# JiGuang283/Ray_Tracing-Rendering

Measured on AMD Instinct MI355X. Metric: Msamples/sec, Cornell Box 800x800 spp=400 MIS, higher is better.
Workload: dtype f64

## Files before the change

### ray_tracing-rendering_amd/csrc/rt_compile.h

```cpp
#pragma once

#include "rt_device.h"

#include <algorithm>
#include <cmath>
#include <cstdlib>
#include <cstring>
#include <map>
#include <set>
#include <vector>

struct CompiledScene {
    std::vector<FSub> subs;
    std::vector<rtr_node> dev_nodes;
    int n_compiled_subtrees = 0;
    std::vector<FInst> inst;
    std::vector<FXf> xf;
    std::vector<FRef> ref;
    std::vector<int32_t> exits;
    std::vector<FBvh> bvh;
    std::vector<double> scan;
    std::vector<FStep> steps;
    std::vector<FGuard> guards;
    std::map<int, std::pair<int, int>> guard_of_ref;
    int step_tail = 0;
    int stack_words = 1;
    bool ok = false;
};

namespace rtc {

constexpr int kLinearMax = 12;
constexpr int kLeafMax = 4;
constexpr int kGroupMax = 8;
constexpr int kMaxInstances = 1 << 18;
inline int top_tree_min() {
    const char* e = std::getenv("RTR_TOP_MIN");
    return e && *e ? std::atoi(e) : 40;
}
constexpr int kMaxTreeDepth = 56;

struct Box {
    double lo[3] = {INFINITY, INFINITY, INFINITY}, hi[3] = {-INFINITY, -INFINITY, -INFINITY};
    void grow(const double* p) {
        for (int c = 0; c < 3; ++c) lo[c] = std::min(lo[c], p[c]), hi[c] = std::max(hi[c], p[c]);
    }
    void grow(const Box& b) {
        grow(b.lo);
        grow(b.hi);
    }
    void pad() {
        for (int c = 0; c < 3; ++c) {
            const double e = 1e-4 + 1e-9 * std::max(std::fabs(lo[c]), std::fabs(hi[c]));
            lo[c] -= e, hi[c] += e;
        }
    }
};

struct PendingRef {
    int node;
    std::vector<int> wrappers;
    Box local;
    int order;
    int group;
    std::vector<int> guards;
};

struct Builder {
    const rtr_scene_desc* s;
    CompiledScene& out;
    int inst_base = 0;
    explicit Builder(CompiledScene& o) : out(o) {}
    double t_lo, t_hi;
    std::vector<int> chain;
    std::vector<int> wrappers;
    std::map<std::vector<uint64_t>, int> inst_of_chain;
    std::vector<std::vector<PendingRef>> pending;
    std::map<std::pair<int, std::vector<uint64_t>>, std::pair<int, int>> seen;
    int visit_counter = 0;
    int current_group = -1, group_counter = 0;
    bool too_complex = false;
    bool guard_mode = false, guard_fail = false;
    int hollows_seen = 0;
    std::vector<int> bvh_stack;
    std::map<std::pair<int, std::vector<uint64_t>>, int> hollows_at_first_visit;
    std::map<int, std::set<int>> hollows_under;
    static constexpr int kGuardLinearMax = 256;

    static uint64_t bits(double v) {
        uint64_t u;
        std::memcpy(&u, &v, 8);
        return u;
    }
    std::vector<uint64_t> chain_key() const {
        std::vector<uint64_t> k;
        for (int w : chain) {
            const rtr_node& n = s->nodes[w];
            k.push_back((uint64_t)n.type);
            k.push_back(bits(n.f[0])), k.push_back(bits(n.f[1])), k.push_back(bits(n.f[2]));
        }
        return k;
    }
    std::vector<uint64_t> full_key() const {
        std::vector<uint64_t> k = chain_key();
        k.push_back(~0ull);
        for (int w : wrappers) k.push_back((uint64_t)s->nodes[w].type);
        return k;
    }

    Box prim_box(const rtr_node& n) const {
        Box b;
        switch (n.type) {
        case RTR_NODE_SPHERE: {
            const double r = std::fabs(n.f[3]);
            double lo[3] = {n.f[0] - r, n.f[1] - r, n.f[2] - r}, hi[3] = {n.f[0] + r, n.f[1] + r, n.f[2] + r};
            b.grow(lo), b.grow(hi);
            break;
        }
        case RTR_NODE_MOVING_SPHERE: {
            const double r = std::fabs(n.f[8]);
            for (double t : {t_lo, t_hi}) {
                const double a = (t - n.f[6]) / (n.f[7] - n.f[6]);
                for (int c = 0; c < 3; ++c) {
                    const double ctr = n.f[c] + a * (n.f[3 + c] - n.f[c]);
                    b.lo[c] = std::min(b.lo[c], ctr - r), b.hi[c] = std::max(b.hi[c], ctr + r);
                }
            }
            break;
        }
        default: {
            const int ka = n.type == RTR_NODE_XY_RECT ? 2 : (n.type == RTR_NODE_XZ_RECT ? 1 : 0);
            const int aa = n.type == RTR_NODE_YZ_RECT ? 1 : 0;
            const int ba = n.type == RTR_NODE_XY_RECT ? 1 : 2;
            b.lo[ka] = n.f[4], b.hi[ka] = n.f[4];
            b.lo[aa] = std::min(n.f[0], n.f[1]), b.hi[aa] = std::max(n.f[0], n.f[1]);
            b.lo[ba] = std::min(n.f[2], n.f[3]), b.hi[ba] = std::max(n.f[2], n.f[3]);
        }
        }
        b.pad();
        return b;
    }

    void walk(int ix) {
        if (too_complex) return;
        const rtr_node& n = s->nodes[ix];
        switch (n.type) {
        case RTR_NODE_BVH:
            bvh_stack.push_back(ix);
            walk(n.a);
            if (n.b != n.a) walk(n.b);
            bvh_stack.pop_back();
            break;
        case RTR_NODE_LIST: {
            bool small = n.b >= 2 && n.b <= kGroupMax && current_group < 0;
            for (int k = 0; k < n.b && small; ++k) small = s->nodes[s->list_children[n.a + k]].type >= RTR_NODE_SPHERE;
            if (small) current_group = group_counter++;
            for (int k = 0; k < n.b; ++k) walk(s->list_children[n.a + k]);
            if (small) current_group = -1;
            break;
        }
        case RTR_NODE_TRANSLATE:
        case RTR_NODE_ROTATE_Y:
            chain.push_back(ix), wrappers.push_back(ix);
            walk(n.a);
            chain.pop_back(), wrappers.pop_back();
            break;
        case RTR_NODE_FLIP_FACE:
            wrappers.push_back(ix);
            walk(n.a);
            wrappers.pop_back();
            break;
        case RTR_NODE_MEDIUM: too_complex = true; break;
        default: {
            const int order = visit_counter++;
// ... 638 lines not shown
```

### ray_tracing-rendering_amd/csrc/rt_debug.h

```cpp
#pragma once

#include "rt_device.h"
#include "rtr_hip.h"

struct rtr_debug_view {
    DScene ds;
    hipStream_t stream;
    int device, n_cus, n_materials;
    int trav;
    size_t stack_bytes;
    int flat_trav;
};
struct rtr_debug_kernel {
    int pipeline;
    int integrator;
    int trav;
    int ms;
    int sorted;
    int shade_phases;
    int lean, quadlit, sort, media, machine;
    int accum;
};
struct rtr_debug_li_out {
    double L[3];
    uint32_t rng_exit;
    int32_t n_closest, n_shadow, pad;
};
struct rtr_debug_plan {
    int32_t fast_ok, has_media, flat_scene, flat_guarded, lean_materials, quad_lights_only, uv_order_dependent, machine_ok;
    int32_t guarded_program, top_tree, needs_uv, n_material_types, shared_div, pair_cast;
    int32_t n_steps, n_visits, n_refs, fast_stack_words, walk_stack_words, n_tie_refs, n_guard_refs;
    int32_t pick_trav, mega_trav, mega_ms, mega_sorted, mega_pair;
    int32_t n_finish;
};
extern "C" {
int rtr_debug_scene_plan(const rtr_scene_desc* scene, int integrator, int flags, rtr_debug_plan* out, size_t size_of_out,
                         int32_t* ref_flags, int64_t cap, void* finish, int64_t finish_cap);
int rtr_debug_frame_shapes(const rtr_scene_desc* scene, int32_t* shapes, int64_t cap, int32_t* n_inst);
int rtr_debug_view_get(rtr_context* ctx, int flags, rtr_debug_view* view, size_t size_of_view);
int rtr_debug_last_kernel(rtr_context* ctx, rtr_debug_kernel* out, size_t size_of_out);
int rtr_debug_li(rtr_context* ctx, const rtr_render_params* params, const int32_t* ijs, rtr_debug_li_out* out, int64_t n);
void rtr_debug_set_error(rtr_context* ctx, const char* msg);
}
```

### ray_tracing-rendering_amd/csrc/rt_device.h

```cpp
#pragma once

#include <hip/hip_runtime.h>
#include <stdint.h>

#include "rtr_hip.h"
#include "rtr_seed.h"

#ifndef RTR_BLOCK
#define RTR_BLOCK 256
#endif

#define RT_DEV __device__ __forceinline__
#define RT_HD __host__ __device__ __forceinline__

typedef double Real;

#define RT_STATS_WORDS 80
#define RT_PROF_BASE 8
#define RT_PROF_REGIONS 32
enum { RG_OTHER = 0, RG_SETUP = 1, RG_RECTS = 2, RG_SPHERES = 3, RG_GENERIC = 4, RG_TREE = 5, RG_LEAVES = 6, RG_FINISH = 7,
       RG_SH_SETUP = 8, RG_SH_RECTS = 9, RG_SH_SPHERES = 10, RG_SH_GENERIC = 11, RG_SH_TREE = 12, RG_SH_LEAVES = 13,
       RG_MEDIA = 14, RG_MATPREP = 15, RG_SHADE_A = 16, RG_SHADE_B = 17, RG_MISS = 18, RG_REGEN = 19, RG_SHADE_RR = 20,
       RG_PARK = 21, RG_BARRIER = 22, RG_EXCHANGE = 23, RG_PAIR_SETUP = 24, RG_PAIR_RUNS = 25, RG_PAIR_SPHERES = 26,
       RG_POLL = 27, RG_BEGIN = 28, RG_SETTLE = 29, RG_COUNT = 30, RG_REJECT = 31,
// ... 72 lines not shown
    s ^= s >> 17;
    s ^= s << 5;
    return s * 2.3283064365386963e-10;
}
RT_DEV Real rng_range(uint32_t& s, Real lo, Real hi) { return lo + (hi - lo) * rng_next(s); }
RT_DEV int rng_int(uint32_t& s, int lo, int hi) { return (int)rng_range(s, lo, hi + 1); }

RT_DEV Real rng_sym(uint32_t& s) {
    s ^= s << 13;
    s ^= s >> 17;
    s ^= s << 5;
    return -1.0 + s * 4.656612873077392578125e-10;
}

RT_DEV V3 random_in_unit_sphere(uint32_t& s) {
    const int region = RT_REGION_CURRENT();
    RT_REGION(RG_REJECT);
    for (;;) {
        Real z = rng_sym(s);
        Real y = rng_sym(s);
        Real x = rng_sym(s);
        V3 p = mk(x, y, z);
        if (len2(p) >= 1) continue;
        RT_REGION(region);
        return p;
    }
}
RT_DEV V3 random_unit_vector(uint32_t& s) { return unit(random_in_unit_sphere(s)); }
RT_DEV V3 random_in_unit_disk(uint32_t& s) {
    for (;;) {
        Real y = rng_sym(s);
        Real x = rng_sym(s);
        V3 p = mk(x, y, 0);
        if (len2(p) >= 1) continue;
        return p;
    }
}
RT_DEV V3 random_cosine_direction(uint32_t& s) {
    Real r1 = rng_next(s);
    Real r2 = rng_next(s);
    Real z = __builtin_sqrt(1 - r2);
    Real phi = 2 * RT_PI * r1;
    Real sphi, cphi;
    sincos(phi, &sphi, &cphi);
    Real x = cphi * __builtin_sqrt(r2);
    Real y = sphi * __builtin_sqrt(r2);
    return mk(x, y, z);
}

RT_DEV Real rcp_refined(Real d) {
    Real r = __builtin_amdgcn_rcp(d);
    Real e = __builtin_fma(-d, r, 1.0);
    r = __builtin_fma(r, e, r);
    e = __builtin_fma(-d, r, 1.0);
    return __builtin_fma(r, e, r);
}
RT_DEV bool rcp_safe(Real d) { return (__builtin_fabs(d) >= 0x1p-100) & (__builtin_fabs(d) <= 0x1p100); }
template <bool SHARED>
RT_DEV Real div_shared(Real n, Real d, Real r, bool guard) {
    if (!SHARED) return n / d;
    const Real q = n * r;
    const Real e = __builtin_fma(-d, q, n);
    Real t = __builtin_fma(e, r, q);
    if (guard && !(__builtin_fabs(n) >= 0x1p-300)) t = n / d;
    return t;
}
struct RayDiv {
    Real rx, ry, rz;
    Real a, ra;
    bool fast;
    bool guard;
};
RT_DEV RayDiv raydiv_none() {
    RayDiv q;
    q.rx = q.ry = q.rz = q.a = q.ra = 0;
    q.fast = q.guard = false;
    return q;
}
RT_DEV bool raydiv_origin_ok(V3 o) {
    return __all((__builtin_fabs(o.x) <= 0x1p80) & (__builtin_fabs(o.y) <= 0x1p80) & (__builtin_fabs(o.z) <= 0x1p80));
}
RT_DEV RayDiv raydiv_make(V3 d, Real tmin, bool origin_ok) {
    RayDiv q;
    q.rx = rcp_refined(d.x), q.ry = rcp_refined(d.y), q.rz = rcp_refined(d.z);
    q.a = q.ra = 0;
    q.guard = !(tmin >= 0x1p-100);
    q.fast = origin_ok && __all(rcp_safe(d.x) & rcp_safe(d.y) & rcp_safe(d.z));
    return q;
}
RT_DEV void raydiv_spheres(RayDiv& q, V3 d) {
    q.a = len2(d);
    q.ra = rcp_refined(q.a);
    q.fast = q.fast && __all(rcp_safe(q.a));
}
RT_DEV V3 raydiv_inv(const RayDiv& q, V3 d) {
    if (q.fast) return mk(q.rx, q.ry, q.rz);
    return mk(1.0 / d.x, 1.0 / d.y, 1.0 / d.z);
}

#define RT_CONST_AS __attribute__((address_space(4)))
template <class T>
RT_DEV const RT_CONST_AS T* as_const(const T* p) {
    return (const RT_CONST_AS T*)(unsigned long long)p;
}
template <class T>
RT_DEV T ld_const(const T* base, int idx) {
    static_assert(sizeof(T) % 8 == 0, "records are multiples of 8 bytes");
    const RT_CONST_AS unsigned long long* src = as_const(reinterpret_cast<const unsigned long long*>(base + idx));
    unsigned long long w[sizeof(T) / 8];
#pragma unroll
    for (unsigned k = 0; k < sizeof(T) / 8; ++k) w[k] = src[k];
    T v;
    __builtin_memcpy(&v, w, sizeof(T));
    return v;
}

struct DScene {
    const rtr_node* nodes;
    const int32_t* list_children;
    const rtr_material* materials;
    const rtr_texture* textures;
    const rtr_perlin* perlin;
    const rtr_image* images;
    const uint8_t* image_bytes;
    const rtr_light* lights;
    rtr_camera camera;
    double background[3];
    int32_t root;
    int32_t n_nodes;
    int32_t n_lights;
    int32_t needs_uv;
    int32_t shared_div;
    int32_t pair_cast;
    const struct FInst* finst;
    const struct FXf* fxf;
    const struct FRef* fref;
    const rtr_node* fprim;
    const double* fscan;
    const struct FMat* fmat;
    const struct FLeaf* fleaf;
    const int32_t* fexit;
    const struct FBvh* fbvh;
    const struct FSub* fsub;
    int32_t n_finst;
    int32_t top_root0, world_inst0, world_linear0;
    float top_bound0;
    int32_t n_fstep;
    const struct FStep* fstep;
    int32_t fstep_tail;
    const struct FGuard* fguard;
    int32_t n_fvisit;
    const struct FVisit* fvisit;
    const struct FFin* ffin;
};

struct FInst {
    double bmin[3], bmax[3];
    int32_t xf_first, n_xf;
    int32_t ref_first, n_ref;
    int32_t bvh_root;
    float bound;
    int32_t flags;
    int32_t scan_first;
    int32_t shape;
    uint64_t runs;
    int32_t xf_type[2];
    double xf_f[2][3];
    double head[6];
};
#define RT_INST_RUNS_MAX 8
#define RT_RUN_BITS 8
#define RT_RUN_COUNT_BITS 5
#define RT_RUN_COUNT_MAX 31
#define RT_INST_XF_INLINE 2
#define RT_INST_ROTATED 1
#define RT_INST_SPHERES 2
#define RT_INST_RUNS 4
#define RT_INST_KEEP_Y 8
#define RT_SHAPE_NONE 0
#define RT_SHAPE_T 1
#define RT_SHAPE_R 2
#define RT_SHAPE_TR 3
#define RT_SHAPE_RT 4
#define RT_SHAPE_OTHER 5
struct FXf {
    int32_t type;
    int32_t pad;
    double f[3];
};
#define RT_EXIT_LONG (~0ull)
struct FRef {
    int32_t node;
    int32_t exit_first;
    int32_t n_exit;
    int32_t pad;
};
struct alignas(16) FFin {
    int32_t kind;
    int32_t mat;
    int32_t levels;
    int32_t flip;
    double op[2][3];
    double g[4];
};
#define RT_FIN_SPHERE 3
#define RT_FIN_ROT0 4
#define RT_FIN_ROT1 8
struct FBvh {
    float lmin[3], lmax[3], rmin[3], rmax[3];
    int32_t left, right;
    int32_t pad[2];
};
#define RT_BVH_DONE (-2147483647 - 1)
struct FMat {
    int32_t type, solid;
    int32_t tex[4];
    int32_t pad[2];
    double f[4];
    double albedo[3];
    double rough, metal;
};
struct FLeaf {
    double f[6];
    int32_t type;
    int32_t tag;
    int32_t pad[2];
};
struct FSub {
    int32_t inst_first, n_inst;
    int32_t top_root;
    int32_t world_inst;
    int32_t world_linear;
    float top_bound;
    int32_t pad[2];
};
#define RT_TOP_INST (1 << 30)
#define RT_NODE_COMPILED 11
struct FStep {
    int32_t kind;
    int32_t sub;
    int32_t mat;
    int32_t pad;
    double neg_inv_density;
    int32_t xf_first, n_xf;
    int32_t exit_first, n_exit;
};
struct FGuard {
    double b[6];
};

struct Hit {
    V3 p, n;
    Real t, u, v;
    int mat;
    bool front;
};

RT_DEV void set_face_normal(Hit& rec, V3 rd, V3 outward) {
    rec.front = dot(rd, outward) < 0;
    rec.n = rec.front ? outward : neg(outward);
}

struct Stack {
    int* col;
    RT_DEV void put(int k, int v) const { col[k * RTR_BLOCK] = v; }
    RT_DEV int get(int k) const { return col[k * RTR_BLOCK]; }
    RT_DEV void putd(int k, Real v) const {
        put(k, __double2loint(v));
        put(k + 1, __double2hiint(v));
    }
    RT_DEV Real getd(int k) const { return __hiloint2double(get(k + 1), get(k)); }
};

#define RT_FRAME_TRANSLATE 8
#define RT_FRAME_ROTATE 14
#define RT_FRAME_FLIP 2
#define RT_LIST_BULK 8
#define RT_LIST_MARK 0x40000000

RT_DEV bool aabb_hit(const double* b, V3 o, V3 inv, Real t_min, Real t_max) {
    {
        Real t0 = (b[0] - o.x) * inv.x, t1 = (b[3] - o.x) * inv.x;
        if (inv.x < 0) {
            Real s = t0;
            t0 = t1, t1 = s;
        }
        t_min = t0 > t_min ? t0 : t_min;
        t_max = t1 < t_max ? t1 : t_max;
        if (t_max <= t_min) return false;
    }
    {
        Real t0 = (b[1] - o.y) * inv.y, t1 = (b[4] - o.y) * inv.y;
        if (inv.y < 0) {
            Real s = t0;
            t0 = t1, t1 = s;
        }
        t_min = t0 > t_min ? t0 : t_min;
        t_max = t1 < t_max ? t1 : t_max;
        if (t_max <= t_min) return false;
    }
    {
        Real t0 = (b[2] - o.z) * inv.z, t1 = (b[5] - o.z) * inv.z;
        if (inv.z < 0) {
            Real s = t0;
            t0 = t1, t1 = s;
        }
// ... 710 lines not shown
            for (int k = RT_INST_XF_INLINE; k < I.n_xf; ++k) {
                const FXf x = ld_const(sc.fxf, I.xf_first + k);
                wrapper_enter(x.type, x.f, lo, ld);
            }
        }
        bool found;
        if (I.bvh_root >= 0) {
            found = scan_instance<ANY, true, false, false>(sc, I, lo, ld, raydiv_none(), time, tmin, tmax, hit_ref, order, st, sp);
        } else if (I.flags & RT_INST_RUNS) {
            RayDiv q = raydiv_make(ld, tmin, origin_ok);
            if (I.flags & RT_INST_SPHERES) raydiv_spheres(q, ld);
            const bool one_box = I.runs == (uint64_t)(RT_RUN_BOX << RT_RUN_COUNT_BITS | 1);
            if (q.fast) {
                if (one_box)
                    run_box<false, true, true>(I.head, I.ref_first, lo, ld, q, tmin, tmax, hit_ref);
                else
                    scan_runs<false, true, true>(sc, I, lo, ld, q, time, tmin, tmax, hit_ref);
            } else {
                if (one_box)
                    run_box<false, false, true>(I.head, I.ref_first, lo, ld, q, tmin, tmax, hit_ref);
                else
                    scan_runs<false, false, true>(sc, I, lo, ld, q, time, tmin, tmax, hit_ref);
            }
            found = ANY && hit_ref != before;
        } else {
            found = leaf_refs<true, false, ANY>(sc, I.ref_first, I.ref_first + I.n_ref, lo, ld, time, tmin, tmax, hit_ref, order);
        }
        if (hit_ref != before) hit_inst = owner, tmax_f = float_above(tmax);
        if (ANY && found) return true;
        node = sp > sp0 ? st.get(--sp) : RT_BVH_DONE;
    }
    return false;
}

template <bool ANY, bool TREES, bool WEXIT, bool TOP, bool GUARD>
__device__ __forceinline__ bool trace_fast(const DScene& sc, const FSub sub, V3 o, V3 d, Real time, Real tmin, Real& tmax,
                                           int& hit_ref, int& hit_inst, const Stack st, const int sp0) {
    const bool top = TOP && sub.top_root >= 0;
    const int inst_first = top ? sub.world_inst : sub.inst_first;
    const int n_inst = top ? (sub.world_linear ? 1 : 0) : sub.n_inst;
    const bool use_boxes = n_inst > RT_FAST_NO_BOX_MAX;
    V3 inv = mk(0, 0, 0);
    if (use_boxes) inv = mk(1.0 / d.x, 1.0 / d.y, 1.0 / d.z);
    hit_ref = -1;
    hit_inst = -1;
    int order = -1;
#ifndef RTR_NO_SHARED_DIV
    const bool origin_ok = (RTR_TREE_SHARED || !TREES) && sc.shared_div != 0 && raydiv_origin_ok(o);
#endif
    for (int ii = inst_first; ii < inst_first + n_inst; ++ii) {
        RT_REGION(WEXIT ? RG_SH_SETUP : RG_SETUP);
        const FInst I = ld_const(sc.finst, ii);
        V3 lo = o, ld = d;
        const int n_xf = I.n_xf;
        if (n_xf) {
            if (use_boxes) {
                Real tn;
                if (!box_enter(I.bmin, I.bmax, o, inv, tmin, tmax, tn)) continue;
            }
            wrapper_enter(I.xf_type[0], I.xf_f[0], lo, ld);
            if (n_xf > 1) wrapper_enter(I.xf_type[1], I.xf_f[1], lo, ld);
            for (int k = RT_INST_XF_INLINE; k < n_xf; ++k) {
                const FXf x = ld_const(sc.fxf, I.xf_first + k);
                wrapper_enter(x.type, x.f, lo, ld);
            }
        }
        RayDiv q = raydiv_none();
#ifndef RTR_NO_SHARED_DIV
        if (RTR_TREE_SHARED || !TREES) {
            q = raydiv_make(ld, tmin, origin_ok);
            if (I.flags & RT_INST_SPHERES) raydiv_spheres(q, ld);
        }
#endif
        bool found;
        if (q.fast)
            found = scan_instance<ANY, TREES, WEXIT, true, GUARD>(sc, I, lo, ld, q, time, tmin, tmax, hit_ref, order, st, sp0);
        else
            found = scan_instance<ANY, TREES, WEXIT, false, GUARD>(sc, I, lo, ld, q, time, tmin, tmax, hit_ref, order, st, sp0);
        RT_REGION(WEXIT ? RG_SH_SETUP : RG_SETUP);
        if (hit_ref >= I.ref_first) hit_inst = ii;
        if (ANY && found) return true;
    }
    if (top) {
        RT_REGION(WEXIT ? RG_SH_TREE : RG_TREE);
        if (trace_top<ANY>(sc, sub, o, d, time, tmin, tmax, hit_ref, hit_inst, order, st, sp0) && ANY) return true;
    }
    return hit_ref >= 0;
}

template <int TYPE>
RT_DEV void pair_rect(Real a0, Real a1, Real b0, Real b1, Real k, int ref, V3 oA, V3 dA, const RayDiv& qA, Real& tmaxA,
                      int& hitA, V3 oB, V3 dB, const RayDiv& qB, Real& tmaxB, int& hitB) {
    const Real tmin = 0.001;
#define RT_PAIR_SEL(V, XY, XZ, YZ) (TYPE == RTR_NODE_XY_RECT ? V.XY : (TYPE == RTR_NODE_XZ_RECT ? V.XZ : V.YZ))
    const Real okA = RT_PAIR_SEL(oA, z, y, x), dkA = RT_PAIR_SEL(dA, z, y, x), rkA = RT_PAIR_SEL(qA, rz, ry, rx);
    const Real okB = RT_PAIR_SEL(oB, z, y, x), dkB = RT_PAIR_SEL(dB, z, y, x), rkB = RT_PAIR_SEL(qB, rz, ry, rx);
    const Real oaA = TYPE == RTR_NODE_YZ_RECT ? oA.y : oA.x, daA = TYPE == RTR_NODE_YZ_RECT ? dA.y : dA.x;
    const Real obA = TYPE == RTR_NODE_XY_RECT ? oA.y : oA.z, dbA = TYPE == RTR_NODE_XY_RECT ? dA.y : dA.z;
    const Real oaB = TYPE == RTR_NODE_YZ_RECT ? oB.y : oB.x, daB = TYPE == RTR_NODE_YZ_RECT ? dB.y : dB.x;
    const Real obB = TYPE == RTR_NODE_XY_RECT ? oB.y : oB.z, dbB = TYPE == RTR_NODE_XY_RECT ? dB.y : dB.z;
#undef RT_PAIR_SEL
    Real nA, nB, tA, tB, uA, wA, u;
    unsigned long long save;
    asm volatile("v_add_f64 %[nA], %[k], -%[okA]\n\t"
                 "v_add_f64 %[nB], %[k], -%[okB]\n\t"
                 "v_mul_f64 %[tA], %[nA], %[rkA]\n\t"
                 "v_mul_f64 %[tB], %[nB], %[rkB]\n\t"
                 "v_fma_f64 %[nA], -%[dkA], %[tA], %[nA]\n\t"
                 "v_fma_f64 %[nB], -%[dkB], %[tB], %[nB]\n\t"
                 "v_fma_f64 %[tA], %[nA], %[rkA], %[tA]\n\t"
                 "v_fma_f64 %[tB], %[nB], %[rkB], %[tB]\n\t"
                 "v_mul_f64 %[uA], %[tA], %[daA]\n\t"
                 "v_mul_f64 %[wA], %[tA], %[dbA]\n\t"
                 "v_add_f64 %[uA], %[oaA], %[uA]\n\t"
                 "v_add_f64 %[wA], %[obA], %[wA]"
                 : [nA] "=&v"(nA), [nB] "=&v"(nB), [tA] "=&v"(tA), [tB] "=&v"(tB), [uA] "=&v"(uA), [wA] "=&v"(wA)
                 : [k] "s"(k), [okA] "v"(okA), [dkA] "v"(dkA), [rkA] "v"(rkA), [okB] "v"(okB), [dkB] "v"(dkB), [rkB] "v"(rkB),
                   [oaA] "v"(oaA), [daA] "v"(daA), [obA] "v"(obA), [dbA] "v"(dbA));
    asm volatile("s_mov_b64 %[save], exec\n\t"
                 "v_cmpx_ngt_f64 vcc, %[tmin], %[tA]\n\t"
                 "v_cmpx_ngt_f64 vcc, %[tA], %[tmaxA]\n\t"
                 "v_cmpx_ngt_f64 vcc, %[a0], %[uA]\n\t"
                 "v_cmpx_nlt_f64 vcc, %[a1], %[uA]\n\t"
                 "v_cmpx_ngt_f64 vcc, %[b0], %[wA]\n\t"
                 "v_cmpx_nlt_f64 vcc, %[b1], %[wA]\n\t"
                 "v_mov_b64 %[tmaxA], %[tA]\n\t"
                 "v_mov_b32 %[hitA], %[ref]\n\t"
                 "s_mov_b64 exec, %[save]\n\t"
                 "v_cmpx_ngt_f64 vcc, %[tmin], %[tB]\n\t"
                 "v_cmpx_ngt_f64 vcc, %[tB], %[tmaxB]\n\t"
                 "s_cbranch_execz .Lpx%=\n\t"
                 "v_mul_f64 %[u], %[tB], %[daB]\n\t"
                 "v_add_f64 %[u], %[oaB], %[u]\n\t"
                 "v_cmpx_ngt_f64 vcc, %[a0], %[u]\n\t"
                 "v_cmpx_nlt_f64 vcc, %[a1], %[u]\n\t"
                 "v_mul_f64 %[u], %[tB], %[dbB]\n\t"
                 "v_add_f64 %[u], %[obB], %[u]\n\t"
                 "v_cmpx_ngt_f64 vcc, %[b0], %[u]\n\t"
                 "v_cmpx_nlt_f64 vcc, %[b1], %[u]\n\t"
                 "v_mov_b64 %[tmaxB], %[tB]\n\t"
                 "v_mov_b32 %[hitB], %[ref]\n"
                 ".Lpx%=:\n\t"
                 "s_mov_b64 exec, %[save]"
                 : [u] "=&v"(u), [save] "=&s"(save), [tmaxA] "+v"(tmaxA), [hitA] "+v"(hitA), [tmaxB] "+v"(tmaxB), [hitB] "+v"(hitB)
                 : [tA] "v"(tA), [uA] "v"(uA), [wA] "v"(wA), [tB] "v"(tB), [oaB] "v"(oaB), [daB] "v"(daB), [obB] "v"(obB),
                   [dbB] "v"(dbB), [a0] "s"(a0), [a1] "s"(a1), [b0] "s"(b0), [b1] "s"(b1), [ref] "s"(ref), [tmin] "s"(tmin)
                 : "vcc");
}
struct PairRay {
    V3 o, d;
    RayDiv q;
};
template <int TYPE>
RT_DEV void pair_rects(const RT_CONST_AS double* p, int cnt, int ref, const PairRay& A, Real& tmaxA, int& hitA, const PairRay& B,
                       Real& tmaxB, int& hitB) {
    int k = 0;
    for (; k + 1 < cnt; k += 2, p += 10) {
        const Real f0 = p[0], f1 = p[1], f2 = p[2], f3 = p[3], f4 = p[4];
        const Real g0 = p[5], g1 = p[6], g2 = p[7], g3 = p[8], g4 = p[9];
        pair_rect<TYPE>(f0, f1, f2, f3, f4, ref + k, A.o, A.d, A.q, tmaxA, hitA, B.o, B.d, B.q, tmaxB, hitB);
        pair_rect<TYPE>(g0, g1, g2, g3, g4, ref + k + 1, A.o, A.d, A.q, tmaxA, hitA, B.o, B.d, B.q, tmaxB, hitB);
    }
    if (k < cnt) pair_rect<TYPE>(p[0], p[1], p[2], p[3], p[4], ref + k, A.o, A.d, A.q, tmaxA, hitA, B.o, B.d, B.q, tmaxB, hitB);
}
RT_DEV void pair_runs(const DScene& sc, const FInst& I, const PairRay& A, Real time, Real& tmaxA, int& hitA, const PairRay& B,
                      Real& tmaxB, int& hitB) {
    const RT_CONST_AS double* p = as_const(sc.fscan) + I.scan_first;
    int ref = I.ref_first;
#pragma nounroll
    for (uint64_t runs = I.runs; runs != 0; runs >>= RT_RUN_BITS) {
        const int type = RTR_NODE_SPHERE + (int)((runs >> RT_RUN_COUNT_BITS) & 7), cnt = (int)(runs & RT_RUN_COUNT_MAX);
        RT_REGION(type >= RTR_NODE_XY_RECT ? RG_PAIR_RUNS : RG_PAIR_SPHERES);
        if (type == RTR_NODE_XY_RECT) {
            pair_rects<RTR_NODE_XY_RECT>(p, cnt, ref, A, tmaxA, hitA, B, tmaxB, hitB);
            p += 5 * cnt;
        } else if (type == RTR_NODE_XZ_RECT) {
            pair_rects<RTR_NODE_XZ_RECT>(p, cnt, ref, A, tmaxA, hitA, B, tmaxB, hitB);
            p += 5 * cnt;
        } else if (type == RTR_NODE_YZ_RECT) {
            pair_rects<RTR_NODE_YZ_RECT>(p, cnt, ref, A, tmaxA, hitA, B, tmaxB, hitB);
            p += 5 * cnt;
        } else if (type == RTR_NODE_SPHERE + RT_RUN_BOX) {
            for (int b = 0, r = ref; b < cnt; ++b, p += 6, r += 6) {
                const Real x0 = p[0], x1 = p[1], y0 = p[2], y1 = p[3], z0 = p[4], z1 = p[5];
                pair_rect<RTR_NODE_XY_RECT>(x0, x1, y0, y1, z1, r, A.o, A.d, A.q, tmaxA, hitA, B.o, B.d, B.q, tmaxB, hitB);
                pair_rect<RTR_NODE_XY_RECT>(x0, x1, y0, y1, z0, r + 1, A.o, A.d, A.q, tmaxA, hitA, B.o, B.d, B.q, tmaxB, hitB);
                pair_rect<RTR_NODE_XZ_RECT>(x0, x1, z0, z1, y1, r + 2, A.o, A.d, A.q, tmaxA, hitA, B.o, B.d, B.q, tmaxB, hitB);
                pair_rect<RTR_NODE_XZ_RECT>(x0, x1, z0, z1, y0, r + 3, A.o, A.d, A.q, tmaxA, hitA, B.o, B.d, B.q, tmaxB, hitB);
                pair_rect<RTR_NODE_YZ_RECT>(y0, y1, z0, z1, x1, r + 4, A.o, A.d, A.q, tmaxA, hitA, B.o, B.d, B.q, tmaxB, hitB);
                pair_rect<RTR_NODE_YZ_RECT>(y0, y1, z0, z1, x0, r + 5, A.o, A.d, A.q, tmaxA, hitA, B.o, B.d, B.q, tmaxB, hitB);
            }
            ref += 5 * cnt;
        } else {
            for (int k = 0; k < cnt; ++k, p += 4) {
                const V3 c = mk(p[0], p[1], p[2]);
                const Real r = p[3];
                Real t;
                if (sphere_hit_t<true>(c, r, A.o, A.d, A.q, 0.001, tmaxA, t)) tmaxA = t, hitA = ref + k;
                if (sphere_hit_t<true>(c, r, B.o, B.d, B.q, 0.001, tmaxB, t)) tmaxB = t, hitB = ref + k;
            }
        }
        ref += cnt;
    }
}
struct PairFrame {
    V3 ao, bo;
    Real adx, adz, bdx, bdz;
};
RT_HD void pair_rot(Real s, Real c, Real x, Real z, Real& rx, Real& rz) {
    rx = c * x - s * z;
    rz = s * x + c * z;
}
RT_HD PairFrame pair_frame(int shape, const double* f0, const double* f1, V3 ao, V3 ad, V3 bo, V3 bd) {
    PairFrame F;
    switch (shape) {
    case RT_SHAPE_T:
        F.ao.x = ao.x - f0[0], F.bo.x = bo.x - f0[0];
        F.ao.y = ao.y - f0[1], F.bo.y = bo.y - f0[1];
        F.ao.z = ao.z - f0[2], F.bo.z = bo.z - f0[2];
        F.adx = ad.x, F.adz = ad.z, F.bdx = bd.x, F.bdz = bd.z;
        break;
    case RT_SHAPE_R:
        pair_rot(f0[0], f0[1], ao.x, ao.z, F.ao.x, F.ao.z), pair_rot(f0[0], f0[1], bo.x, bo.z, F.bo.x, F.bo.z);
        F.ao.y = ao.y, F.bo.y = bo.y;
        pair_rot(f0[0], f0[1], ad.x, ad.z, F.adx, F.adz), pair_rot(f0[0], f0[1], bd.x, bd.z, F.bdx, F.bdz);
        break;
    case RT_SHAPE_TR: {
        const Real ax = ao.x - f0[0], bx = bo.x - f0[0];
        const Real az = ao.z - f0[2], bz = bo.z - f0[2];
        F.ao.y = ao.y - f0[1], F.bo.y = bo.y - f0[1];
        pair_rot(f1[0], f1[1], ax, az, F.ao.x, F.ao.z), pair_rot(f1[0], f1[1], bx, bz, F.bo.x, F.bo.z);
        pair_rot(f1[0], f1[1], ad.x, ad.z, F.adx, F.adz), pair_rot(f1[0], f1[1], bd.x, bd.z, F.bdx, F.bdz);
        break;
    }
    case RT_SHAPE_RT: {
        Real ax, az, bx, bz;
        pair_rot(f0[0], f0[1], ao.x, ao.z, ax, az), pair_rot(f0[0], f0[1], bo.x, bo.z, bx, bz);
        pair_rot(f0[0], f0[1], ad.x, ad.z, F.adx, F.adz), pair_rot(f0[0], f0[1], bd.x, bd.z, F.bdx, F.bdz);
        F.ao.x = ax - f1[0], F.bo.x = bx - f1[0];
        F.ao.y = ao.y - f1[1], F.bo.y = bo.y - f1[1];
        F.ao.z = az - f1[2], F.bo.z = bz - f1[2];
        break;
    }
    default:
        F.ao = ao, F.bo = bo;
        F.adx = ad.x, F.adz = ad.z, F.bdx = bd.x, F.bdz = bd.z;
        break;
    }
    return F;
}
__device__ __forceinline__ void trace_pair(const DScene& sc, V3 ao, V3 ad, Real atime, Real& a_tmax, int& a_ref, int& a_inst,
                                           V3 bo, V3 bd, Real& b_tmax, int& b_ref, const Stack st) {
    a_ref = -1, a_inst = -1, b_ref = -1;
#ifndef RTR_NO_SHARED_DIV
    const bool ok_a = raydiv_origin_ok(ao), ok_b = raydiv_origin_ok(bo);
#else
    const bool ok_a = false, ok_b = false;
#endif
    const Real way = rcp_refined(ad.y), wby = rcp_refined(bd.y);
    const bool wa_y = rcp_safe(ad.y), wb_y = rcp_safe(bd.y);
    for (int ii = 0; ii < sc.n_finst; ++ii) {
        RT_REGION(RG_PAIR_SETUP);
        const FInst I = ld_const(sc.finst, ii);
        PairRay A, B;
        if (I.shape != RT_SHAPE_OTHER) {
            const PairFrame F = pair_frame(I.shape, I.xf_f[0], I.xf_f[1], ao, ad, bo, bd);
            A.o = F.ao, B.o = F.bo;
            A.d = mk(F.adx, ad.y, F.adz), B.d = mk(F.bdx, bd.y, F.bdz);
        } else {
            A.o = ao, A.d = ad, B.o = bo, B.d = bd;
            wrapper_enter(I.xf_type[0], I.xf_f[0], A.o, A.d);
            wrapper_enter(I.xf_type[0], I.xf_f[0], B.o, B.d);
            if (I.n_xf > 1) {
                wrapper_enter(I.xf_type[1], I.xf_f[1], A.o, A.d);
                wrapper_enter(I.xf_type[1], I.xf_f[1], B.o, B.d);
            }
            for (int k = RT_INST_XF_INLINE; k < I.n_xf; ++k) {
                const FXf x = ld_const(sc.fxf, I.xf_first + k);
                wrapper_enter(x.type, x.f, A.o, A.d);
                wrapper_enter(x.type, x.f, B.o, B.d);
            }
        }
        A.q.guard = B.q.guard = false;
        A.q.rx = rcp_refined(A.d.x), A.q.rz = rcp_refined(A.d.z);
        B.q.rx = rcp_refined(B.d.x), B.q.rz = rcp_refined(B.d.z);
        A.q.ry = way, B.q.ry = wby;
        bool sa = rcp_safe(A.d.x) & rcp_safe(A.d.z) & wa_y, sb = rcp_safe(B.d.x) & rcp_safe(B.d.z) & wb_y;
        A.q.a = A.q.ra = B.q.a = B.q.ra = 0;
        if (I.flags & RT_INST_SPHERES) {
            A.q.a = len2(A.d), B.q.a = len2(B.d);
            A.q.ra = rcp_refined(A.q.a), B.q.ra = rcp_refined(B.q.a);
            sa = sa & rcp_safe(A.q.a), sb = sb & rcp_safe(B.q.a);
        }
        if (ok_a && ok_b && __all(sa & sb)) {
            A.q.fast = B.q.fast = true;
            pair_runs(sc, I, A, atime, a_tmax, a_ref, B, b_tmax, b_ref);
        } else {
            A.q.fast = ok_a && __all(sa), B.q.fast = ok_b && __all(sb);
            int order = -1;
            if (A.q.fast)
                scan_instance<false, false, false, true>(sc, I, A.o, A.d, A.q, atime, 0.001, a_tmax, a_ref, order, st, 0);
            else
                scan_instance<false, false, false, false>(sc, I, A.o, A.d, A.q, atime, 0.001, a_tmax, a_ref, order, st, 0);
            if (B.q.fast)
                scan_instance<true, false, true, true>(sc, I, B.o, B.d, B.q, 0.0, 0.001, b_tmax, b_ref, order, st, 0);
            else
                scan_instance<true, false, true, false>(sc, I, B.o, B.d, B.q, 0.0, 0.001, b_tmax, b_ref, order, st, 0);
        }
        RT_REGION(RG_PAIR_SETUP);
        if (a_ref >= I.ref_first) a_inst = ii;
    }
}

template <bool UV>
__device__ __forceinline__ void fast_finish_long(const DScene& sc, V3 o, V3 d, Real time, Real t, int ref, int inst, Hit& rec) {
    const FInst I = ld_const(sc.finst, inst);
    const FRef R = ld_const(sc.fref, ref);
    V3 lo = o, ld = d;
    for (int k = 0; k < I.n_xf; ++k) {
        const FXf x = ld_const(sc.fxf, I.xf_first + k);
        wrapper_enter(x.type, x.f, lo, ld);
    }
    const rtr_node n = ld_const(sc.fprim, ref);
    const int type = n.type;
    if (type >= RTR_NODE_XY_RECT) {
        Real oa, da, ob, db;
        if (type == RTR_NODE_XY_RECT) {
            oa = lo.x, da = ld.x, ob = lo.y, db = ld.y;
        } else if (type == RTR_NODE_XZ_RECT) {
            oa = lo.x, da = ld.x, ob = lo.z, db = ld.z;
        } else {
            oa = lo.y, da = ld.y, ob = lo.z, db = ld.z;
        }
        rect_fill(n, type, lo, ld, t, oa + t * da, ob + t * db, UV, rec);
    } else {
        V3 center;
        Real radius;
        sphere_geom(n, type, time, center, radius);
        sphere_fill(n, type, center, radius, lo, ld, t, UV, rec);
    }
    int level = I.n_xf;
    for (int e = 0; e < R.n_exit; ++e) {
        const rtr_node w = ld_const(sc.nodes, as_const(sc.fexit)[R.exit_first + e]);
        V3 wd = d;
        if (w.type != RTR_NODE_FLIP_FACE) {
            V3 wo = o;
            for (int k = 0; k < level; ++k) {
                const FXf x = ld_const(sc.fxf, I.xf_first + k);
                wrapper_enter(x.type, x.f, wo, wd);
            }
            --level;
        }
        wrapper_epilogue(w, wd, rec);
    }
}
RT_DEV void xf_exit(bool rot, Real f0, Real f1, Real f2, V3 wd, Hit& rec) {
    if (!rot) {
        rec.p = add(rec.p, mk(f0, f1, f2));
        set_face_normal(rec, wd, rec.n);
    } else {
        const Real s = f0, c = f1;
        V3 p = rec.p, nn = rec.n;
        p.x = c * rec.p.x + s * rec.p.z;
        p.z = -s * rec.p.x + c * rec.p.z;
        nn.x = c * rec.n.x + s * rec.n.z;
        nn.z = -s * rec.n.x + c * rec.n.z;
        rec.p = p;
        set_face_normal(rec, wd, nn);
    }
}
RT_DEV void xf_epilogue(int type, const double* f, V3 wd, Hit& rec) {
    xf_exit(type != RTR_NODE_TRANSLATE, f[0], f[1], f[2], wd, rec);
}
template <bool UV>
RT_DEV void fast_finish_flat(const FFin* ffin, V3 o, V3 d, Real t, int ref, Hit& rec) {
    FFin F = ld_const(ffin, ref);
    asm volatile("" : "+v"(F.kind), "+v"(F.mat), "+v"(F.levels), "+v"(F.flip));
    asm volatile("" : "+v"(F.op[0][0]), "+v"(F.op[0][1]), "+v"(F.op[0][2]), "+v"(F.op[1][0]), "+v"(F.op[1][1]), "+v"(F.op[1][2]));
    asm volatile("" : "+v"(F.g[0]), "+v"(F.g[1]), "+v"(F.g[2]), "+v"(F.g[3]));
    const int n_lev = F.levels & 3;
    const bool rot0 = (F.levels & RT_FIN_ROT0) != 0, rot1 = (F.levels & RT_FIN_ROT1) != 0;
    V3 lo = o, ld = d, d1 = d;
    if (n_lev > 0) {
        xf_enter(rot0, F.op[0][0], F.op[0][1], F.op[0][2], lo, ld);
        d1 = ld;
        if (n_lev > 1) xf_enter(rot1, F.op[1][0], F.op[1][1], F.op[1][2], lo, ld);
    }
    rec.t = t;
    if (F.kind != RT_FIN_SPHERE) {
        if (UV) {
            const Real oa = F.kind == 0 ? lo.y : lo.x, da = F.kind == 0 ? ld.y : ld.x;
            const Real ob = F.kind == 2 ? lo.y : lo.z, db = F.kind == 2 ? ld.y : ld.z;
            const Real a = oa + t * da, b = ob + t * db;
            rec.u = (a - F.g[0]) / (F.g[1] - F.g[0]);
            rec.v = (b - F.g[2]) / (F.g[3] - F.g[2]);
        }
        const V3 outward = mk(F.kind == 0 ? 1.0 : 0.0, F.kind == 1 ? 1.0 : 0.0, F.kind == 2 ? 1.0 : 0.0);
        set_face_normal(rec, ld, outward);
        rec.p = add(lo, scl(t, ld));
    } else {
        rec.p = add(lo, scl(t, ld));
        const V3 outward = divs(sub(rec.p, mk(F.g[0], F.g[1], F.g[2])), F.g[3]);
        set_face_normal(rec, ld, outward);
        if (UV) sphere_uv(outward, rec.u, rec.v);
    }
    rec.mat = F.mat;
    if (n_lev > 1) xf_exit(rot1, F.op[1][0], F.op[1][1], F.op[1][2], ld, rec);
    if (n_lev > 0) xf_exit(rot0, F.op[0][0], F.op[0][1], F.op[0][2], d1, rec);
    rec.front = rec.front != (F.flip != 0);
}
template <bool UV, bool FLAT>
RT_DEV void fast_finish(const DScene& sc, V3 o, V3 d, Real time, Real t, int ref, int inst, Hit& rec) {
    RT_REGION(RG_FINISH);
    if (FLAT && sc.ffin != nullptr) {
        fast_finish_flat<UV>(sc.ffin, o, d, t, ref, rec);
        return;
    }
    const FInst I = ld_const(sc.finst, inst);
    const rtr_node n = ld_const(sc.fprim, ref);
    unsigned long long code = (unsigned long long)__double_as_longlong(n.f[9]);
    const int type = n.type;
    if (I.n_xf > RT_INST_XF_INLINE || type == RTR_NODE_MOVING_SPHERE || code == RT_EXIT_LONG) {
        fast_finish_long<UV>(sc, o, d, time, t, ref, inst, rec);
        return;
    }
    V3 lo = o, ld = d;
    V3 d1 = d;
    if (I.n_xf > 0) {
        wrapper_enter(I.xf_type[0], I.xf_f[0], lo, ld);
        d1 = ld;
        if (I.n_xf > 1) wrapper_enter(I.xf_type[1], I.xf_f[1], lo, ld);
    }
    if (type >= RTR_NODE_XY_RECT) {
        Real oa, da, ob, db;
        if (type == RTR_NODE_XY_RECT) {
            oa = lo.x, da = ld.x, ob = lo.y, db = ld.y;
        } else if (type == RTR_NODE_XZ_RECT) {
            oa = lo.x, da = ld.x, ob = lo.z, db = ld.z;
        } else {
            oa = lo.y, da = ld.y, ob = lo.z, db = ld.z;
        }
        rect_fill(n, type, lo, ld, t, oa + t * da, ob + t * db, UV, rec);
    } else {
        sphere_fill(n, type, ld3(n.f), n.f[3], lo, ld, t, UV, rec);
    }
    int level = I.n_xf;
    for (; code != 0; code >>= 2) {
        if ((code & 3) == 2) {
            rec.front = !rec.front;
        } else {
            --level;
            const bool outer = level == 0;
            const double f[3] = {outer ? I.xf_f[0][0] : I.xf_f[1][0], outer ? I.xf_f[0][1] : I.xf_f[1][1],
                                 outer ? I.xf_f[0][2] : I.xf_f[1][2]};
            xf_epilogue(outer ? I.xf_type[0] : I.xf_type[1], f, outer ? d1 : ld, rec);
        }
    }
}

#define RT_TRAV_EXACT 0
#define RT_TRAV_MEDIA 1
#define RT_TRAV_FAST 2
#define RT_TRAV_PROGRAM 3
#define RT_TRAV_FLAT 4
// ... 1030 lines not shown
```

### ray_tracing-rendering_amd/csrc/rt_kernels.h

```cpp
#pragma once

#include "rt_render.h"

#ifndef RTR_MEGA_WAVES
#define RTR_MEGA_WAVES 4
#endif
#ifndef RTR_PROGRAM_WAVES
#define RTR_PROGRAM_WAVES 3
#endif

constexpr int mega_waves(int integ, int trav, int ms) {
    if (ms == RT_MS_LEAN) return RTR_MEGA_WAVES;
    if (rt_is_program(trav)) return RTR_PROGRAM_WAVES;
    if (trav == RT_TRAV_MEDIA || trav == RT_TRAV_EXACT) return 2;
    if (ms == RT_MS_QUADLIT) return 3;
    if (integ == RTR_INTEGRATOR_RR || integ == RTR_INTEGRATOR_PATH) return 3;
    return 2;
}

#define RT_PARK_WORDS 19
struct Park {
    double* base;
    RT_DEV V3 get3(int k) const { return mk(base[k * RTR_BLOCK], base[(k + 1) * RTR_BLOCK], base[(k + 2) * RTR_BLOCK]); }
    RT_DEV void set3(int k, V3 v) const {
// ... 187 lines not shown
            if (!__syncthreads_or(!done)) break;
            RT_REGION(RG_EXCHANGE);
            const int c0 = s_cnt[0], c1 = s_cnt[1], c2 = s_cnt[2], c3 = s_cnt[3];
            int b0 = 0, b1 = (c0 + 63) & ~63, b2 = b1 + ((c1 + 63) & ~63), b3 = b2 + ((c2 + 63) & ~63);
            if (b3 + c3 > RTR_BLOCK) b1 = c0, b2 = c0 + c1, b3 = c0 + c1 + c2;
            const int pos = (cls == 0 ? b0 : (cls == 1 ? b1 : (cls == 2 ? b2 : b3))) + ticket;
            if (shade_me) {
                xw[(SX_P + 0) * RTR_BLOCK + pos] = rec.p.x, xw[(SX_P + 1) * RTR_BLOCK + pos] = rec.p.y, xw[(SX_P + 2) * RTR_BLOCK + pos] = rec.p.z;
                xw[(SX_N + 0) * RTR_BLOCK + pos] = rec.n.x, xw[(SX_N + 1) * RTR_BLOCK + pos] = rec.n.y, xw[(SX_N + 2) * RTR_BLOCK + pos] = rec.n.z;
                xw[(SX_RD + 0) * RTR_BLOCK + pos] = ps.rd.x, xw[(SX_RD + 1) * RTR_BLOCK + pos] = ps.rd.y, xw[(SX_RD + 2) * RTR_BLOCK + pos] = ps.rd.z;
                const unsigned long long pack = (unsigned long long)rng | ((unsigned long long)(rec.mat & 0xffff) << 32) |
                                                ((unsigned long long)threadIdx.x << 48) | ((unsigned long long)(rec.front ? 1 : 0) << 56) |
                                                ((unsigned long long)(ps.depth >= P.rr_start ? 1 : 0) << 57);
                xw[SX_PACK * RTR_BLOCK + pos] = __longlong_as_double((long long)pack);
            }
            RT_REGION(RG_BARRIER);
            __syncthreads();
            RT_REGION(RG_EXCHANGE);
            if (threadIdx.x < 4) s_cnt[threadIdx.x] = 0;
            {
                const int q = threadIdx.x;
                const bool mine = (q >= b0 && q < b0 + c0) || (q >= b1 && q < b1 + c1) || (q >= b2 && q < b2 + c2) || (q >= b3 && q < b3 + c3);
                if (mine) {
                    const unsigned long long pack = (unsigned long long)__double_as_longlong(xin[SX_PACK * RTR_BLOCK + q]);
                    Hit h;
                    h.u = 0, h.v = 0, h.t = 0;
                    h.p = mk(xin[(SX_P + 0) * RTR_BLOCK + q], xin[(SX_P + 1) * RTR_BLOCK + q], xin[(SX_P + 2) * RTR_BLOCK + q]);
                    h.n = mk(xin[(SX_N + 0) * RTR_BLOCK + q], xin[(SX_N + 1) * RTR_BLOCK + q], xin[(SX_N + 2) * RTR_BLOCK + q]);
                    h.mat = (int)((pack >> 32) & 0xffff);
                    h.front = ((pack >> 56) & 1) != 0;
                    const int owner = (int)((pack >> 48) & 0xff);
                    const Park po{pk.base - threadIdx.x + owner};
                    PathState sh;
                    sh.rd = mk(xin[(SX_RD + 0) * RTR_BLOCK + q], xin[(SX_RD + 1) * RTR_BLOCK + q], xin[(SX_RD + 2) * RTR_BLOCK + q]);
                    sh.ro = h.p, sh.tm = 0;
                    sh.thr = po.get3(SK_THR);
                    sh.L = mk(0.0, 0.0, 0.0);
                    sh.prev_bsdf_pdf = 0.0;
                    sh.depth = ((pack >> 57) & 1) ? P.rr_start : P.rr_start - 1;
                    sh.specular_bounce = false;
                    uint32_t r2 = (uint32_t)pack;
                    const V3 wo = neg(unit(sh.rd));
                    ShadowReq rq;
                    const MatCtx mc = mat_prepare<MS>(sc, h);
                    shade_a_mis<MS, INTEG, 2>(sc, sh, h, mc, wo, r2, rq);
                    if (rq.valid) {
                        po.set3(SK_SWI, rq.wi);
                        po.set(SK_STMAX, rq.tmax);
                        po.set3(SK_CONTRIB, rq.contrib);
                    }
                    const bool go = shade_b_mis<MS, INTEG>(sc, sh, h, mc, wo, r2, P.rr_start);
                    po.set3(SK_THR, sh.thr);
                    po.set(SK_PDF, sh.prev_bsdf_pdf);
                    xw[(SX_RD + 0) * RTR_BLOCK + q] = sh.rd.x, xw[(SX_RD + 1) * RTR_BLOCK + q] = sh.rd.y, xw[(SX_RD + 2) * RTR_BLOCK + q] = sh.rd.z;
                    const unsigned long long back = (unsigned long long)r2 | ((unsigned long long)(go ? 1 : 0) << 32) |
                                                    ((unsigned long long)(sh.specular_bounce ? 1 : 0) << 33) |
                                                    ((unsigned long long)(rq.valid ? 1 : 0) << 34);
                    xw[SX_PACK * RTR_BLOCK + q] = __longlong_as_double((long long)back);
                }
            }
            RT_REGION(RG_BARRIER);
            __syncthreads();
            RT_REGION(RG_PARK);
            if (shade_me) {
                const unsigned long long back = (unsigned long long)__double_as_longlong(xin[SX_PACK * RTR_BLOCK + pos]);
                rng = (uint32_t)back;
                ps.ro = mk(xin[(SX_P + 0) * RTR_BLOCK + pos], xin[(SX_P + 1) * RTR_BLOCK + pos], xin[(SX_P + 2) * RTR_BLOCK + pos]);
                ps.rd = mk(xin[(SX_RD + 0) * RTR_BLOCK + pos], xin[(SX_RD + 1) * RTR_BLOCK + pos], xin[(SX_RD + 2) * RTR_BLOCK + pos]);
                ps.specular_bounce = ((back >> 33) & 1) != 0;
                pending = ((back >> 34) & 1) != 0;
                const bool go = ((back >> 32) & 1) != 0;
                ended = !go || ++ps.depth >= P.max_depth;
            }
            RT_REGION(RG_OTHER);
            if (pending) {
                pk.set(SK_NSHADOW, pk.get(SK_NSHADOW) + 1.0);
                if (!cast_shadow<TRAV>(sc, ps.ro, pk.get3(SK_SWI), pk.get(SK_STMAX), rng, st))
                    pk.set3(SK_L, add(pk.get3(SK_L), pk.get3(SK_CONTRIB)));
            }
            RT_REGION(RG_REGEN);
            if (ended) {
                const V3 L = pk.get3(SK_L);
                accp[0] += L.x, accp[RTR_BLOCK] += L.y, accp[2 * RTR_BLOCK] += L.z;
                if (ACC == 2) {
                    const double y = luminance(L);
                    q += y * y;
                }
                ++n_samples;
                ++s;
                done = s >= s_end || ((s & 7) == 0 && render_cancelled(P));
                if (!done) begin_sample<SK_THR, SK_L, SK_PDF>(sc, P, pk, slot, s, rng, ps);
            }
        }
        cnt.closest = (uint32_t)pk.get(SK_NCLOSEST);
        cnt.shadow = (uint32_t)pk.get(SK_NSHADOW);
    } else if (TRAV == RT_TRAV_MEDIA) {
        V3 acc = acc_start<ACC>(P, slot);
        while (!done) {
            if (fresh) {
                if ((s & 7) == 0 && render_cancelled(P)) break;
                V3 ro, rd;
                Real tm;
                camera_sample(sc, P, i, j, s, rng, ro, rd, tm);
                path_begin(ps, ro, rd, tm);
                fresh = false;
            }
            if (!bounce<INTEG, TRAV>(sc, ps, rng, st, P.max_depth, P.rr_start, cnt)) {
                acc = add(acc, ps.L);
                if (ACC == 2) {
                    const double y = luminance(ps.L);
                    q += y * y;
                }
                ++n_samples;
                ++s;
                fresh = true;
                done = s >= s_end;
            }
        }
        pk.set3(PK_ACC, acc);
    } else if (PAIR) {
        pk.set2(PK_NCAST, 0u, 0u);
        pk.set2(PK_PIXEL, (uint32_t)i, (uint32_t)j);
        pk.set3(PK_L, mk(0.0, 0.0, 0.0));
        if (!done) begin_sample<PK_THR, -1, PK_PDF, PK_PIXEL>(sc, P, pk, slot, s, rng, ps);
        uint32_t it = 0;
        bool pending = false;
        bool settle = false;
        V3 so = mk(0.0, 0.0, 0.0);
        PhaseClocks clk;
        while (!done || settle) {
            RTR_CLK(other);
            RT_REGION(RG_OTHER);
            const bool cast_a = !done;
            Real a_tmax = RT_INF, b_tmax = 0.0;
            int a_ref, a_inst, b_ref;
            V3 swi = mk(1.0, 1.0, 1.0);
            RT_REGION(RG_COUNT);
            {
                uint32_t n_closest, n_shadow;
                pk.get2(PK_NCAST, n_closest, n_shadow);
                pk.set2(PK_NCAST, n_closest + (cast_a ? 1u : 0u), n_shadow + (pending ? 1u : 0u));
            }
            RT_REGION(RG_OTHER);
            if (!cast_a) {
                ps.ro = mk(0.0, 0.0, 0.0), ps.rd = mk(1.0, 1.0, 1.0), ps.tm = 0.0;
                a_tmax = 0.0;
            }
            if (pending) {
                swi = pk.get3(PK_SWI);
                b_tmax = pk.get(PK_STMAX);
            } else {
                so = mk(0.0, 0.0, 0.0);
            }
            trace_pair(sc, ps.ro, ps.rd, ps.tm, a_tmax, a_ref, a_inst, so, swi, b_tmax, b_ref, st);
            RTR_CLK(closest);
            RT_REGION(RG_POLL);
            const uint32_t cancel_word = cancel_poll_issue(P, it++);
            RT_REGION(RG_SETTLE);
            const bool lit = pending && b_ref < 0;
            if (lit || settle) {
                V3 L = pk.get3(PK_L);
                if (lit) L = add(L, pk.get3(PK_CONTRIB));
                if (settle) {
                    pk.set3(PK_ACC, add(pk.get3(PK_ACC), L));
                    if (ACC == 2) {
                        const double y = luminance(L);
                        q += y * y;
                    }
                    L = mk(0.0, 0.0, 0.0);
                    settle = false;
                }
                pk.set3(PK_L, L);
            }
            pending = false;
            RTR_CLK(shadow);
            if (cast_a) {
                bool ended;
                if (a_ref < 0) {
                    RT_REGION(RG_MISS);
                    pk.set3(PK_L, add(pk.get3(PK_L), miss_radiance<INTEG, MS>(sc, pk.get3(PK_THR), ps.ro, ps.rd, ps.depth,
                                                                          ps.specular_bounce, pk.get(PK_PDF))));
                    ended = true;
                } else {
                    Hit rec;
                    rec.u = 0, rec.v = 0;
                    if (MS == RT_MS_FULL && sc.needs_uv)
                        fast_finish<true, true>(sc, ps.ro, ps.rd, ps.tm, a_tmax, a_ref, a_inst, rec);
                    else
                        fast_finish<false, true>(sc, ps.ro, ps.rd, ps.tm, a_tmax, a_ref, a_inst, rec);
                    ps.thr = pk.get3(PK_THR);
                    ps.L = mk(0.0, 0.0, 0.0);
                    ps.prev_bsdf_pdf = pk.get(PK_PDF);
                    const V3 wo = neg(unit(ps.rd));
                    ParkedReq rq{false, pk};
                    const MatCtx mc = mat_prepare<MS>(sc, rec);
                    shade_a_mis<MS, INTEG>(sc, ps, rec, mc, wo, rng, rq);
                    pending = rq.valid;
                    const bool go = shade_b_mis<MS, INTEG>(sc, ps, rec, mc, wo, rng, P.rr_start);
                    RT_REGION(RG_PARK);
                    ps.ro = rec.p;
                    so = rec.p;
                    pk.set3(PK_THR, ps.thr);
                    if (ps.L.x != 0.0 || ps.L.y != 0.0 || ps.L.z != 0.0) pk.set3(PK_L, add(pk.get3(PK_L), ps.L));
                    pk.set(PK_PDF, ps.prev_bsdf_pdf);
                    ended = !go || ++ps.depth >= P.max_depth;
                }
                RTR_CLK(shade);
                RT_REGION(RG_REGEN);
                if (ended) {
                    settle = true;
                    ++n_samples;
                    ++s;
                    done = s >= s_end;
                    RT_REGION(RG_BEGIN);
                    if (!done) begin_sample<PK_THR, -1, PK_PDF, PK_PIXEL>(sc, P, pk, slot, s, rng, ps);
                }
            }
            RT_REGION(RG_POLL);
            if (cancel_poll_take(P, cancel_word)) done = true;
        }
        pk.get2(PK_NCAST, cnt.closest, cnt.shadow);
        clk.flush(P);
    } else {
        pk.set2(PK_NCAST, 0u, 0u);
        pk.set2(PK_PIXEL, (uint32_t)i, (uint32_t)j);
        if (!done) begin_sample<PK_THR, PK_L, PK_PDF, PK_PIXEL>(sc, P, pk, slot, s, rng, ps);
        PhaseClocks clk;
        uint32_t it = 0;
        while (!done) {
            bool pending = false, ended = false;
            bool shadowed = false;
            RTR_CLK(other);
            RT_REGION(RG_OTHER);
            {
                Hit rec;
                rec.u = 0, rec.v = 0;
                const bool hit_any = cast_closest<TRAV, MS == RT_MS_FULL>(sc, ps.ro, ps.rd, ps.tm, rec, rng, st);
                RTR_CLK(closest);
                if (!hit_any) {
                    RT_REGION(RG_MISS);
                    pk.set3(PK_L, add(pk.get3(PK_L), miss_radiance<INTEG, MS>(sc, pk.get3(PK_THR), ps.ro, ps.rd, ps.depth,
                                                                          ps.specular_bounce, pk.get(PK_PDF))));
                    ended = true;
                } else {
                    ps.thr = pk.get3(PK_THR);
                    ps.L = mk(0.0, 0.0, 0.0);
                    ps.prev_bsdf_pdf = pk.get(PK_PDF);
                    bool go;
                    if (INTEG == RTR_INTEGRATOR_RR) {
                        go = shade_rr<MS>(sc, ps, rec, rng, P.rr_start);
                    } else if (INTEG == RTR_INTEGRATOR_PATH) {
                        go = shade_path<MS>(sc, ps, rec, rng);
                    } else {
                        const V3 wo = neg(unit(ps.rd));
                        ShadowReq rq;
                        MatCtx mc = mat_prepare<MS>(sc, rec);
                        shade_a_mis<MS, INTEG>(sc, ps, rec, mc, wo, rng, rq);
                        if (rt_is_program(TRAV)) {
                            if (ps.L.x != 0.0 || ps.L.y != 0.0 || ps.L.z != 0.0) {
                                pk.set3(PK_L, add(pk.get3(PK_L), ps.L));
                                ps.L = mk(0.0, 0.0, 0.0);
                            }
                            if (rq.valid) {
                                shadowed = true;
                                if (!cast_shadow<TRAV>(sc, rec.p, rq.wi, rq.tmax, rng, st))
                                    pk.set3(PK_L, add(pk.get3(PK_L), rq.contrib));
                                mc = mat_prepare<MS>(sc, rec);
                            }
                        } else if (rq.valid) {
                            pending = true;
                            pk.set3(PK_SWI, rq.wi);
                            pk.set(PK_STMAX, rq.tmax);
                            pk.set3(PK_CONTRIB, rq.contrib);
                        }
                        go = shade_b_mis<MS, INTEG>(sc, ps, rec, mc, wo, rng, P.rr_start);
                    }
                    RT_REGION(RG_PARK);
                    ps.ro = rec.p;
                    pk.set3(PK_THR, ps.thr);
                    if (ps.L.x != 0.0 || ps.L.y != 0.0 || ps.L.z != 0.0) pk.set3(PK_L, add(pk.get3(PK_L), ps.L));
                    pk.set(PK_PDF, ps.prev_bsdf_pdf);
                    ended = !go || ++ps.depth >= P.max_depth;
                }
            }
            RTR_CLK(shade);
            RT_REGION(RG_OTHER);
            if (pending) {
                if (!cast_shadow<TRAV>(sc, ps.ro, pk.get3(PK_SWI), pk.get(PK_STMAX), rng, st))
                    pk.set3(PK_L, add(pk.get3(PK_L), pk.get3(PK_CONTRIB)));
            }
            RTR_CLK(shadow);
            RT_REGION(RG_POLL);
            const uint32_t cancel_word = cancel_poll_issue(P, it++);
            RT_REGION(RG_REGEN);
            if (ended) {
                pk.set3(PK_ACC, add(pk.get3(PK_ACC), pk.get3(PK_L)));
                if (ACC == 2) {
                    const double y = luminance(pk.get3(PK_L));
                    q += y * y;
                }
                ++n_samples;
                ++s;
                done = s >= s_end;
                RT_REGION(RG_BEGIN);
                if (!done) begin_sample<PK_THR, PK_L, PK_PDF, PK_PIXEL>(sc, P, pk, slot, s, rng, ps);
            }
            RT_REGION(RG_COUNT);
// ... 5 lines not shown
            RT_REGION(RG_POLL);
            if (cancel_poll_take(P, cancel_word)) done = true;
        }
        pk.get2(PK_NCAST, cnt.closest, cnt.shadow);
        clk.flush(P);
    }
#ifdef RTR_REGION_PROFILE
    RT_REGION(RG_OTHER);
    __syncthreads();
    if (threadIdx.x < 2 * RT_PROF_REGIONS) {
        unsigned long long v = 0;
        for (int w = 0; w < 4; ++w) v += rt_prof_lds[w * 2 * RT_PROF_REGIONS + threadIdx.x];
        if (v) atomicAdd(&P.stats[RT_PROF_BASE + threadIdx.x], v);
    }
#endif
    if (!SORT) {
        const V3 acc = pk.get3(PK_ACC);
        double* out = P.partial + (size_t)cell * 3 * RTR_BLOCK + threadIdx.x;
        out[0] = acc.x;
        out[RTR_BLOCK] = acc.y;
        out[2 * RTR_BLOCK] = acc.z;
    }
    if (ACC == 2) P.q_part[(size_t)cell * RTR_BLOCK + threadIdx.x] = q;
    unsigned long long a = wave_sum(n_samples), b = wave_sum(cnt.closest), c = wave_sum(cnt.shadow);
    if ((threadIdx.x & 63) == 0) {
        atomicAdd(&P.stats[0], a);
        atomicAdd(&P.stats[1], b);
        atomicAdd(&P.stats[2], c);
    }
    const int interrupted = __syncthreads_or(active && s < s_end);
    if (threadIdx.x == 0) {
        P.done[cell] = !interrupted;
        if (interrupted) atomicAdd(&P.stats[7], 1ull);
    }
}


struct QueueWave {
    int block;
    int next;
    unsigned long long samples;
};
RT_DEV bool queue_take(const RenderK& P, uint32_t* __restrict__ q_counter, const int n_blocks, QueueWave& qw, bool need,
                       const Park& pk, int* my_cell, int& s) {
    bool got = false;
    unsigned long long m = __ballot(need);
    while (m) {
        if (qw.block >= 0 && qw.next == RT_QUEUE_JOBS) {
            const int first = __builtin_ctzll(m);
            uint32_t b = 0;
            if ((int)__lane_id() == first) b = atomicAdd(q_counter, 1u);
            b = (uint32_t)__builtin_amdgcn_readlane((int)b, first);
            qw.block = b < (uint32_t)n_blocks ? (int)b : -1;
            qw.next = 0;
        }
        if (qw.block < 0) {
            if (need) *my_cell = -1;
            break;
        }
        const QueueBlock qb = queue_block(P, qw.block);
        const int tile = P.tile_ids[qb.slot];
        const int tile_y = (P.tiles_y - 1) - tile / P.tiles_x;
        const int tile_x = tile % P.tiles_x;
        const int cell = qb.slot * P.chunks + qb.chunk;
        const int k = qw.next + (int)__builtin_amdgcn_mbcnt_hi((uint32_t)(m >> 32), __builtin_amdgcn_mbcnt_lo((uint32_t)m, 0u));
        bool now = false;
        if (need && k < RT_QUEUE_JOBS) {
            const int i = tile_x * 16 + (k & 15), j = tile_y * 16 + qb.quarter * 4 + (k >> 4);
            if (i >= P.x0 && i < P.x1 && j >= P.y0 && j < P.y1 && qb.s0 < qb.s1) {
                uint32_t lo, hi;
                queue_pack(i, j, qb.s1, lo, hi);
                pk.set2(PK_PIXEL, lo, hi);
                *my_cell = cell;
                s = qb.s0;
                got = now = true, need = false;
            } else {
                atomicAdd(&P.done[cell], 1);
            }
        }
        qw.samples += (unsigned long long)__builtin_popcountll(__ballot(now)) * (unsigned long long)(qb.s1 - qb.s0);
        const int taken = qw.next + (int)__builtin_popcountll(m);
        qw.next = taken < RT_QUEUE_JOBS ? taken : RT_QUEUE_JOBS;
        m = __ballot(need);
    }
    return got;
}

template <int INTEG, int TRAV, int MS>
__global__ void __launch_bounds__(RTR_BLOCK, mega_waves(INTEG, TRAV, MS))
    k_mega_queue(const DScene* __restrict__ scp, const RenderK P, const int stack_words, uint32_t* __restrict__ q_counter,
                 const int n_blocks) {
    static_assert(mega_pairable(INTEG, TRAV), "no pair-cast variant of this kernel");
    extern __shared__ int lds_stack[];
    const DScene& sc = *scp;
    const Stack st{lds_stack + threadIdx.x};
    const Park pk{reinterpret_cast<double*>(lds_stack + stack_words * RTR_BLOCK) + threadIdx.x};
    int* const my_cell = lds_stack + threadIdx.x;
#ifdef RTR_REGION_PROFILE
    if (threadIdx.x < 4 * 2 * RT_PROF_REGIONS + 8) rt_prof_lds[threadIdx.x] = 0;
    if (threadIdx.x + 256 < 4 * 2 * RT_PROF_REGIONS + 8) rt_prof_lds[threadIdx.x + 256] = 0;
    __syncthreads();
    if ((threadIdx.x & 63) == 0) rt_prof_lds[4 * 2 * RT_PROF_REGIONS + (threadIdx.x >> 6) * 2] = __builtin_readcyclecounter();
#endif
    PathCounters cnt;
    cnt.closest = 0, cnt.shadow = 0;
    PathState ps;
    uint32_t rng = 1;
    int s = 0;
    QueueWave qw{0, RT_QUEUE_JOBS, 0ull};
    pk.set3(PK_ACC, mk(0.0, 0.0, 0.0));
    pk.set2(PK_NCAST, 0u, 0u);
    pk.set3(PK_L, mk(0.0, 0.0, 0.0));
    *my_cell = -1;
    bool done = !queue_take(P, q_counter, n_blocks, qw, true, pk, my_cell, s);
    if (!done) {
        uint32_t lo, hi;
        int i, j, s_end;
        pk.get2(PK_PIXEL, lo, hi);
        queue_unpack(lo, hi, i, j, s_end);
        camera_sample(sc, P, i, j, s, rng, ps.ro, ps.rd, ps.tm);
        ps.depth = 0, ps.specular_bounce = false;
        pk.set3(PK_THR, mk(1.0, 1.0, 1.0));
        pk.set(PK_PDF, 0.0);
    }
    uint32_t it = 0;
    bool pending = false;
    bool settle = false;
    V3 so = mk(0.0, 0.0, 0.0);
    PhaseClocks clk;
    while (!done || settle) {
        RTR_CLK(other);
        RT_REGION(RG_OTHER);
        const bool cast_a = !done;
        Real a_tmax = RT_INF, b_tmax = 0.0;
        int a_ref, a_inst, b_ref;
        V3 swi = mk(1.0, 1.0, 1.0);
        RT_REGION(RG_COUNT);
        {
            uint32_t n_closest, n_shadow;
            pk.get2(PK_NCAST, n_closest, n_shadow);
            pk.set2(PK_NCAST, n_closest + (cast_a ? 1u : 0u), n_shadow + (pending ? 1u : 0u));
        }
        RT_REGION(RG_OTHER);
        if (!cast_a) {
            ps.ro = mk(0.0, 0.0, 0.0), ps.rd = mk(1.0, 1.0, 1.0), ps.tm = 0.0;
            a_tmax = 0.0;
        }
        if (pending) {
            swi = pk.get3(PK_SWI);
            b_tmax = pk.get(PK_STMAX);
        } else {
            so = mk(0.0, 0.0, 0.0);
        }
        trace_pair(sc, ps.ro, ps.rd, ps.tm, a_tmax, a_ref, a_inst, so, swi, b_tmax, b_ref, st);
        RTR_CLK(closest);
        RT_REGION(RG_POLL);
        const uint32_t cancel_word = cancel_poll_issue(P, it++);
        RT_REGION(RG_SETTLE);
        const bool lit = pending && b_ref < 0;
        if (lit || settle) {
            V3 L = pk.get3(PK_L);
            if (lit) L = add(L, pk.get3(PK_CONTRIB));
            if (settle) {
                pk.set3(PK_ACC, add(pk.get3(PK_ACC), L));
                L = mk(0.0, 0.0, 0.0);
                settle = false;
            }
            pk.set3(PK_L, L);
        }
        pending = false;
        RTR_CLK(shadow);
        bool begin = false;
        if (cast_a) {
            bool ended;
            if (a_ref < 0) {
                RT_REGION(RG_MISS);
                pk.set3(PK_L, add(pk.get3(PK_L), miss_radiance<INTEG, MS>(sc, pk.get3(PK_THR), ps.ro, ps.rd, ps.depth,
                                                                      ps.specular_bounce, pk.get(PK_PDF))));
                ended = true;
            } else {
                Hit rec;
                rec.u = 0, rec.v = 0;
                if (MS == RT_MS_FULL && sc.needs_uv)
                    fast_finish<true, true>(sc, ps.ro, ps.rd, ps.tm, a_tmax, a_ref, a_inst, rec);
                else
                    fast_finish<false, true>(sc, ps.ro, ps.rd, ps.tm, a_tmax, a_ref, a_inst, rec);
                ps.thr = pk.get3(PK_THR);
                ps.L = mk(0.0, 0.0, 0.0);
                ps.prev_bsdf_pdf = pk.get(PK_PDF);
                const V3 wo = neg(unit(ps.rd));
                ParkedReq rq{false, pk};
                const MatCtx mc = mat_prepare<MS>(sc, rec);
                shade_a_mis<MS, INTEG>(sc, ps, rec, mc, wo, rng, rq);
                pending = rq.valid;
                const bool go = shade_b_mis<MS, INTEG>(sc, ps, rec, mc, wo, rng, P.rr_start);
                RT_REGION(RG_PARK);
                ps.ro = rec.p;
                so = rec.p;
                pk.set3(PK_THR, ps.thr);
                if (ps.L.x != 0.0 || ps.L.y != 0.0 || ps.L.z != 0.0) pk.set3(PK_L, add(pk.get3(PK_L), ps.L));
                pk.set(PK_PDF, ps.prev_bsdf_pdf);
                ended = !go || ++ps.depth >= P.max_depth;
            }
            RTR_CLK(shade);
            RT_REGION(RG_REGEN);
            if (ended) {
                settle = true;
                ++s;
                begin = true;
            }
        }
        const bool job_end = !cast_a && *my_cell >= 0;
        if (__ballot(job_end)) {
            RT_REGION(RG_EXCHANGE);
            if (job_end) {
                uint32_t lo, hi;
                pk.get2(PK_PIXEL, lo, hi);
                const V3 acc = pk.get3(PK_ACC);
                const int cell = *my_cell;
                double* out = P.partial + (size_t)cell * 3 * RTR_BLOCK + ((lo >> 12) & 0xf0u) + (lo & 0xfu);
                out[0] = acc.x;
                out[RTR_BLOCK] = acc.y;
                out[2 * RTR_BLOCK] = acc.z;
                atomicAdd(&P.done[cell], 1);
                pk.set3(PK_ACC, mk(0.0, 0.0, 0.0));
            }
            if (queue_take(P, q_counter, n_blocks, qw, job_end, pk, my_cell, s)) done = false, begin = true;
        }
        if (begin) {
            uint32_t lo, hi;
            int i, j, s_end;
            pk.get2(PK_PIXEL, lo, hi);
            queue_unpack(lo, hi, i, j, s_end);
            done = s >= s_end;
            if (!done) {
                RT_REGION(RG_BEGIN);
                camera_sample(sc, P, i, j, s, rng, ps.ro, ps.rd, ps.tm);
                ps.depth = 0, ps.specular_bounce = false;
                pk.set3(PK_THR, mk(1.0, 1.0, 1.0));
                pk.set(PK_PDF, 0.0);
            }
        }
        RT_REGION(RG_POLL);
        if (__any(cancel_poll_take(P, cancel_word))) {
            const unsigned long long here = __ballot(1);
            if ((int)__lane_id() == __builtin_ctzll(here)) atomicAdd(&P.stats[7], 1ull);
            int left = 0;
            if (*my_cell >= 0) {
                uint32_t lo, hi;
                pk.get2(PK_PIXEL, lo, hi);
                left = (int)hi - s;
            }
            for (unsigned long long m = __ballot(left > 0); m; m &= m - 1)
                qw.samples -= (unsigned long long)__builtin_amdgcn_readlane(left, __builtin_ctzll(m));
            *my_cell = -1;
            done = true;
        }
    }
    pk.get2(PK_NCAST, cnt.closest, cnt.shadow);
    clk.flush(P);
#ifdef RTR_REGION_PROFILE
    RT_REGION(RG_OTHER);
    __syncthreads();
    if (threadIdx.x < 2 * RT_PROF_REGIONS) {
        unsigned long long v = 0;
        for (int w = 0; w < 4; ++w) v += rt_prof_lds[w * 2 * RT_PROF_REGIONS + threadIdx.x];
        if (v) atomicAdd(&P.stats[RT_PROF_BASE + threadIdx.x], v);
    }
#endif
    unsigned long long b = wave_sum(cnt.closest), c = wave_sum(cnt.shadow);
    if ((threadIdx.x & 63) == 0) {
        atomicAdd(&P.stats[0], qw.samples);
        atomicAdd(&P.stats[1], b);
        atomicAdd(&P.stats[2], c);
    }
}

struct LiOut {
    double L[3];
    uint32_t rng_exit;
    int32_t n_closest, n_shadow, pad;
};
template <int INTEG, int TRAV>
__global__ void __launch_bounds__(RTR_BLOCK) k_li(const DScene sc, const RenderK P, const int32_t* __restrict__ ijs,
                                                   const rtr_li_ray* __restrict__ rays, LiOut* __restrict__ out, long long n) {
    extern __shared__ int lds_stack[];
    const Stack st{lds_stack + threadIdx.x};
    const long long k = (long long)blockIdx.x * RTR_BLOCK + threadIdx.x;
    if (k >= n) return;
    uint32_t rng;
    V3 ro, rd;
    Real tm;
    if (rays) {
        const rtr_li_ray r = rays[k];
        ro = ld3(r.origin), rd = ld3(r.direction), tm = r.time, rng = r.rng_state;
    } else {
        const int i = ijs[3 * k], j = ijs[3 * k + 1], s = ijs[3 * k + 2];
        camera_sample(sc, P, i, j, s, rng, ro, rd, tm);
    }
    PathState ps;
    path_begin(ps, ro, rd, tm);
    PathCounters cnt;
    cnt.closest = 0, cnt.shadow = 0;
    while (bounce<INTEG, TRAV>(sc, ps, rng, st, P.max_depth, P.rr_start, cnt)) {
    }
    LiOut o;
    o.L[0] = ps.L.x, o.L[1] = ps.L.y, o.L[2] = ps.L.z;
// ... 779 lines not shown
```

### ray_tracing-rendering_amd/csrc/rt_lower.h

```cpp
#pragma once

#include "rt_compile.h"
#include "rt_machine.h"

#include <functional>

struct SceneFacts {
    int fast_stack_words = 1;
    int walk_extra_words = 0;
    bool lean_materials = false;
    bool quad_lights_only = false;
    bool flat_scene = false;
    bool flat_guarded = false;
    bool uv_order_dependent = false;
    bool machine_ok = false;
    bool guarded_program = false;
    bool top_tree = false;
    bool needs_uv = false;
    bool pair_cast = false;
    int n_material_types = 0;
    int n_materials = 0;
    double t_lo = 0, t_hi = 0;
    bool camera_times_small = true;
};
// ... 180 lines not shown
    std::vector<FLeaf> out(prims.size());
    for (size_t r = 0; r < prims.size(); ++r) {
        FLeaf L{};
        const rtr_node& n = prims[r];
        const int nf = n.type == RTR_NODE_SPHERE ? 4 : (n.type == RTR_NODE_MOVING_SPHERE ? 0 : 5);
        for (int k = 0; k < nf; ++k) L.f[k] = n.f[k];
        L.type = n.type, L.tag = n.reserved;
        out[r] = L;
    }
    return out;
}

inline void build_scan_runs(CompiledScene& cs, const std::vector<rtr_node>& prims) {
    cs.scan.clear();
    for (FInst& I : cs.inst) {
        I.flags &= ~RT_INST_RUNS;
        I.scan_first = 0;
        I.runs = 0;
        if (I.bvh_root >= 0 || I.n_ref == 0) continue;
        std::vector<std::pair<int, int>> runs;
        std::vector<double> data;
        bool ok = true;
        const int kBox = RTR_NODE_SPHERE + RT_RUN_BOX;
        auto same = [](double a, double b) { return std::memcmp(&a, &b, 8) == 0; };
        auto box_at = [&](int r) {
            if (r + 6 > I.ref_first + I.n_ref) return false;
            const rtr_node* p = &prims[r];
            static const int want_type[6] = {RTR_NODE_XY_RECT, RTR_NODE_XY_RECT, RTR_NODE_XZ_RECT,
                                             RTR_NODE_XZ_RECT, RTR_NODE_YZ_RECT, RTR_NODE_YZ_RECT};
            for (int k = 0; k < 6; ++k)
                if (p[k].type != want_type[k] || (p[k].reserved & RT_TIE_FLAG)) return false;
            const double x0 = p[0].f[0], x1 = p[0].f[1], y0 = p[0].f[2], y1 = p[0].f[3], z1 = p[0].f[4], z0 = p[1].f[4];
            const double want[6][5] = {{x0, x1, y0, y1, z1}, {x0, x1, y0, y1, z0}, {x0, x1, z0, z1, y1},
                                       {x0, x1, z0, z1, y0}, {y0, y1, z0, z1, x1}, {y0, y1, z0, z1, x0}};
            for (int k = 0; k < 6; ++k)
                for (int c = 0; c < 5; ++c)
                    if (!same(p[k].f[c], want[k][c])) return false;
            return true;
        };
        for (int r = I.ref_first; r < I.ref_first + I.n_ref && ok;) {
            const rtr_node& n = prims[r];
            if (n.reserved & RT_TIE_FLAG) ok = false;
            const bool box = box_at(r);
            const bool guarded = (n.reserved & RT_GUARD_FLAG) != 0;
            const int type = box ? kBox : (guarded ? RTR_NODE_SPHERE + RT_RUN_GUARDED : n.type);
            if (runs.empty() || runs.back().first != type || runs.back().second == RT_RUN_COUNT_MAX) runs.push_back({type, 0});
            ++runs.back().second;
            if (guarded) {
                data.insert(data.end(), n.f, n.f + 6);
                r += 1;
            } else if (box) {
                const double rec[6] = {n.f[0], n.f[1], n.f[2], n.f[3], prims[r + 1].f[4], n.f[4]};
                data.insert(data.end(), rec, rec + 6);
                r += 6;
            } else {
                const int nf = n.type == RTR_NODE_SPHERE ? 4 : (n.type == RTR_NODE_MOVING_SPHERE ? 9 : 5);
                data.insert(data.end(), n.f, n.f + nf);
                r += 1;
            }
        }
        if (!ok || (int)runs.size() > RT_INST_RUNS_MAX) continue;
        I.scan_first = (int32_t)cs.scan.size();
        for (size_t k = 0; k < runs.size(); ++k)
            I.runs |= (uint64_t)((runs[k].first - RTR_NODE_SPHERE) << RT_RUN_COUNT_BITS | runs[k].second) << (RT_RUN_BITS * k);
        cs.scan.insert(cs.scan.end(), data.begin(), data.end());
        for (size_t k = 0; k < 6; ++k) I.head[k] = k < data.size() ? data[k] : 0.0;
        I.flags |= RT_INST_RUNS;
    }
    cs.scan.resize(cs.scan.size() + 16, 0.0);
}

inline std::vector<FMat> build_materials(const rtr_scene_desc* s) {
    std::vector<FMat> fm((size_t)s->n_materials);
    auto solid = [&](int t) { return t >= 0 && s->textures[t].type == RTR_TEX_SOLID; };
    auto clampd = [](double x, double lo, double hi) { return x < lo ? lo : (x > hi ? hi : x); };
    for (int k = 0; k < s->n_materials; ++k) {
        const rtr_material& m = s->materials[k];
        FMat f{};
        f.type = m.type;
        for (int q = 0; q < 4; ++q) f.tex[q] = m.tex[q], f.f[q] = m.f[q];
        switch (m.type) {
        case RTR_MAT_LAMBERTIAN:
        case RTR_MAT_DIFFUSE_LIGHT:
        case RTR_MAT_ISOTROPIC: f.solid = solid(m.tex[0]); break;
        case RTR_MAT_PBR: f.solid = solid(m.tex[0]) && solid(m.tex[1]) && solid(m.tex[2]) && m.tex[3] < 0; break;
        default: f.solid = 1;
        }
        if (f.solid && m.type != RTR_MAT_METAL && m.type != RTR_MAT_DIELECTRIC) {
            for (int q = 0; q < 3; ++q) f.albedo[q] = s->textures[m.tex[0]].f[q];
            if (m.type == RTR_MAT_PBR) {
                f.rough = clampd(s->textures[m.tex[1]].f[0], 0.01, 1.0);
                f.metal = s->textures[m.tex[2]].f[0];
            }
        }
        fm[(size_t)k] = f;
    }
    return fm;
}

inline bool shared_div_allowed(const rtr_scene_desc* s, const CompiledScene& cs) {
    for (int k = 0; k < s->n_nodes; ++k) {
        const rtr_node& n = s->nodes[k];
        const int nf = n.type == RTR_NODE_TRANSLATE ? 3 : n.type == RTR_NODE_SPHERE ? 4 : n.type == RTR_NODE_MOVING_SPHERE ? 9
                       : n.type >= RTR_NODE_XY_RECT ? 5 : 0;
        for (int q = 0; q < nf; ++q)
            if (!(std::fabs(n.f[q]) <= 0x1p60)) return false;
        if (n.type == RTR_NODE_MOVING_SPHERE && !(std::fabs(n.f[7] - n.f[6]) >= 0x1p-20)) return false;
    }
    if (!(std::fabs(s->camera.time0) <= 0x1p60 && std::fabs(s->camera.time1) <= 0x1p60)) return false;
    for (const FInst& I : cs.inst)
        if (I.n_xf > 30) return false;
    return !getenv("RTR_NO_SHARED_DIV");
}

inline int frame_shape(const FInst& I) {
    if (I.n_xf == 0) return RT_SHAPE_NONE;
    if (I.n_xf > RT_INST_XF_INLINE) return RT_SHAPE_OTHER;
    int code = 0;
    for (int k = 0; k < I.n_xf; ++k) {
        if (I.xf_type[k] == RTR_NODE_TRANSLATE) {
            code = code << 2 | 1;
        } else if (I.xf_type[k] == RTR_NODE_ROTATE_Y) {
            code = code << 2 | 2;
        } else {
            return RT_SHAPE_OTHER;
        }
    }
    switch (code) {
    case 1: return RT_SHAPE_T;
    case 2: return RT_SHAPE_R;
    case 1 << 2 | 2: return RT_SHAPE_TR;
    case 2 << 2 | 1: return RT_SHAPE_RT;
    default: return RT_SHAPE_OTHER;
    }
}

inline bool pair_cast_allowed(const rtr_scene_desc* s, const CompiledScene& cs, const DScene& d, bool flat_scene) {
    if (!(flat_scene && s->n_lights > 0 && d.shared_div && d.top_root0 < 0 && d.n_finst > 0 && d.n_finst <= RT_FAST_NO_BOX_MAX))
        return false;
    for (int k = 0; k < d.n_finst; ++k) {
        const FInst& I = cs.inst[k];
        if (!(I.flags & RT_INST_RUNS)) return false;
        if (!(I.flags & RT_INST_KEEP_Y)) return false;
        for (uint64_t runs = I.runs; runs != 0; runs >>= RT_RUN_BITS) {
            const int type = RTR_NODE_SPHERE + (int)((runs >> RT_RUN_COUNT_BITS) & 7);
            if (type != RTR_NODE_SPHERE && type != RTR_NODE_XY_RECT && type != RTR_NODE_XZ_RECT && type != RTR_NODE_YZ_RECT &&
                type != RTR_NODE_SPHERE + RT_RUN_BOX)
                return false;
        }
    }
    return true;
}

inline std::vector<FFin> build_finish(const CompiledScene& cs, const std::vector<rtr_node>& prims, bool flat) {
    std::vector<FFin> out;
    if (!flat || !cs.ok || cs.subs.empty()) return out;
    const FSub& sub0 = cs.subs[0];
    out.assign(prims.size(), FFin{});
    for (int ii = sub0.inst_first; ii < sub0.inst_first + sub0.n_inst; ++ii) {
        const FInst& I = cs.inst[ii];
        if (I.n_xf > RT_INST_XF_INLINE) return {};
        for (int r = I.ref_first; r < I.ref_first + I.n_ref; ++r) {
            const rtr_node& n = prims[r];
            unsigned long long code;
            std::memcpy(&code, &n.f[9], 8);
            if (n.type == RTR_NODE_MOVING_SPHERE || code == RT_EXIT_LONG) return {};
            FFin F{};
            F.kind = n.type == RTR_NODE_SPHERE ? RT_FIN_SPHERE : (n.type == RTR_NODE_YZ_RECT ? 0 : (n.type == RTR_NODE_XZ_RECT ? 1 : 2));
            F.mat = n.a;
            F.levels = I.n_xf;
            for (int k = 0; k < I.n_xf; ++k) {
                if (I.xf_type[k] == RTR_NODE_ROTATE_Y) F.levels |= k == 0 ? RT_FIN_ROT0 : RT_FIN_ROT1;
                for (int q = 0; q < 3; ++q) F.op[k][q] = I.xf_f[k][q];
            }
            int left = I.n_xf, flips = 0;
            for (; code != 0; code >>= 2) {
                if ((code & 3) == 2)
                    ++flips;
                else
                    --left, flips = 0;
            }
            if (left != 0) return {};
            F.flip = flips & 1;
            for (int q = 0; q < 4; ++q) F.g[q] = n.f[q];
            out[(size_t)r] = F;
        }
    }
    return out;
}

inline void material_facts(const rtr_scene_desc* s, SceneFacts& f) {
    f.n_materials = s->n_materials;
    f.lean_materials = true;
    unsigned type_mask = 0;
    for (int k = 0; k < s->n_materials; ++k) type_mask |= 1u << s->materials[k].type;
    f.n_material_types = __builtin_popcount(type_mask);
    f.quad_lights_only = true;
    for (int k = 0; k < s->n_lights; ++k)
        if (s->lights[k].type != RTR_LIGHT_QUAD) f.quad_lights_only = false;
    if (!f.quad_lights_only) f.lean_materials = false;
    for (int k = 0; k < s->n_materials; ++k) {
        const rtr_material& m = s->materials[k];
        if (m.type != RTR_MAT_LAMBERTIAN && m.type != RTR_MAT_DIFFUSE_LIGHT) f.lean_materials = false;
        else if (s->textures[m.tex[0]].type != RTR_TEX_SOLID) f.lean_materials = false;
    }
}

inline bool uv_order_dependent(const rtr_scene_desc* s, const rtr_scene_info& info) {
    if (!info.needs_uv) return false;
    std::function<bool(int, int)> tex_reads_uv = [&](int t, int guard) {
        if (t < 0 || guard > 8) return false;
        const rtr_texture& x = s->textures[t];
        if (x.type == RTR_TEX_IMAGE) return x.a >= 0;
        if (x.type == RTR_TEX_CHECKER) return tex_reads_uv(x.a, guard + 1) || tex_reads_uv(x.b, guard + 1);
        return false;
    };
    for (int k = 0; k < s->n_nodes; ++k) {
        if (s->nodes[k].type != RTR_NODE_MOVING_SPHERE) continue;
        const rtr_material& m = s->materials[s->nodes[k].a];
        const int n_tex = m.type == RTR_MAT_PBR ? 4 : (m.type == RTR_MAT_METAL || m.type == RTR_MAT_DIELECTRIC ? 0 : 1);
        for (int q = 0; q < n_tex; ++q)
            if (tex_reads_uv(m.tex[q], 0)) return true;
    }
    return false;
}

}

inline LoweredScene lower_scene(const rtr_scene_desc* s, rtr_scene_info& info) {
    LoweredScene L;
    CompiledScene& cs = L.cs = rtc::compile_validated(s, info);
    SceneFacts& f = L.facts;
    L.steps = rtc::build_steps(cs);
    L.visits = rtc::build_visits(cs, L.steps);
    f.machine_ok = !L.visits.empty();
    for (const FStep& st : L.steps) f.guarded_program |= st.kind == 3 || st.n_xf > 0 || st.n_exit > 0;
    L.prims = rtc::build_prims(s, cs);
    bool any_tie = rtc::flag_ties_within_instances(cs, L.prims);
    any_tie |= rtc::flag_ties_across_instances(cs, L.prims);
    L.leaves = rtc::build_leaf_records(cs, L.prims);
    rtc::build_scan_runs(cs, L.prims);
    for (FInst& I : cs.inst) I.shape = rtc::frame_shape(I);
    f.fast_stack_words = cs.stack_words;
    f.flat_scene = cs.ok && cs.bvh.empty() && !any_tie && cs.guard_of_ref.empty();
    f.flat_guarded = cs.ok && cs.bvh.empty() && !any_tie && !cs.guard_of_ref.empty();
    f.walk_extra_words = cs.n_compiled_subtrees ? cs.stack_words : 0;
    DScene& d = L.ds;
    std::memset(&d, 0, sizeof d);
    d.n_finst = cs.ok ? cs.subs[0].n_inst : 0;
    d.top_root0 = cs.ok ? cs.subs[0].top_root : -1;
    d.world_inst0 = cs.ok ? cs.subs[0].world_inst : -1;
    d.world_linear0 = cs.ok ? cs.subs[0].world_linear : 0;
    d.top_bound0 = cs.ok ? cs.subs[0].top_bound : 0.0f;
    d.n_fstep = (int32_t)L.steps.size();
    d.fstep_tail = cs.step_tail;
    d.n_fvisit = (int32_t)L.visits.size();
    d.camera = s->camera;
    for (int k = 0; k < 3; ++k) d.background[k] = s->background[k];
    d.root = s->root;
    d.n_nodes = s->n_nodes;
    d.n_lights = s->n_lights;
    d.needs_uv = info.needs_uv;
    d.shared_div = rtc::shared_div_allowed(s, cs);
    d.pair_cast = rtc::pair_cast_allowed(s, cs, d, f.flat_scene);
    f.top_tree = d.top_root0 >= 0, f.needs_uv = info.needs_uv != 0, f.pair_cast = d.pair_cast != 0;
    L.finish = rtc::build_finish(cs, L.prims, f.flat_scene || f.flat_guarded);
    rtc::material_facts(s, f);
    f.uv_order_dependent = rtc::uv_order_dependent(s, info);
    L.mats = rtc::build_materials(s);
    f.t_lo = std::min(0.0, std::min(s->camera.time0, s->camera.time1));
    f.t_hi = std::max(0.0, std::max(s->camera.time0, s->camera.time1));
    f.camera_times_small = std::fabs(s->camera.time0) <= 0x1p60 && std::fabs(s->camera.time1) <= 0x1p60;
    return L;
}
```

### ray_tracing-rendering_amd/csrc/rt_test_kernels.h

```cpp
#pragma once

#include "rt_kernels.h"
#include "rtr_hip_test.h"
#include "rtr_testrec.h"

template <int TRAV>
__global__ void __launch_bounds__(RTR_BLOCK) k_test_hits(const DScene sc, rtr_hit_record* recs, long long n) {
    extern __shared__ int lds_stack[];
    const Stack st{lds_stack + threadIdx.x};
    const long long k = (long long)blockIdx.x * RTR_BLOCK + threadIdx.x;
    if (k >= n) return;
    rtr_hit_record r = recs[k];
    uint32_t rng = r.rng_in;
    Hit rec;
    rec.u = rec.v = __builtin_nan("");
    rec.mat = -1;
    rec.t = 0, rec.p = mk(0, 0, 0), rec.n = mk(0, 0, 0), rec.front = false;
    Real tmax = r.t_max;
    bool h;
    if (TRAV == RT_TRAV_FAST || TRAV == RT_TRAV_TOP) {
        int ref, inst;
        h = trace_fast<false, true, false, TRAV == RT_TRAV_TOP>(sc, sub_scene0(sc), ld3(r.o), ld3(r.d), r.time, r.t_min, tmax, ref, inst, st, 0);
        if (h) fast_finish<true>(sc, ld3(r.o), ld3(r.d), r.time, tmax, ref, inst, rec);
    } else if (rt_is_program(TRAV)) {
        h = cast_closest<TRAV>(sc, ld3(r.o), ld3(r.d), r.time, rec, rng, st, r.t_min, tmax);
    } else {
        h = traverse<true, TRAV == RT_TRAV_MEDIA>(sc, sc.root, ld3(r.o), ld3(r.d), r.time, r.t_min, tmax, rec, rng, st, 0);
    }
    r.rng_out = rng;
    r.hit = h;
    r.front_face = h ? (int)rec.front : 0;
    r.material = h ? rec.mat : -1;
    r.pad = 0;
    r.t = h ? rec.t : 0;
    r.p[0] = h ? rec.p.x : 0, r.p[1] = h ? rec.p.y : 0, r.p[2] = h ? rec.p.z : 0;
    r.n[0] = h ? rec.n.x : 0, r.n[1] = h ? rec.n.y : 0, r.n[2] = h ? rec.n.z : 0;
    r.u = h ? rec.u : 0, r.v = h ? rec.v : 0;
    recs[k] = r;
}

template <int TRAV>
__global__ void __launch_bounds__(RTR_BLOCK) k_test_flat_hits(const DScene sc, rtr_hit_record* recs, long long n) {
    extern __shared__ int lds_stack[];
    const Stack st{lds_stack + threadIdx.x};
    const long long k = (long long)blockIdx.x * RTR_BLOCK + threadIdx.x;
    if (k >= n) return;
    rtr_hit_record r = recs[k];
    uint32_t rng = r.rng_in;
    Hit rec;
    rec.u = rec.v = __builtin_nan("");
    rec.mat = -1;
    rec.t = 0, rec.p = mk(0, 0, 0), rec.n = mk(0, 0, 0), rec.front = false;
    const bool h = cast_closest<TRAV>(sc, ld3(r.o), ld3(r.d), r.time, rec, rng, st, r.t_min, r.t_max);
    r.rng_out = rng;
    r.hit = h;
    r.front_face = h ? (int)rec.front : 0;
    r.material = h ? rec.mat : -1;
    r.pad = 0;
    r.t = h ? rec.t : 0;
    r.p[0] = h ? rec.p.x : 0, r.p[1] = h ? rec.p.y : 0, r.p[2] = h ? rec.p.z : 0;
    r.n[0] = h ? rec.n.x : 0, r.n[1] = h ? rec.n.y : 0, r.n[2] = h ? rec.n.z : 0;
    r.u = h ? rec.u : 0, r.v = h ? rec.v : 0;
    recs[k] = r;
}

__global__ void __launch_bounds__(RTR_BLOCK) k_test_pair(const DScene sc, rtr_pair_record* recs, long long n) {
    extern __shared__ int lds_stack[];
    const Stack st{lds_stack + threadIdx.x};
    const long long k = (long long)blockIdx.x * RTR_BLOCK + threadIdx.x;
    if (k >= n) return;
    rtr_pair_record r = recs[k];
    Real a_t = r.a_tmax, b_t = r.b_tmax;
    int a_ref, a_inst, b_ref;
    trace_pair(sc, ld3(r.ao), ld3(r.ad), 0.0, a_t, a_ref, a_inst, ld3(r.bo), ld3(r.bd), b_t, b_ref, st);
    Real s_t = r.a_tmax, sb_t = r.b_tmax;
    int s_ref, s_inst, sb_ref, sb_inst;
    trace_fast<false, false, false, false, false>(sc, sub_scene0(sc), ld3(r.ao), ld3(r.ad), 0.0, 0.001, s_t, s_ref, s_inst, st, 0);
    trace_fast<true, false, true, false, false>(sc, sub_scene0(sc), ld3(r.bo), ld3(r.bd), 0.0, 0.001, sb_t, sb_ref, sb_inst, st, 0);
    r.a_t = a_t, r.s_a_t = s_t;
    r.a_ref = a_ref, r.a_inst = a_inst, r.b_hit = b_ref >= 0;
    r.s_a_ref = s_ref, r.s_a_inst = s_inst, r.s_b_hit = sb_ref >= 0;
    recs[k] = r;
}

__global__ void __launch_bounds__(RTR_BLOCK) k_test_materials(const DScene sc, rtr_mat_record* recs, long long n) {
    const long long k = (long long)blockIdx.x * RTR_BLOCK + threadIdx.x;
    if (k >= n) return;
    rtr_mat_record r = recs[k];
    Hit rec;
    rec.p = ld3(r.p), rec.n = ld3(r.n);
    rec.u = r.u, rec.v = r.v, rec.t = 1.0;
    rec.front = r.front_face != 0;
    rec.mat = r.material;
    const V3 wo = ld3(r.wo), wi = ld3(r.wi_in);
    uint32_t rng = r.rng_in;
    BSDFSample bs;
    bs.wi = mk(0, 0, 0), bs.f = mk(0, 0, 0), bs.pdf = 0, bs.is_specular = false, bs.is_transmission = false;
    const MatCtx mc = mat_prepare(sc, rec);
    const bool ok = mat_sample(mc, rec, wo, bs, rng);
    r.rng_out = rng;
    r.sample_ok = ok, r.is_specular = bs.is_specular, r.pad = 0;
    r.is_transmission = bs.is_transmission;
    r.s_wi[0] = bs.wi.x, r.s_wi[1] = bs.wi.y, r.s_wi[2] = bs.wi.z;
    r.s_f[0] = bs.f.x, r.s_f[1] = bs.f.y, r.s_f[2] = bs.f.z;
    r.s_pdf = bs.pdf;
    const V3 e = mat_eval(mc, wo, wi);
    r.eval[0] = e.x, r.eval[1] = e.y, r.eval[2] = e.z;
    r.pdf = mat_pdf(mc, rec, wo, wi);
    const V3 em = mat_emitted(mc, rec);
    r.emitted[0] = em.x, r.emitted[1] = em.y, r.emitted[2] = em.z;
    recs[k] = r;
}

__global__ void __launch_bounds__(RTR_BLOCK) k_test_lights(const DScene sc, rtr_light_record* recs, long long n) {
    const long long k = (long long)blockIdx.x * RTR_BLOCK + threadIdx.x;
    if (k >= n) return;
    rtr_light_record r = recs[k];
    const rtr_light l = ld_const(sc.lights, r.light);
    uint32_t rng = 0x2545F491u;
    LightSample s = light_sample(l, ld3(r.p), r.u[0], r.u[1], rng, sc.image_bytes);
    r.Li[0] = s.Li.x, r.Li[1] = s.Li.y, r.Li[2] = s.Li.z;
    r.wi[0] = s.wi.x, r.wi[1] = s.wi.y, r.wi[2] = s.wi.z;
    r.pdf = s.pdf, r.dist = s.dist, r.is_delta = s.is_delta, r.pad2 = 0;
    r.pdf_dir = light_pdf(l, ld3(r.p), ld3(r.dir), sc.image_bytes);
    recs[k] = r;
}

__global__ void __launch_bounds__(RTR_BLOCK) k_test_sincos(unsigned long long* out) {
    unsigned long long bad = 0, tested = 0;
    const unsigned long long stride = (unsigned long long)gridDim.x * RTR_BLOCK;
    for (unsigned long long s = (unsigned long long)blockIdx.x * RTR_BLOCK + threadIdx.x; s < (1ull << 32); s += stride) {
        const Real phi = 2.0 * RT_PI * ((uint32_t)s * 2.3283064365386963e-10);
        Real s2, c2;
        sincos(phi, &s2, &c2);
        const Real s1 = sin(phi), c1 = cos(phi);
        bad += (__double_as_longlong(s1) != __double_as_longlong(s2)) | (__double_as_longlong(c1) != __double_as_longlong(c2));
        ++tested;
    }
    bad = wave_sum(bad);
    tested = wave_sum(tested);
    if ((threadIdx.x & 63) == 0 && bad) atomicAdd(out, bad);
    if ((threadIdx.x & 63) == 0 && tested) atomicAdd(out + 1, tested);
}

__global__ void __launch_bounds__(RTR_BLOCK) k_test_shared_div(unsigned long long* out, unsigned per_thread) {
    unsigned long long x = 0x9E3779B97F4A7C15ull * ((unsigned long long)blockIdx.x * RTR_BLOCK + threadIdx.x + 1);
    auto next = [&]() {
        x ^= x >> 12, x ^= x << 25, x ^= x >> 27;
        return x * 0x2545F4914F6CDD1Dull;
    };
    auto make = [&](int emin, int espan) {
        const unsigned long long u = next();
        const int e = emin + (int)((u >> 52) % (unsigned)espan);
        const double m = __longlong_as_double((u & 0x800FFFFFFFFFFFFFull) | 0x3FF0000000000000ull);
        return ldexp(m, e);
    };
    unsigned long long bad = 0, tested = 0;
    for (unsigned k = 0; k < per_thread; ++k) {
        double n, d;
        if (k & 3) {
            d = make(-100, 200), n = make(-300, 500);
        } else {
            const double o = (double)(long long)(next() >> 11) * 0x1p-53 * 2000.0 - 1000.0;
            const double p = (k & 4) ? o + make(-60, 60) : (double)(long long)(next() >> 11) * 0x1p-53 * 2000.0 - 1000.0;
            n = p - o;
            d = (k & 8) ? make(-40, 40) : (double)(long long)(next() >> 11) * 0x1p-52 - 1.0;
        }
        if (!rcp_safe(d)) continue;
        const double r = rcp_refined(d);
        const double t = div_shared<true>(n, d, r, false), ref = n / d;
        if (__builtin_fabs(n) >= 0x1p-300)
            bad += __double_as_longlong(t) != __double_as_longlong(ref);
        else
            bad += !(__builtin_fabs(t) < 0x1p-200) || !(__builtin_fabs(ref) < 0x1p-200);
        const double g = div_shared<true>(n, d, r, true);
        bad += __double_as_longlong(g) != __double_as_longlong(ref);
        ++tested;
    }
    bad = wave_sum(bad);
    tested = wave_sum(tested);
    if ((threadIdx.x & 63) == 0 && bad) atomicAdd(out, bad);
    if ((threadIdx.x & 63) == 0 && tested) atomicAdd(out + 1, tested);
}

#define RT_REP32(S) S S S S S S S S S S S S S S S S S S S S S S S S S S S S S S S S
template <int KIND>
__global__ void __launch_bounds__(RTR_BLOCK) k_test_issue_rate(unsigned long long* out, int iters, double seed) {
    double a = seed + threadIdx.x, b = seed * 0.5, c = 1.0 / (seed + 3.0), d = seed;
    float fa = (float)a, fb = (float)b, fc = (float)c;
    int ia = threadIdx.x, ib = 3, ic = 0;
    unsigned long long m = 0;
    const unsigned long long t0 = __builtin_readcyclecounter();
    for (int i = 0; i < iters; ++i) {
        if (KIND == 0) asm volatile(RT_REP32("v_fma_f64 %0, %1, %2, %1\n") : "+v"(d) : "v"(b), "v"(c));
        if (KIND == 1) asm volatile(RT_REP32("v_add_f64 %0, %1, %2\n") : "+v"(d) : "v"(b), "v"(c));
        if (KIND == 2) asm volatile(RT_REP32("v_mul_f64 %0, %1, %2\n") : "+v"(d) : "v"(b), "v"(c));
        if (KIND == 3) asm volatile(RT_REP32("v_rcp_f64 %0, %1\n") : "+v"(d) : "v"(b));
        if (KIND == 4) asm volatile(RT_REP32("v_rsq_f64 %0, %1\n") : "+v"(d) : "v"(b));
        if (KIND == 5) asm volatile(RT_REP32("v_cmp_lt_f64 %0, %1, %2\n") : "=s"(m) : "v"(b), "v"(c));
        if (KIND == 6) asm volatile(RT_REP32("v_cndmask_b32 %0, %1, %2, vcc\n") : "=v"(ic) : "v"(ib), "v"(ia) : "vcc");
        if (KIND == 7) asm volatile(RT_REP32("v_mov_b32 %0, %1\n") : "+v"(ia) : "v"(ib));
        if (KIND == 8) asm volatile(RT_REP32("v_fma_f32 %0, %1, %2, %1\n") : "+v"(fa) : "v"(fb), "v"(fc));
        if (KIND == 9) asm volatile(RT_REP32("s_and_b64 %0, %0, exec\n") : "+s"(m) : : "scc");
        if (KIND == 10) asm volatile(RT_REP32("v_div_scale_f64 %0, vcc, %1, %2, %1\n") : "+v"(d) : "v"(b), "v"(c) : "vcc");
        if (KIND == 11) asm volatile(RT_REP32("v_div_fixup_f64 %0, %1, %2, %1\n") : "+v"(d) : "v"(b), "v"(c));
        if (KIND == 13) asm volatile(RT_REP32("v_cndmask_b32_e64 %0, %1, %2, %3\n") : "=v"(ic) : "v"(ib), "v"(ia), "s"(m));
        if (KIND == 14) asm volatile(RT_REP32("v_min_f32 %0, %1, %2\n") : "=v"(fa) : "v"(fb), "v"(fc));
        if (KIND == 15) asm volatile(RT_REP32("v_cmp_lt_f32 vcc, %1, %2\nv_cndmask_b32 %0, %1, %2, vcc\n") : "=v"(fa) : "v"(fb), "v"(fc) : "vcc");
        if (KIND == 16) { int i0, i1, i2, i3; asm volatile(RT_REP32("v_cndmask_b32 %0, %4, %5, vcc\nv_cndmask_b32 %1, %4, %5, vcc\nv_cndmask_b32 %2, %4, %5, vcc\nv_cndmask_b32 %3, %4, %5, vcc\n") : "=v"(i0), "=v"(i1), "=v"(i2), "=v"(i3) : "v"(ib), "v"(ia) : "vcc"); ic = i0 + i1 + i2 + i3; }
        if (KIND == 17) asm volatile(RT_REP32("v_cmp_lt_f64 vcc, %1, %2\nv_cndmask_b32 %0, %3, %4, vcc\n") : "=v"(ic) : "v"(b), "v"(c), "v"(ib), "v"(ia) : "vcc");
        if (KIND == 12)
            asm volatile(RT_REP32("v_cmp_lt_f64 %0, %1, %2\ns_and_b64 %0, %0, exec\n") : "=s"(m) : "v"(b), "v"(c) : "scc");
    }
    const unsigned long long t1 = __builtin_readcyclecounter();
    if (d == 12345.678 || fa == 1.5f || ia == -77 || ic == -78 || m == 0x1234567ull) out[2] = 1;
    if ((threadIdx.x & 63) == 0) {
        atomicAdd(&out[0], t1 - t0);
        atomicAdd(&out[1], 1ull);
    }
}

__global__ void __launch_bounds__(RTR_BLOCK) k_stream8(const double* __restrict__ in, double* __restrict__ out, long long n) {
    for (long long i = (long long)blockIdx.x * RTR_BLOCK + threadIdx.x; i < n; i += (long long)gridDim.x * RTR_BLOCK)
        out[i] = in[i] + 1.0;
}
```

### ray_tracing-rendering_amd/csrc/rtr_capi.hip

```cpp
#define RTR_TU_CAPI
#include "rt_lower.h"
#include "rt_kernels.h"
#include "rt_launch.h"
#include "rt_machine.h"
#include "rt_debug.h"

#include <atomic>
#include <cstdio>
#include <cstring>
#include <functional>
#include <map>
#include <mutex>
#include <string>
#include <vector>

namespace {

thread_local std::string g_create_error;

struct DevBuf {
    void* p = nullptr;
    size_t cap = 0;
};
struct SceneBufs {
    DevBuf nodes, kids, mats, tex, perlin, images, imgbytes, lights;
    DevBuf finst, fxf, fref, fexit, fbvh, fsub, fscan, fguard, fstep, fvisit, fprim, fleaf, fmat, ffin, dscene;
    DevBuf* begin() { return &nodes; }
    DevBuf* end() { return begin() + sizeof(SceneBufs) / sizeof(DevBuf); }
};
static_assert(sizeof(SceneBufs) == 23 * sizeof(DevBuf), "SceneBufs holds DevBufs only");

}

struct rtr_context {
    int device = 0;
    hipStream_t own_stream = nullptr;
    hipStream_t stream = nullptr;
    hipStream_t side_stream = nullptr;
    std::string err;
    bool has_scene = false;
    rtr_scene_info info{};
    DScene ds{};
    SceneFacts facts;
    SceneBufs sb;
    DevBuf b_tiles, b_partial, b_done, b_stats, b_cancel, b_test, b_stage;
    DevBuf b_denoise;
    DevBuf b_query;
    DevBuf b_display;
    DevBuf b_display_io;
    std::vector<int> last_tiles;
    WavefrontPool pool;
    void* h_stage = nullptr;
    size_t h_stage_cap = 0;
    hipEvent_t ev0 = nullptr, ev1 = nullptr;
    bool stats_pending = false;
    bool in_flight = false;
    rtr_render_stats stats{};
    rtr_debug_kernel last_kernel{-1, -1, -1, -1, 0, 0, 0, 0, 0, 0, 0};
    std::atomic<uint32_t> render_seq{0};
    std::atomic<uint32_t> cancelled_upto{0};
    uint32_t pending_id = 0;
    std::mutex cancel_mu;
    int n_cus = 256;
    uint64_t scene_gen = 0;
    std::vector<rtr_accum*> accums;
    uint64_t camera_gen = 0;
    bool camera_dirty = false;
    std::vector<rtr_history*> histories;
};

struct rtr_accum {
    rtr_context* ctx = nullptr;
    rtr_render_params params{};
    uint64_t scene_gen = 0;
    uint64_t camera_gen = 0;
    std::vector<int> tiles;
    int tiles_x = 0, tiles_y = 0;
    bool moments = false;
    DevBuf d_tiles, d_sum, d_count;
    DevBuf d_q, d_qpart;
    DevBuf d_s1, d_active, d_nactive, d_err;
    mutable std::vector<int> h_counts;
    mutable bool counts_stale = false;
    DevBuf d_out;
    DevBuf d_feat;
    int feat_k = 0;
    void* h_out = nullptr;
    size_t h_out_cap = 0;
};

struct rtr_history {
    rtr_context* ctx = nullptr;
    int W = 0, H = 0, x0 = 0, y0 = 0, x1 = 0, y1 = 0;
    DevBuf d_planes[2];
    DevBuf d_mom;
    int cur = 0;
    bool have = false;
    rtr_camera cam{};
};

namespace {

int fail(rtr_context* c, int code, const std::string& msg) {
    if (c)
        c->err = msg;
    else
        g_create_error = msg;
    return code;
}

#define HIPCHK(ctx, expr)                                                                                   \
    do {                                                                                                     \
        hipError_t e_ = (expr);                                                                              \
        if (e_ != hipSuccess)                                                                                \
            return fail(ctx, RTR_ERR_DEVICE, std::string(#expr) + ": " + hipGetErrorString(e_));             \
    } while (0)

int ensure(rtr_context* c, DevBuf& b, size_t bytes) {
    if (bytes == 0) bytes = 16;
    if (b.cap >= bytes) return RTR_OK;
    if (b.p) {
        HIPCHK(c, hipFree(b.p));
        b.p = nullptr;
        b.cap = 0;
    }
    hipError_t e = hipMalloc(&b.p, bytes);
    if (e != hipSuccess) return fail(c, RTR_ERR_NOMEM, std::string("hipMalloc: ") + hipGetErrorString(e));
    b.cap = bytes;
    return RTR_OK;
}

int ensure_behind_queue(rtr_context* c, DevBuf& b, size_t bytes) {
    if (b.p && b.cap < std::max(bytes, (size_t)16)) HIPCHK(c, hipStreamSynchronize(c->stream));
    return ensure(c, b, bytes);
}

int upload(rtr_context* c, DevBuf& b, const void* src, size_t bytes) {
    int rc = ensure(c, b, bytes);
    if (rc) return rc;
    if (bytes) HIPCHK(c, hipMemcpy(b.p, src, bytes, hipMemcpyHostToDevice));
    return RTR_OK;
}
template <typename T>
int put(rtr_context* c, DevBuf& b, const T* src, size_t n, const T*& member) {
    const int rc = upload(c, b, src, sizeof(T) * n);
    member = static_cast<const T*>(b.p);
    return rc;
}
template <typename T>
int put(rtr_context* c, DevBuf& b, const std::vector<T>& src, const T*& member) {
    return put(c, b, src.data(), src.size(), member);
}

const double* display_srgb_table() {
    static const struct Table {
        double s[256];
        Table() {
            s[0] = 0.0;
            for (int b = 1; b < 256; ++b) {
                const double v = b / 255.0;
                s[b] = v <= 0.04045 ? v / 12.92 : std::pow((v + 0.055) / 1.055, 2.4);
            }
        }
    } table;
    return table.s;
}
constexpr size_t kDisplayHistOff = 256 * sizeof(double), kDisplayRecOff = kDisplayHistOff + RTR_DISPLAY_BINS * sizeof(unsigned);
constexpr size_t kDisplayBytes = kDisplayRecOff + sizeof(DisplayRec);

struct Validator {
    const rtr_scene_desc* s;
    std::string msg;
    std::vector<int> state;
    std::vector<int> need;
    std::vector<int> depth;
    std::vector<char> media;
    int code = RTR_OK;

    bool bad(int c, const std::string& m) {
        if (code == RTR_OK) {
            code = c;
            msg = m;
        }
// ... 491 lines not shown
static void free_accum(rtr_accum* a) {
    DevBuf* bufs[] = {&a->d_tiles, &a->d_sum, &a->d_count, &a->d_out, &a->d_q, &a->d_qpart, &a->d_s1, &a->d_active, &a->d_nactive, &a->d_err,
                      &a->d_feat};
    for (DevBuf* b : bufs)
        if (b->p) hipFree(b->p);
    if (a->h_out) hipHostFree(a->h_out);
    delete a;
}

static void free_history(rtr_history* h) {
    for (DevBuf* b : {&h->d_planes[0], &h->d_planes[1], &h->d_mom})
        if (b->p) hipFree(b->p);
    delete h;
}

void rtr_launch_resolve(const ResolveK& R, hipStream_t stream) {
    hipLaunchKernelGGL(k_resolve, dim3((unsigned)R.r.n_tiles), dim3(RTR_BLOCK), 0, stream, R);
}

extern "C" {

uint32_t rtr_abi_version(void) { return RTR_ABI_VERSION; }

int rtr_device_count(void) {
    int n = 0;
    hipError_t e = hipGetDeviceCount(&n);
    if (e != hipSuccess) return RTR_ERR_DEVICE;
    return n;
}

uint32_t rtr_sample_seed(uint32_t seed, int32_t image_width, int32_t i, int32_t j, int32_t s) {
    return rtr_sample_seed_inline(seed, image_width, i, j, s);
}

int rtr_validate_scene(const rtr_scene_desc* scene, rtr_scene_info* info, char* msg, size_t msg_cap) {
    Validator v;
    v.s = scene;
    int rc = v.run(info);
    if (msg && msg_cap) {
        std::snprintf(msg, msg_cap, "%s", v.msg.c_str());
    }
    if (rc == RTR_OK && info) rtc::compile_validated(scene, *info);
    return rc;
}

int rtr_create(int device_ordinal, rtr_context** out_ctx) {
    if (!out_ctx) return fail(nullptr, RTR_ERR_INVALID, "null out_ctx");
    *out_ctx = nullptr;
    int n = 0;
    hipError_t e = hipGetDeviceCount(&n);
    if (e != hipSuccess || n <= 0)
        return fail(nullptr, RTR_ERR_DEVICE,
                    std::string("no HIP device: ") + (e != hipSuccess ? hipGetErrorString(e) : "count is 0"));
    if (device_ordinal < 0 || device_ordinal >= n) return fail(nullptr, RTR_ERR_INVALID, "device ordinal out of range");
    rtr_context* c = new rtr_context();
    c->device = device_ordinal;
#define CREATE_CHK(expr)                                                                     \
    do {                                                                                     \
        hipError_t e_ = (expr);                                                              \
        if (e_ != hipSuccess) {                                                              \
            g_create_error = std::string(#expr) + ": " + hipGetErrorString(e_);              \
            delete c;                                                                        \
            return RTR_ERR_DEVICE;                                                           \
        }                                                                                    \
    } while (0)
    CREATE_CHK(hipSetDevice(device_ordinal));
    {
        hipDeviceProp_t prop;
        CREATE_CHK(hipGetDeviceProperties(&prop, device_ordinal));
        c->n_cus = prop.multiProcessorCount > 0 ? prop.multiProcessorCount : 256;
    }
    CREATE_CHK(hipStreamCreateWithFlags(&c->own_stream, hipStreamNonBlocking));
    CREATE_CHK(hipStreamCreateWithFlags(&c->side_stream, hipStreamNonBlocking));
    CREATE_CHK(hipEventCreate(&c->ev0));
    CREATE_CHK(hipEventCreate(&c->ev1));
#undef CREATE_CHK
    c->stream = c->own_stream;
    int rc = ensure(c, c->b_stats, RT_STATS_WORDS * sizeof(unsigned long long));
    if (!rc) rc = ensure(c, c->b_cancel, sizeof(uint32_t));
    if (!rc && hipMemset(c->b_cancel.p, 0, sizeof(uint32_t)) != hipSuccess) rc = RTR_ERR_DEVICE;
    if (!rc) rc = ensure(c, c->b_display, kDisplayBytes);
    if (!rc && hipMemcpy(c->b_display.p, display_srgb_table(), 256 * sizeof(double), hipMemcpyHostToDevice) != hipSuccess)
        rc = RTR_ERR_DEVICE;
    if (rc) {
        g_create_error = c->err;
        rtr_destroy(c);
        return rc;
    }
    *out_ctx = c;
    return RTR_OK;
}

void rtr_destroy(rtr_context* c) {
    if (!c) return;
    hipSetDevice(c->device);
    if (c->stream) hipStreamSynchronize(c->stream);
    for (rtr_accum* a : c->accums) free_accum(a);
    c->accums.clear();
    for (rtr_history* h : c->histories) free_history(h);
    c->histories.clear();
    for (DevBuf& b : c->sb)
        if (b.p) hipFree(b.p);
    DevBuf* bufs[] = {&c->b_tiles, &c->b_partial, &c->b_done, &c->b_stats, &c->b_cancel, &c->b_test, &c->b_stage, &c->b_denoise,
                      &c->b_query, &c->b_display, &c->b_display_io};
    for (DevBuf* b : bufs)
        if (b->p) hipFree(b->p);
    c->pool.release();
    if (c->h_stage) hipHostFree(c->h_stage);
    if (c->ev0) hipEventDestroy(c->ev0);
    if (c->ev1) hipEventDestroy(c->ev1);
    if (c->own_stream) hipStreamDestroy(c->own_stream);
    if (c->side_stream) hipStreamDestroy(c->side_stream);
    delete c;
}

int rtr_set_stream(rtr_context* c, void* hip_stream) {
    if (!c) return RTR_ERR_INVALID;
    HIPCHK(c, hipSetDevice(c->device));
    HIPCHK(c, hipStreamSynchronize(c->stream));
    c->stream = hip_stream ? reinterpret_cast<hipStream_t>(hip_stream) : c->own_stream;
    return RTR_OK;
}

int rtr_upload_scene(rtr_context* c, const rtr_scene_desc* s) {
    if (!c) return RTR_ERR_INVALID;
    Validator v;
    v.s = s;
    rtr_scene_info info{};
    int rc = v.run(&info);
    if (rc) return fail(c, rc, "scene rejected: " + v.msg);
    HIPCHK(c, hipSetDevice(c->device));
    HIPCHK(c, hipStreamSynchronize(c->stream));
    c->has_scene = false;
    ++c->scene_gen;
    const LoweredScene L = lower_scene(s, info);
    const CompiledScene& cs = L.cs;
    SceneBufs& b = c->sb;
    DScene& d = c->ds = L.ds;
    if ((rc = put(c, b.nodes, cs.dev_nodes, d.nodes))) return rc;
    if ((rc = put(c, b.kids, s->list_children, s->n_list_children, d.list_children))) return rc;
    if ((rc = put(c, b.mats, s->materials, s->n_materials, d.materials))) return rc;
    if ((rc = put(c, b.tex, s->textures, s->n_textures, d.textures))) return rc;
    if ((rc = put(c, b.perlin, s->perlin, s->n_perlin, d.perlin))) return rc;
    if ((rc = put(c, b.images, s->images, s->n_images, d.images))) return rc;
    if ((rc = put(c, b.imgbytes, s->image_bytes, s->n_image_bytes, d.image_bytes))) return rc;
    if ((rc = put(c, b.lights, s->lights, s->n_lights, d.lights))) return rc;
    if ((rc = put(c, b.finst, cs.inst, d.finst))) return rc;
    if ((rc = put(c, b.fxf, cs.xf, d.fxf))) return rc;
    if ((rc = put(c, b.fref, cs.ref, d.fref))) return rc;
    if ((rc = put(c, b.fexit, cs.exits, d.fexit))) return rc;
    if ((rc = put(c, b.fbvh, cs.bvh, d.fbvh))) return rc;
    if ((rc = put(c, b.fsub, cs.subs, d.fsub))) return rc;
    if ((rc = put(c, b.fscan, cs.scan, d.fscan))) return rc;
    if ((rc = put(c, b.fguard, cs.guards, d.fguard))) return rc;
    if ((rc = put(c, b.fstep, L.steps, d.fstep))) return rc;
    if ((rc = put(c, b.fvisit, L.visits, d.fvisit))) return rc;
    if ((rc = put(c, b.fprim, L.prims, d.fprim))) return rc;
    if ((rc = put(c, b.fleaf, L.leaves, d.fleaf))) return rc;
    if ((rc = put(c, b.fmat, L.mats, d.fmat))) return rc;
    if ((rc = put(c, b.ffin, L.finish, d.ffin))) return rc;
    if (L.finish.empty()) d.ffin = nullptr;
    if ((rc = upload(c, b.dscene, &d, sizeof(DScene)))) return rc;
    c->info = info;
    c->facts = L.facts;
    c->camera_dirty = false;
    c->has_scene = true;
    return RTR_OK;
}

static int render_core(rtr_context* c, const rtr_render_params* p, double* d_rgb, int64_t row_stride, unsigned char* tile_done,
                       int blocking, rtr_accum* acc = nullptr, const AccumPlanK* plan = nullptr);

int rtr_render_device(rtr_context* c, const rtr_render_params* p, double* d_rgb, int64_t row_stride, int blocking) {
    if (!c) return RTR_ERR_INVALID;
    if (!c->has_scene) return fail(c, RTR_ERR_NO_SCENE, "rtr_render before rtr_upload_scene");
    if (int prc = params_check(c, p)) return prc;
    if (!d_rgb || row_stride < (int64_t)(p->x1 - p->x0)) return fail(c, RTR_ERR_INVALID, "bad output buffer / stride");
    return render_core(c, p, d_rgb, row_stride, nullptr, blocking);
}

static int render_core(rtr_context* c, const rtr_render_params* p, double* d_rgb, int64_t row_stride, unsigned char* tile_done,
                       int blocking, rtr_accum* acc, const AccumPlanK* plan) {
    HIPCHK(c, hipSetDevice(c->device));
    (void)hipGetLastError();
    int rc = RTR_OK;

    RenderK P{};
    P.W = p->image_width, P.H = p->image_height;
    P.x0 = p->x0, P.y0 = p->y0, P.x1 = p->x1, P.y1 = p->y1;
    P.spp = p->spp, P.max_depth = p->max_depth, P.rr_start = p->rr_start_depth;
    P.seed = p->seed;
    P.integrator = p->integrator;
    std::vector<int> tiles;
    if (acc)
        P.tiles_x = acc->tiles_x, P.tiles_y = acc->tiles_y;
    else
        tiles = owned_tiles(*p, P.tiles_x, P.tiles_y);
    P.n_tiles = (int)(acc ? acc->tiles.size() : tiles.size());
    if (P.n_tiles == 0) {
        if ((rc = finish_stats(c))) return rc;
        c->stats = rtr_render_stats{};
        c->last_kernel = rtr_debug_kernel{-1, -1, -1, -1, 0, 0, 0, 0, 0, 0, 0};
        return RTR_OK;
    }

    int pipeline = p->pipeline;
    if (pipeline == RTR_PIPELINE_AUTO) pipeline = RTR_PIPELINE_MEGAKERNEL;
    const int trav = pick_trav(c->facts, c->info, p->flags);
    if (pipeline == RTR_PIPELINE_WAVEFRONT && (!c->facts.machine_ok || (trav != RT_TRAV_FLAT && trav != RT_TRAV_FAST && trav != RT_TRAV_PROGRAM)))
        return fail(c, RTR_ERR_UNSUPPORTED, "the wavefront pipeline runs the compiled traversals only: this graph (or "
                                            "RTR_FLAG_REFERENCE_ORDER) needs the reference-order walk of the megakernel");
    if (pipeline == RTR_PIPELINE_WAVEFRONT && (p->flags & RTR_FLAG_WF_PERSISTENT) && c->facts.guarded_program)
        return fail(c, RTR_ERR_UNSUPPORTED, "RTR_FLAG_WF_PERSISTENT: the traversal machine does not run step programs with "
                                            "guarded primitives (hollow spheres under bvh_nodes) or media under transforms; "
                                            "the lockstep stages do");
    int chunks = p->spp_chunks, guided[3] = {0, 0, 0};
    if (chunks == 0 && (rc = choose_chunks(c, P, p->integrator, pipeline, trav, p->spp, p->flags, &chunks, guided))) return rc;
    P.n_big = guided[0], P.big_spp = guided[1], P.small_spp = guided[2];
    P.chunks = chunks;

    const size_t partial_bytes = (size_t)P.n_tiles * chunks * 3 * RTR_BLOCK * sizeof(double);
    const size_t done_bytes = ((size_t)P.n_tiles * chunks + 1) * sizeof(int);
    const bool same_tiles = acc || tiles == c->last_tiles;
    if ((c->stats_pending || c->in_flight) && (!same_tiles || partial_bytes > c->b_partial.cap || done_bytes > c->b_done.cap ||
                                               pipeline == RTR_PIPELINE_WAVEFRONT)) {
        if ((rc = finish_stats(c))) return rc;
    }
    if (!same_tiles) {
        c->last_tiles.clear();
        if ((rc = upload(c, c->b_tiles, tiles.data(), tiles.size() * sizeof(int)))) return rc;
        c->last_tiles = tiles;
    }
    if ((rc = ensure(c, c->b_partial, partial_bytes))) return rc;
    if ((rc = ensure(c, c->b_done, done_bytes))) return rc;
    P.tile_ids = static_cast<const int*>(acc ? acc->d_tiles.p : c->b_tiles.p);
    if (acc) {
        P.tile_s0 = static_cast<const int*>(acc->d_count.p);
        P.acc_in = static_cast<const double*>(acc->d_sum.p);
        P.tile_s1 = static_cast<const int*>(acc->d_s1.p);
        P.active = static_cast<const int*>(acc->d_active.p);
        P.n_active = static_cast<const int*>(acc->d_nactive.p);
        if (acc->moments) {
            P.q_in = static_cast<const double*>(acc->d_q.p);
            P.q_part = static_cast<double*>(acc->d_qpart.p);
        }
    }
    P.stats = static_cast<unsigned long long*>(c->b_stats.p);
    P.cancel = static_cast<const uint32_t*>(c->b_cancel.p);
    P.partial = static_cast<double*>(c->b_partial.p);
    P.done = static_cast<int*>(c->b_done.p);
    if (pipeline == RTR_PIPELINE_MEGAKERNEL && (rc = launch_mega(c, P, p->integrator, trav, true, nullptr, p->flags))) return rc;
    const bool queue = pipeline == RTR_PIPELINE_MEGAKERNEL && mega_queue(mega_variant(c->facts, p->integrator, trav, p->flags, nullptr), P, p->flags);

    const uint32_t id = c->render_seq.fetch_add(1) + 1;
    P.render_id = id;
    c->stats_pending = false;
    c->in_flight = true;
    c->stats = rtr_render_stats{};
    c->stats.spp_chunks = chunks;
    c->last_kernel = rtr_debug_kernel{-1, -1, -1, -1, 0, 0, 0, 0, 0, 0, 0};
    LaunchedKernel launched{};
    c->pending_id = id;
    HIPCHK(c, hipMemsetAsync(c->b_stats.p, 0, RT_STATS_WORDS * sizeof(unsigned long long), c->stream));
    if (c->camera_dirty) {
        hipLaunchKernelGGL(k_camera_store, dim3(1), dim3(64), 0, c->stream, static_cast<DScene*>(c->sb.dscene.p), c->ds.camera);
        HIPCHK(c, hipGetLastError());
        c->camera_dirty = false;
    }
    HIPCHK(c, hipEventRecord(c->ev0, c->stream));
    if (pipeline == RTR_PIPELINE_WAVEFRONT) {
        int launches = 0;
        WavefrontPlan plan{};
        plan.has_lights = c->ds.n_lights > 0;
        plan.media = trav == RT_TRAV_PROGRAM;
        plan.lean = c->facts.lean_materials && !plan.media;
        plan.quadlit = c->facts.quad_lights_only && !c->info.needs_uv;
        plan.sort = !plan.lean && c->facts.n_material_types > 1;
        plan.n_cus = c->n_cus;
        plan.lds = stack_bytes(c->facts, c->info, trav);
        plan.trav = trav;
        plan.machine = (p->flags & RTR_FLAG_WF_PERSISTENT) != 0;
        if (plan.machine) c->stats.flags_in_effect |= RTR_FLAG_WF_PERSISTENT;
        rc = wavefront_render(c->pool, static_cast<const DScene*>(c->sb.dscene.p), plan, P, p->integrator, d_rgb, row_stride,
                              tile_done, c->stream, &c->cancelled_upto, &launches, &launched, c->err);
        c->last_kernel = rtr_debug_kernel{pipeline, p->integrator, launched.trav, launched.ms, launched.sorted, launched.phases,
                                          plan.lean, plan.quadlit, plan.sort, plan.media, plan.machine};
        if (rc && rc != RTR_ERR_CANCELLED) return rc;
        if (rc == RTR_ERR_CANCELLED) c->stats.cancelled = 1;
        c->stats.kernel_launches = launches;
    } else {
        int launches = 2;
        if (acc) {
            acc->counts_stale = true;
            AccumPlanK K = *plan;
            K.n_tiles = P.n_tiles;
            K.count = static_cast<const int*>(acc->d_count.p);
            K.err = static_cast<const double*>(acc->d_err.p);
            K.tile_s1 = static_cast<int*>(acc->d_s1.p);
            K.active = static_cast<int*>(acc->d_active.p);
            K.n_active = static_cast<int*>(acc->d_nactive.p);
            if (K.mode == 2) {
                hipLaunchKernelGGL(k_accum_errors, dim3((unsigned)P.n_tiles), dim3(RTR_BLOCK), 0, c->stream, accum_view(acc),
                                   static_cast<const double*>(acc->d_q.p), static_cast<double*>(acc->d_err.p));
                ++launches;
            }
            hipLaunchKernelGGL(k_accum_plan, dim3(1), dim3(1024), 0, c->stream, K);
// ... 644 lines not shown
    static thread_local uint32_t upto;
    upto = c->render_seq.load();
    if (upto == 0 || upto == c->cancelled_upto.load()) return RTR_OK;
    c->cancelled_upto.store(upto);
    hipSetDevice(c->device);
    hipError_t e = hipMemcpyAsync(c->b_cancel.p, &upto, sizeof(uint32_t), hipMemcpyHostToDevice, c->side_stream);
    if (e == hipSuccess) e = hipStreamSynchronize(c->side_stream);
    return e == hipSuccess ? RTR_OK : RTR_ERR_DEVICE;
}

int rtr_get_stats(rtr_context* c, rtr_render_stats* out) {
    if (!c || !out) return RTR_ERR_INVALID;
    HIPCHK(c, hipSetDevice(c->device));
    int rc = finish_stats(c);
    if (rc) return rc;
    *out = c->stats;
    return RTR_OK;
}

const char* rtr_last_error(const rtr_context* c) { return c ? c->err.c_str() : g_create_error.c_str(); }

static int li_run(rtr_context* c, const rtr_render_params* p, const int32_t* ijs, const rtr_li_ray* rays, LiOut* host_out,
                  int64_t n) {
    if (!c) return RTR_ERR_INVALID;
    if (!c->has_scene) return fail(c, RTR_ERR_NO_SCENE, "rtr_li_* before rtr_upload_scene");
    if (int prc = params_check(c, p)) return prc;
    if (n == 0) return RTR_OK;
    HIPCHK(c, hipSetDevice(c->device));
    HIPCHK(c, hipStreamSynchronize(c->stream));
    const size_t in_bytes = rays ? (size_t)n * sizeof(rtr_li_ray) : (size_t)n * 3 * sizeof(int32_t);
    const size_t in_pad = (in_bytes + 15) & ~(size_t)15;
    int rc = ensure(c, c->b_test, in_pad + (size_t)n * sizeof(LiOut));
    if (rc) return rc;
    char* base = static_cast<char*>(c->b_test.p);
    HIPCHK(c, hipMemcpy(base, rays ? (const void*)rays : (const void*)ijs, in_bytes, hipMemcpyHostToDevice));
    RenderK P{};
    P.W = p->image_width, P.H = p->image_height;
    P.spp = p->spp, P.max_depth = p->max_depth, P.rr_start = p->rr_start_depth;
    P.seed = p->seed;
    const int32_t* d_ijs = rays ? nullptr : reinterpret_cast<const int32_t*>(base);
    const rtr_li_ray* d_rays = rays ? reinterpret_cast<const rtr_li_ray*>(base) : nullptr;
    LiOut* d_out = reinterpret_cast<LiOut*>(base + in_pad);
    int trav = per_ray_trav(c->facts, c->info, p->flags, false);
    const size_t lds = stack_bytes(c->facts, c->info, trav);
    const dim3 grid((unsigned)((n + RTR_BLOCK - 1) / RTR_BLOCK));
    const bool n1 = p->integrator != RTR_INTEGRATOR_MIS && p->integrator != RTR_INTEGRATOR_RR;
    if (n1 && trav == RT_TRAV_EXACT) trav = RT_TRAV_MEDIA;
    auto launch = [&](auto integ, auto travs) {
        constexpr int I = decltype(integ)::value;
        return dispatch_trav(travs, trav, [&](auto t) {
            constexpr int T = decltype(t)::value;
            if ((rc = set_lds(c, k_li<I, T>, lds))) return;
            hipLaunchKernelGGL((k_li<I, T>), grid, dim3(RTR_BLOCK), lds, c->stream, c->ds, P, d_ijs, d_rays, d_out, (long long)n);
        });
    };
    using TravsN1 = TravSet<RT_TRAV_FAST, RT_TRAV_PROGRAM_EXT, RT_TRAV_MEDIA>;
    bool found;
    switch (p->integrator) {
    case RTR_INTEGRATOR_MIS: found = launch(std::integral_constant<int, RTR_INTEGRATOR_MIS>{}, PerRayTravs{}); break;
    case RTR_INTEGRATOR_RR: found = launch(std::integral_constant<int, RTR_INTEGRATOR_RR>{}, PerRayTravs{}); break;
    case RTR_INTEGRATOR_PATH: found = launch(std::integral_constant<int, RTR_INTEGRATOR_PATH>{}, TravsN1{}); break;
    case RTR_INTEGRATOR_PBR: found = launch(std::integral_constant<int, RTR_INTEGRATOR_PBR>{}, TravsN1{}); break;
    default: found = launch(std::integral_constant<int, RTR_INTEGRATOR_NEE>{}, TravsN1{}); break;
    }
    if (!found) return no_per_ray_kernel(c, trav);
    if (rc) return rc;
    HIPCHK(c, hipGetLastError());
    HIPCHK(c, hipStreamSynchronize(c->stream));
    HIPCHK(c, hipMemcpy(host_out, d_out, (size_t)n * sizeof(LiOut), hipMemcpyDeviceToHost));
    return RTR_OK;
}

int rtr_li_samples(rtr_context* c, const rtr_render_params* p, const int32_t* ijs, double* L, int64_t n) {
    if (!c) return RTR_ERR_INVALID;
    if (n < 0 || (n > 0 && (!ijs || !L))) return fail(c, RTR_ERR_INVALID, "bad sample / radiance arrays");
    if (int prc = params_check(c, p)) return prc;
    for (int64_t k = 0; k < n; ++k)
        if (ijs[3 * k] < 0 || ijs[3 * k] >= p->image_width || ijs[3 * k + 1] < 0 || ijs[3 * k + 1] >= p->image_height ||
            ijs[3 * k + 2] < 0)
            return fail(c, RTR_ERR_INVALID, "sample outside the image");
    std::vector<LiOut> out((size_t)n);
    int rc = li_run(c, p, ijs, nullptr, out.data(), n);
    if (rc) return rc;
    for (int64_t k = 0; k < n; ++k)
        for (int q = 0; q < 3; ++q) L[3 * k + q] = out[(size_t)k].L[q];
    return RTR_OK;
}

int rtr_li_rays(rtr_context* c, const rtr_render_params* p, const rtr_li_ray* rays, double* L, int64_t n) {
    if (!c) return RTR_ERR_INVALID;
    if (n < 0 || (n > 0 && (!rays || !L))) return fail(c, RTR_ERR_INVALID, "bad ray / radiance arrays");
    for (int64_t k = 0; k < n; ++k)
        if (rays[k].rng_state == 0) return fail(c, RTR_ERR_INVALID, "a xorshift32 state must not be 0 (rtweekend.h:24-34)");
    std::vector<LiOut> out((size_t)n);
    int rc = li_run(c, p, nullptr, rays, out.data(), n);
    if (rc) return rc;
    for (int64_t k = 0; k < n; ++k)
        for (int q = 0; q < 3; ++q) L[3 * k + q] = out[(size_t)k].L[q];
    return RTR_OK;
}

int rtr_debug_view_get(rtr_context* c, int flags, rtr_debug_view* v, size_t size) {
    if (!c || !v || size != sizeof(rtr_debug_view)) return RTR_ERR_INVALID;
    if (!c->has_scene) return fail(c, RTR_ERR_NO_SCENE, "rtr_test_* before rtr_upload_scene");
    v->ds = c->ds;
    v->stream = c->stream;
    v->device = c->device;
    v->n_cus = c->n_cus;
    v->n_materials = c->facts.n_materials;
    v->trav = per_ray_trav(c->facts, c->info, flags, true);
    v->stack_bytes = stack_bytes(c->facts, c->info, v->trav);
    const int picked = pick_trav(c->facts, c->info, flags);
    v->flat_trav = picked == RT_TRAV_FLAT ? RT_TRAV_FLAT
                   : (picked == RT_TRAV_FAST && c->facts.flat_guarded && !c->facts.top_tree ? RT_TRAV_FLAT_GUARD : -1);
    return RTR_OK;
}
int rtr_debug_scene_plan(const rtr_scene_desc* s, int integrator, int flags, rtr_debug_plan* out, size_t size, int32_t* ref_flags,
                         int64_t cap, void* finish, int64_t finish_cap) {
    if (!out || size != sizeof(rtr_debug_plan) || cap < 0 || (cap > 0 && !ref_flags)) return RTR_ERR_INVALID;
    if (finish_cap < 0 || (finish_cap > 0 && !finish)) return RTR_ERR_INVALID;
    Validator v;
    v.s = s;
    rtr_scene_info info{};
    if (int rc = v.run(&info)) return rc;
    const LoweredScene L = lower_scene(s, info);
    const SceneFacts& f = L.facts;
    int ties = 0, guards = 0;
    for (size_t k = 0; k < L.prims.size(); ++k) {
        ties += (L.prims[k].reserved & RT_TIE_FLAG) != 0, guards += (L.prims[k].reserved & RT_GUARD_FLAG) != 0;
        if ((int64_t)k < cap) ref_flags[k] = L.prims[k].reserved;
    }
    const int trav = pick_trav(f, info, flags);
    const MegaVariant m = mega_variant(f, integrator, trav, flags, nullptr);
    *out = rtr_debug_plan{info.fast_ok, info.has_media, f.flat_scene, f.flat_guarded, f.lean_materials, f.quad_lights_only,
                          f.uv_order_dependent, f.machine_ok, f.guarded_program, f.top_tree, f.needs_uv, f.n_material_types,
                          L.ds.shared_div, L.ds.pair_cast, (int32_t)L.steps.size(), (int32_t)L.visits.size(),
                          (int32_t)L.prims.size(), f.fast_stack_words, info.stack_words + f.walk_extra_words, ties, guards,
                          trav, m.trav, m.ms, m.sorted, m.pair, (int32_t)L.finish.size()};
    if (finish_cap > 0 && !L.finish.empty())
        std::memcpy(finish, L.finish.data(), sizeof(FFin) * (size_t)std::min<int64_t>(finish_cap, (int64_t)L.finish.size()));
    return RTR_OK;
}
int rtr_debug_frame_shapes(const rtr_scene_desc* s, int32_t* shapes, int64_t cap, int32_t* n_inst) {
    if (!n_inst || cap < 0 || (cap > 0 && !shapes)) return RTR_ERR_INVALID;
    Validator v;
    v.s = s;
    rtr_scene_info info{};
    if (int rc = v.run(&info)) return rc;
    const LoweredScene L = lower_scene(s, info);
    *n_inst = L.ds.n_finst;
    for (int k = 0; k < L.ds.n_finst && k < cap; ++k) shapes[k] = L.cs.inst[(size_t)k].shape;
    return RTR_OK;
}
int rtr_debug_last_kernel(rtr_context* c, rtr_debug_kernel* out, size_t size) {
    if (!c || !out || size != sizeof(rtr_debug_kernel)) return RTR_ERR_INVALID;
    *out = c->last_kernel;
    return RTR_OK;
}
int rtr_debug_li(rtr_context* c, const rtr_render_params* p, const int32_t* ijs, rtr_debug_li_out* out, int64_t n) {
    static_assert(sizeof(rtr_debug_li_out) == sizeof(LiOut), "one layout");
    if (n < 0 || (n > 0 && (!ijs || !out))) return RTR_ERR_INVALID;
    return li_run(c, p, ijs, nullptr, reinterpret_cast<LiOut*>(out), n);
}
void rtr_debug_set_error(rtr_context* c, const char* msg) {
    if (c) c->err = msg ? msg : "";
}

}

namespace {

constexpr int64_t kQuerySlice = (int64_t)1 << 22;

int query_check(rtr_context* c, const void* rays, const void* out, int64_t n, int32_t flags) {
    if (!c) return RTR_ERR_INVALID;
    if (flags & ~RTR_FLAG_REFERENCE_ORDER) return fail(c, RTR_ERR_INVALID, "rtr_query_*: unknown flag bits");
    if (n < 0 || (n > 0 && (!rays || !out))) return fail(c, RTR_ERR_INVALID, "rtr_query_*: negative n or NULL array");
    if (!c->has_scene) return fail(c, RTR_ERR_NO_SCENE, "rtr_query_* before rtr_upload_scene");
    return RTR_OK;
}
int query_check_rays(rtr_context* c, const rtr_ray* rays, int64_t n) {
    const bool media = c->info.has_media != 0;
    for (int64_t k = 0; k < n; ++k)
        if (rtr_ray_bad(rays[k], media))
            return fail(c, RTR_ERR_INVALID, "rtr_query_*: bad ray at index " + std::to_string(k) +
                                                " (non-finite origin / direction / time / t_min, NaN t_max, or rng_state 0 in a "
                                                "scene with media)");
    return RTR_OK;
}

bool query_staged(size_t stack) {
    const char* e = getenv("RTR_QUERY_STAGED");
    const bool want = e ? e[0] != '0' : RTR_QUERY_STAGED_DEFAULT != 0;
    return want && stack + RTR_QUERY_STAGE_BYTES <= 160 * 1024;
}

int query_launch(rtr_context* c, const rtr_ray* d_rays, rtr_ray_hit* d_hits, uint8_t* d_occ, uint32_t* d_rng, int64_t n, int flags) {
    const int trav = per_ray_trav(c->facts, c->info, flags, true);
    const size_t stack = stack_bytes(c->facts, c->info, trav);
    const bool staged = query_staged(stack);
    const size_t lds = stack + (staged ? RTR_QUERY_STAGE_BYTES : 0);
    const int stage_word = (int)(stack / sizeof(int));
    const int media = c->info.has_media != 0;
    DScene ds = c->ds;
    ds.needs_uv = 1;
    const dim3 grid((unsigned)((n + RTR_BLOCK - 1) / RTR_BLOCK));
    int rc = RTR_OK;
    auto launch = [&](auto t, auto s) {
        constexpr int T = decltype(t)::value;
        constexpr bool S = decltype(s)::value;
        if (d_hits) {
            if ((rc = set_lds(c, k_query_closest<T, S>, lds))) return;
            hipLaunchKernelGGL((k_query_closest<T, S>), grid, dim3(RTR_BLOCK), lds, c->stream, ds, d_rays, d_hits, (long long)n, media,
                               stage_word);
        } else {
            if ((rc = set_lds(c, k_query_any<T, S>, lds))) return;
            hipLaunchKernelGGL((k_query_any<T, S>), grid, dim3(RTR_BLOCK), lds, c->stream, ds, d_rays, d_occ, d_rng, (long long)n, media,
                               stage_word);
        }
    };
    if (!dispatch_trav(PerRayTravsTop{}, trav, [&](auto t) { staged ? launch(t, std::true_type{}) : launch(t, std::false_type{}); }))
        return no_per_ray_kernel(c, trav);
    if (rc) return rc;
    HIPCHK(c, hipGetLastError());
    return RTR_OK;
}

int query_host(rtr_context* c, const rtr_ray* rays, rtr_ray_hit* hits, uint8_t* occ, uint32_t* rng_out, int64_t n, int flags) {
    HIPCHK(c, hipSetDevice(c->device));
    (void)hipGetLastError();
    const int64_t slice = std::min(n, kQuerySlice);
    const size_t in_bytes = (size_t)slice * sizeof(rtr_ray);
    const size_t out_bytes = hits ? (size_t)slice * sizeof(rtr_ray_hit) : (size_t)slice * sizeof(uint32_t);
    const size_t occ_bytes = hits ? 0 : (((size_t)slice + 15) & ~(size_t)15);
    if (int rc = ensure(c, c->b_query, in_bytes + out_bytes + occ_bytes)) return rc;
    char* base = static_cast<char*>(c->b_query.p);
    rtr_ray* d_rays = reinterpret_cast<rtr_ray*>(base);
    rtr_ray_hit* d_hits = hits ? reinterpret_cast<rtr_ray_hit*>(base + in_bytes) : nullptr;
    uint32_t* d_rng = hits ? nullptr : reinterpret_cast<uint32_t*>(base + in_bytes);
    uint8_t* d_occ = hits ? nullptr : reinterpret_cast<uint8_t*>(base + in_bytes + out_bytes);
    for (int64_t k0 = 0; k0 < n; k0 += slice) {
        const int64_t m = std::min(slice, n - k0);
        HIPCHK(c, hipMemcpyAsync(d_rays, rays + k0, (size_t)m * sizeof(rtr_ray), hipMemcpyHostToDevice, c->stream));
        if (int rc = query_launch(c, d_rays, d_hits, d_occ, d_rng, m, flags)) return rc;
        if (hits) {
            HIPCHK(c, hipMemcpyAsync(hits + k0, d_hits, (size_t)m * sizeof(rtr_ray_hit), hipMemcpyDeviceToHost, c->stream));
        } else {
            HIPCHK(c, hipMemcpyAsync(occ + k0, d_occ, (size_t)m, hipMemcpyDeviceToHost, c->stream));
            if (rng_out) HIPCHK(c, hipMemcpyAsync(rng_out + k0, d_rng, (size_t)m * sizeof(uint32_t), hipMemcpyDeviceToHost, c->stream));
        }
        HIPCHK(c, hipStreamSynchronize(c->stream));
    }
    return RTR_OK;
}

int query_device(rtr_context* c, const rtr_ray* d_rays, rtr_ray_hit* d_hits, uint8_t* d_occ, uint32_t* d_rng, int64_t n, int flags,
                 int blocking) {
    HIPCHK(c, hipSetDevice(c->device));
    (void)hipGetLastError();
    if (int rc = query_launch(c, d_rays, d_hits, d_occ, d_rng, n, flags)) return rc;
    if (blocking) HIPCHK(c, hipStreamSynchronize(c->stream));
    return RTR_OK;
}

}

extern "C" {

int rtr_query_closest(rtr_context* c, const rtr_ray* rays, rtr_ray_hit* hits, int64_t n, int32_t flags) {
    if (int rc = query_check(c, rays, hits, n, flags)) return rc;
    if (n == 0) return RTR_OK;
    if (int rc = query_check_rays(c, rays, n)) return rc;
    return query_host(c, rays, hits, nullptr, nullptr, n, flags);
}

int rtr_query_occluded(rtr_context* c, const rtr_ray* rays, uint8_t* occluded, uint32_t* rng_out, int64_t n, int32_t flags) {
    if (int rc = query_check(c, rays, occluded, n, flags)) return rc;
    if (n == 0) return RTR_OK;
    if (int rc = query_check_rays(c, rays, n)) return rc;
    return query_host(c, rays, nullptr, occluded, rng_out, n, flags);
}

int rtr_query_closest_device(rtr_context* c, const rtr_ray* d_rays, rtr_ray_hit* d_hits, int64_t n, int32_t flags, int blocking) {
    if (int rc = query_check(c, d_rays, d_hits, n, flags)) return rc;
    if (n == 0) return RTR_OK;
    return query_device(c, d_rays, d_hits, nullptr, nullptr, n, flags, blocking);
}

int rtr_query_occluded_device(rtr_context* c, const rtr_ray* d_rays, uint8_t* d_occluded, uint32_t* d_rng_out, int64_t n,
                              int32_t flags, int blocking) {
    if (int rc = query_check(c, d_rays, d_occluded, n, flags)) return rc;
    if (n == 0) return RTR_OK;
    return query_device(c, d_rays, nullptr, d_occluded, d_rng_out, n, flags, blocking);
}

}

extern "C" {

int rtr_set_camera(rtr_context* c, const rtr_camera* cam) {
    if (!c) return RTR_ERR_INVALID;
    if (!cam) return fail(c, RTR_ERR_INVALID, "null camera");
    if (!c->has_scene) return fail(c, RTR_ERR_NO_SCENE, "rtr_set_camera before rtr_upload_scene");
    static_assert(sizeof(rtr_camera) == 24 * sizeof(double), "rtr_camera is 24 doubles");
    double v[24];
    std::memcpy(v, cam, sizeof v);
// ... 272 lines not shown
```

### ray_tracing-rendering_amd/native.py

```python
import ctypes as C
import os
import weakref

import numpy as np

from . import _abi as A
from .scene import Scene

_HERE = os.path.dirname(os.path.abspath(__file__))
_LIB = None

_STATUS = {A.RTR_ERR_INVALID: "RTR_ERR_INVALID", A.RTR_ERR_UNSUPPORTED: "RTR_ERR_UNSUPPORTED",
           A.RTR_ERR_DEVICE: "RTR_ERR_DEVICE", A.RTR_ERR_NO_SCENE: "RTR_ERR_NO_SCENE",
           A.RTR_ERR_CANCELLED: "RTR_ERR_CANCELLED", A.RTR_ERR_NOMEM: "RTR_ERR_NOMEM"}

EXPORTS = ("rtr_abi_version", "rtr_device_count", "rtr_create", "rtr_destroy", "rtr_set_stream",
           "rtr_upload_scene", "rtr_render_device", "rtr_render_host", "rtr_render_tiles_host", "rtr_plan_chunks", "rtr_li_samples", "rtr_li_rays",
           "rtr_synchronize", "rtr_cancel", "rtr_get_stats", "rtr_last_error", "rtr_sample_seed", "rtr_validate_scene",
           "rtr_accum_create", "rtr_accum_render", "rtr_accum_resolve", "rtr_accum_tiles", "rtr_accum_destroy",
           "rtr_accum_create_ex", "rtr_accum_render_tiles", "rtr_accum_moments", "rtr_accum_errors", "rtr_accum_refine",
           "rtr_denoise_defaults", "rtr_accum_features", "rtr_accum_denoise", "rtr_denoise_host",
           "rtr_query_closest", "rtr_query_occluded", "rtr_query_closest_device", "rtr_query_occluded_device",
           "rtr_set_camera", "rtr_get_camera", "rtr_accum_reset", "rtr_temporal_defaults", "rtr_history_create",
           "rtr_history_clear", "rtr_history_destroy", "rtr_history_planes", "rtr_accum_denoise_temporal",
           "rtr_display_defaults", "rtr_display_srgb_thresholds", "rtr_display_histogram", "rtr_display_host",
           "rtr_display_device", "rtr_accum_resolve_device", "rtr_accum_features_device", "rtr_accum_denoise_device",
           "rtr_accum_denoise_temporal_device")
TEST_EXPORTS = ("rtr_test_hits", "rtr_test_materials", "rtr_test_lights", "rtr_test_li", "rtr_test_reference_order",
                "rtr_test_stream8", "rtr_test_sincos_exhaustive", "rtr_test_shared_division", "rtr_test_issue_rates", "rtr_test_last_kernel",
                "rtr_test_temporal_planes", "rtr_test_scene_plan", "rtr_test_flat_hits", "rtr_test_pair_frames",
                "rtr_test_pair_frame_host", "rtr_test_pair_cast", "rtr_test_queue_blocks_host", "rtr_test_queue_pack_host")
_TEST_LIB = None


class SceneInfoC(C.Structure):
    _fields_ = [("stack_words", C.c_int32), ("has_media", C.c_int32), ("needs_uv", C.c_int32),
                ("graph_depth", C.c_int32), ("fast_ok", C.c_int32), ("fast_instances", C.c_int32),
                ("fast_refs", C.c_int32), ("fast_stack_words", C.c_int32), ("compiled_subtrees", C.c_int32),
                ("program_steps", C.c_int32), ("inverted_boxes", C.c_int32), ("top_trees", C.c_int32)]


class KernelRecordC(C.Structure):
    _fields_ = [(name, C.c_int32) for name in ("pipeline", "integrator", "trav", "ms", "sorted", "shade_phases", "lean",
                                               "quadlit", "sort", "media", "machine", "accum")]


class ScenePlanC(C.Structure):
    _fields_ = [(name, C.c_int32) for name in (
        "fast_ok", "has_media", "flat_scene", "flat_guarded", "lean_materials", "quad_lights_only", "uv_order_dependent",
        "machine_ok", "guarded_program", "top_tree", "needs_uv", "n_material_types", "shared_div", "pair_cast", "n_steps",
        "n_visits", "n_refs", "fast_stack_words", "walk_stack_words", "n_tie_refs", "n_guard_refs", "pick_trav", "mega_trav",
        "mega_ms", "mega_sorted", "mega_pair", "n_finish")]


FINISH_DTYPE = np.dtype([("kind", "<i4"), ("material", "<i4"), ("levels", "<i4"), ("flip", "<i4"), ("op", "<f8", (2, 3)),
                         ("g", "<f8", (4,))])


PAIR_FRAME_DTYPE = np.dtype([("ao", "<f8", (3,)), ("ad", "<f8", (3,)), ("bo", "<f8", (3,)), ("bd", "<f8", (3,)),
                             ("fo", "<f8", (3,)), ("fd", "<f8", (3,)), ("same_frame", "<i4"), ("pad", "<i4")])
PAIR_DTYPE = np.dtype([("ao", "<f8", (3,)), ("ad", "<f8", (3,)), ("a_tmax", "<f8"), ("bo", "<f8", (3,)), ("bd", "<f8", (3,)),
                       ("b_tmax", "<f8"), ("a_t", "<f8"), ("s_a_t", "<f8"), ("a_ref", "<i4"), ("a_inst", "<i4"),
                       ("b_hit", "<i4"), ("s_a_ref", "<i4"), ("s_a_inst", "<i4"), ("s_b_hit", "<i4")])
QUEUE_BLOCK_DTYPE = np.dtype([(name, "<i4") for name in ("slot", "quarter", "chunk", "s0", "s1", "ref_s0", "ref_s1", "pad")])
FRAME_SHAPES = ("none", "T", "R", "TR", "RT", "other")


class RtrError(RuntimeError):
    def __init__(self, code, message):
        super().__init__("%s (%d): %s" % (_STATUS.get(code, "rtr_status"), code, message))
        self.code = code
        self.message = message


def library_path():
    return os.environ.get("RTR_HIP_LIBRARY") or os.path.join(_HERE, "librtr_hip.so")


def lib():
    global _LIB
    if _LIB is not None:
        return _LIB
    path = library_path()
    if not os.path.exists(path):
        raise RtrError(A.RTR_ERR_DEVICE, "HIP library %s is missing: run __graft_entry__.build(); there is no "
                       "CPU fallback" % path)
    L = C.CDLL(path)
    P = C.POINTER
    vp = C.c_void_p
    L.rtr_abi_version.restype = C.c_uint32
    L.rtr_device_count.restype = C.c_int
    L.rtr_create.argtypes = [C.c_int, P(vp)]
    L.rtr_destroy.argtypes = [vp]
    L.rtr_destroy.restype = None
    L.rtr_set_stream.argtypes = [vp, vp]
    L.rtr_upload_scene.argtypes = [vp, P(A.SceneDescC)]
    L.rtr_render_device.argtypes = [vp, P(A.RenderParamsC), vp, C.c_int64, C.c_int]
    L.rtr_render_host.argtypes = [vp, P(A.RenderParamsC), vp, C.c_int64]
    L.rtr_plan_chunks.argtypes = [vp, P(A.RenderParamsC)]
    L.rtr_li_samples.argtypes = [vp, P(A.RenderParamsC), vp, vp, C.c_int64]
    L.rtr_synchronize.argtypes = [vp]
    L.rtr_cancel.argtypes = [vp]
    L.rtr_get_stats.argtypes = [vp, P(A.RenderStatsC)]
    L.rtr_last_error.argtypes = [vp]
    L.rtr_last_error.restype = C.c_char_p
    L.rtr_sample_seed.argtypes = [C.c_uint32, C.c_int32, C.c_int32, C.c_int32, C.c_int32]
    L.rtr_sample_seed.restype = C.c_uint32
    L.rtr_validate_scene.argtypes = [P(A.SceneDescC), P(SceneInfoC), C.c_char_p, C.c_size_t]
    L.rtr_li_rays.argtypes = [vp, P(A.RenderParamsC), vp, vp, C.c_int64]
    L.rtr_accum_create.argtypes = [vp, P(A.RenderParamsC), P(vp)]
    L.rtr_accum_render.argtypes = [vp, vp, C.c_int32, C.c_int]
    L.rtr_accum_resolve.argtypes = [vp, vp, vp, C.c_int64, vp]
    L.rtr_accum_tiles.argtypes = [vp, vp, vp, vp, C.c_int64, P(C.c_int64)]
    L.rtr_accum_destroy.argtypes = [vp]
    L.rtr_accum_destroy.restype = None
    L.rtr_accum_create_ex.argtypes = [vp, P(A.RenderParamsC), C.c_uint32, P(vp)]
    L.rtr_accum_render_tiles.argtypes = [vp, vp, vp, C.c_int64, C.c_int]
    L.rtr_accum_moments.argtypes = [vp, vp, vp, C.c_int64]
    L.rtr_accum_errors.argtypes = [vp, vp, vp, C.c_int64, P(C.c_int64)]
    L.rtr_accum_refine.argtypes = [vp, vp, C.c_double, C.c_int32, C.c_int32, C.c_int, P(C.c_int32)]
    L.rtr_denoise_defaults.argtypes = [P(A.DenoiseParamsC)]
    L.rtr_denoise_defaults.restype = None
    L.rtr_accum_features.argtypes = [vp, vp, C.c_int32, vp, C.c_int64]
    L.rtr_accum_denoise.argtypes = [vp, vp, P(A.DenoiseParamsC), vp, C.c_int64, vp]
    L.rtr_denoise_host.argtypes = [vp, P(A.DenoiseParamsC), C.c_int32, C.c_int32, vp, vp, vp, vp, vp, vp]
    L.rtr_query_closest.argtypes = [vp, vp, vp, C.c_int64, C.c_int32]
    L.rtr_query_occluded.argtypes = [vp, vp, vp, vp, C.c_int64, C.c_int32]
    L.rtr_query_closest_device.argtypes = [vp, vp, vp, C.c_int64, C.c_int32, C.c_int]
    L.rtr_query_occluded_device.argtypes = [vp, vp, vp, vp, C.c_int64, C.c_int32, C.c_int]
    L.rtr_set_camera.argtypes = [vp, P(A.CameraC)]
    L.rtr_get_camera.argtypes = [vp, P(A.CameraC)]
    L.rtr_accum_reset.argtypes = [vp, vp, C.c_uint32]
    L.rtr_temporal_defaults.argtypes = [P(A.TemporalParamsC)]
    L.rtr_temporal_defaults.restype = None
    L.rtr_history_create.argtypes = [vp, P(A.RenderParamsC), P(vp)]
    L.rtr_history_clear.argtypes = [vp, vp]
    L.rtr_history_destroy.argtypes = [vp]
    L.rtr_history_destroy.restype = None
    L.rtr_history_planes.argtypes = [vp, vp, vp, C.c_int64]
    L.rtr_accum_denoise_temporal.argtypes = [vp, vp, vp, P(A.DenoiseParamsC), P(A.TemporalParamsC), vp, C.c_int64, vp]
    L.rtr_display_defaults.argtypes = [P(A.DisplayParamsC)]
    L.rtr_display_defaults.restype = None
    L.rtr_display_srgb_thresholds.argtypes = [vp]
    L.rtr_display_srgb_thresholds.restype = None
    L.rtr_display_histogram.argtypes = [vp, C.c_int32, C.c_int32, vp, C.c_int64, vp, P(C.c_int64)]
    L.rtr_display_host.argtypes = [vp, P(A.DisplayParamsC), C.c_int32, C.c_int32, vp, C.c_int64, vp, vp, P(A.DisplayResultC)]
    L.rtr_display_device.argtypes = [vp, P(A.DisplayParamsC), C.c_int32, C.c_int32, vp, C.c_int64, vp, vp,
                                     P(A.DisplayResultC), C.c_int]
    for name, argtypes in A.DEVICE_OUTPUT_SIGNATURES.items():
        getattr(L, name).argtypes = argtypes
    if L.rtr_abi_version() != A.RTR_ABI_VERSION:
        raise RtrError(A.RTR_ERR_INVALID, "librtr_hip.so ABI version mismatch")
    _LIB = L
    return L


def test_lib():
    global _TEST_LIB
    if _TEST_LIB is not None:
        return _TEST_LIB
    lib()
    path = os.environ.get("RTR_HIP_TEST_LIBRARY") or os.path.join(os.path.dirname(library_path()), "librtr_hip_test.so")
    if not os.path.exists(path):
        path = os.path.join(_HERE, "librtr_hip_test.so")
    if not os.path.exists(path):
        raise RtrError(A.RTR_ERR_DEVICE, "test library %s is missing: run __graft_entry__.build()" % path)
    T = C.CDLL(path, mode=C.RTLD_GLOBAL)
    vp = C.c_void_p
    for name in ("rtr_test_hits", "rtr_test_materials", "rtr_test_lights"):
        getattr(T, name).argtypes = [vp, vp, C.c_int64]
    T.rtr_test_li.argtypes = [vp, C.POINTER(A.RenderParamsC), vp, C.c_int64]
    T.rtr_test_reference_order.argtypes = [vp, C.c_int]
    T.rtr_test_stream8.argtypes = [vp, C.c_int64, C.c_int]
    T.rtr_test_sincos_exhaustive.argtypes = [vp, C.POINTER(C.c_uint64), C.POINTER(C.c_uint64)]
    T.rtr_test_issue_rates.argtypes = [vp, C.POINTER(C.c_double), C.c_int]
    T.rtr_test_shared_division.argtypes = [vp, C.POINTER(C.c_uint64), C.POINTER(C.c_uint64)]
    T.rtr_test_last_kernel.argtypes = [vp, C.POINTER(KernelRecordC), C.c_size_t]
    T.rtr_test_temporal_planes.argtypes = [vp] + [C.c_int32] * 6 + [C.POINTER(A.CameraC), C.POINTER(A.CameraC), C.c_int,
                                                                    C.POINTER(A.TemporalParamsC)] + [vp] * 8
    T.rtr_test_scene_plan.argtypes = [C.POINTER(A.SceneDescC), C.c_int32, C.c_int32, C.POINTER(ScenePlanC), vp, C.c_int64,
                                      vp, C.c_int64]
    T.rtr_test_flat_hits.argtypes = [vp, vp, C.c_int64, C.c_int, C.POINTER(C.c_int32)]
    T.rtr_test_pair_frames.argtypes = [C.POINTER(A.SceneDescC), vp, C.c_int64, C.POINTER(C.c_int32)]
    T.rtr_test_pair_frame_host.argtypes = [C.c_int32, vp, vp, C.c_int64]
    T.rtr_test_pair_cast.argtypes = [vp, vp, C.c_int64]
    T.rtr_test_queue_blocks_host.argtypes = [C.c_int32] * 6 + [vp, C.c_int64]
    T.rtr_test_queue_pack_host.argtypes = [C.c_int32] * 3 + [C.POINTER(C.c_uint32), C.POINTER(C.c_uint32), vp]
    _TEST_LIB = T
    return T


def validate_scene(scene):
    L = lib()
    d = scene.desc()
    info = SceneInfoC()
    msg = C.create_string_buffer(256)
    rc = L.rtr_validate_scene(C.byref(d), C.byref(info), msg, len(msg))
    if rc != 0:
        raise RtrError(rc, msg.value.decode())
    return {"stack_words": info.stack_words, "has_media": bool(info.has_media), "needs_uv": bool(info.needs_uv),
            "graph_depth": info.graph_depth, "fast_ok": bool(info.fast_ok), "fast_instances": info.fast_instances,
            "fast_refs": info.fast_refs, "fast_stack_words": info.fast_stack_words,
            "compiled_subtrees": info.compiled_subtrees, "program_steps": info.program_steps,
            "inverted_boxes": info.inverted_boxes, "top_trees": info.top_trees}


def scene_plan(scene, integrator=4, flags=0):
    T = test_lib()
    d = scene.desc()
    plan = ScenePlanC()
    rc = T.rtr_test_scene_plan(C.byref(d), int(integrator), int(flags), C.byref(plan), None, 0, None, 0)
    if rc != 0:
        raise RtrError(rc, "scene rejected")
    ref_flags = np.zeros(plan.n_refs, dtype=np.int32)
    finish = np.zeros(plan.n_finish, dtype=FINISH_DTYPE)
    T.rtr_test_scene_plan(C.byref(d), int(integrator), int(flags), C.byref(plan), ref_flags.ctypes.data, len(ref_flags),
                          finish.ctypes.data, len(finish))
    out = {name: int(getattr(plan, name)) for name, _ in ScenePlanC._fields_}
    out["ref_flags"] = ref_flags
    out["finish"] = finish
    return out


def pair_frames(scene):
    T = test_lib()
    d = scene.desc()
    n = C.c_int32(0)
    rc = T.rtr_test_pair_frames(C.byref(d), None, 0, C.byref(n))
    if rc != 0:
        raise RtrError(rc, "scene rejected")
    shapes = np.zeros(n.value, dtype=np.int32)
    T.rtr_test_pair_frames(C.byref(d), shapes.ctypes.data, len(shapes), C.byref(n))
    return [FRAME_SHAPES[k] for k in shapes]


def pair_frame_host(shape, ops, ao, ad, bo, bd):
    recs = np.zeros(len(ao), dtype=PAIR_FRAME_DTYPE)
    recs["ao"], recs["ad"], recs["bo"], recs["bd"] = ao, ad, bo, bd
    ops = np.ascontiguousarray(ops, dtype=np.float64).reshape(6)
    rc = test_lib().rtr_test_pair_frame_host(FRAME_SHAPES.index(shape), ops.ctypes.data, recs.ctypes.data, len(recs))
    if rc != 0:
        raise RtrError(rc, "rtr_test_pair_frame_host")
    return recs


def queue_blocks_host(n_tiles, spp, chunks, guided=(0, 0, 0)):
    recs = np.zeros(n_tiles * chunks * 4, dtype=QUEUE_BLOCK_DTYPE)
    rc = test_lib().rtr_test_queue_blocks_host(n_tiles, spp, chunks, *[int(g) for g in guided], recs.ctypes.data, len(recs))
    if rc != 0:
        raise RtrError(rc, "rtr_test_queue_blocks_host")
    return recs


def queue_pack_host(i, j, s_end):
    lo, hi = C.c_uint32(0), C.c_uint32(0)
    out = np.zeros(3, dtype=np.int32)
    rc = test_lib().rtr_test_queue_pack_host(int(i), int(j), int(s_end), C.byref(lo), C.byref(hi), out.ctypes.data)
    if rc != 0:
        raise RtrError(rc, "rtr_test_queue_pack_host")
    return (lo.value, hi.value), tuple(int(v) for v in out)


def denoise_defaults(**overrides):
    p = A.DenoiseParamsC()
    lib().rtr_denoise_defaults(C.byref(p))
    for k, v in overrides.items():
        if k not in ("iterations", "feature_spp", "sigma_l", "sigma_n", "sigma_a", "sigma_z"):
            raise TypeError("no denoise parameter %r" % k)
        setattr(p, k, v)
    return p


def temporal_defaults(**overrides):
    p = A.TemporalParamsC()
    lib().rtr_temporal_defaults(C.byref(p))
    for k, v in overrides.items():
        if k not in ("alpha_min", "tau_z", "tau_n", "min_weight"):
            raise TypeError("no temporal parameter %r" % k)
        setattr(p, k, v)
    return p


def display_defaults(**overrides):
    p = A.DisplayParamsC()
    lib().rtr_display_defaults(C.byref(p))
    for k, v in overrides.items():
        if k not in ("auto_exposure", "meter_permille", "tone_curve", "encoding", "exposure", "key", "white"):
            raise TypeError("no display parameter %r" % k)
        setattr(p, k, v)
    return p


def srgb_thresholds():
    out = np.zeros(256, dtype=np.float64)
    lib().rtr_display_srgb_thresholds(out.ctypes.data)
    return out


def _display_result(r):
    return {"scale": r.scale, "metered": r.metered, "n_metered": int(r.n_metered)}


def camera_struct(cam):
    if isinstance(cam, A.CameraC):
        return cam
    if isinstance(cam, np.ndarray):
        rec = np.ascontiguousarray(cam, dtype=A.CAMERA_DTYPE).reshape(-1)
        if len(rec) != 1:
            raise ValueError("one camera record expected")
        return A.CameraC.from_buffer_copy(rec.tobytes())
    out = A.CameraC()
    for name, ctype in A.CameraC._fields_:
        v = np.asarray(cam[name], dtype=np.float64).reshape(-1)
        setattr(out, name, float(v[0]) if ctype is C.c_double else ctype(*v))
    return out


def denoise_host(ctx, color, q, count, feat, params=None, rgb8=False, out=None):
    color = np.ascontiguousarray(color, dtype=np.float64)
    h, w = color.shape[:2]
    q = np.ascontiguousarray(q, dtype=np.float64)
    count = np.ascontiguousarray(count, dtype=np.int32)
    feat = np.ascontiguousarray(feat, dtype=np.float64)
    if color.shape != (h, w, 3) or q.shape != (h, w) or count.shape != (h, w) or feat.shape != (h, w, A.FEATURES):
        raise ValueError("planes of shapes (H, W, 3), (H, W), (H, W), (H, W, 7) expected")
    dtype = np.uint8 if rgb8 else np.float64
    if out is None:
        out = np.zeros((h, w, 3), dtype=dtype)
    elif out.shape != (h, w, 3) or out.dtype != dtype or not out.flags.c_contiguous:
        raise ValueError("out must be a C-contiguous %s array of shape (%d, %d, 3)" % (np.dtype(dtype).name, h, w))
    prm = params if params is not None else denoise_defaults()
    ctx._chk(ctx._L.rtr_denoise_host(ctx._h, C.byref(prm), w, h, color.ctypes.data, q.ctypes.data, count.ctypes.data,
                                     feat.ctypes.data, None if rgb8 else out.ctypes.data, out.ctypes.data if rgb8 else None))
    return out


class Context:

    def __init__(self, device=0):
        self._L = lib()
        h = C.c_void_p()
        rc = self._L.rtr_create(int(device), C.byref(h))
        if rc != 0:
            raise RtrError(rc, self._L.rtr_last_error(None).decode())
        self._h = h
        self.device = int(device)
        self.scene = None
        self.camera_updated = False
        self._accums = weakref.WeakSet()

    def close(self):
        if getattr(self, "_h", None):
            for a in list(self._accums):
                a._h = None
            self._L.rtr_destroy(self._h)
            self._h = None

    def __enter__(self):
        return self

    def __exit__(self, *exc):
        self.close()

    def __del__(self):
        try:
            self.close()
        except Exception:
            pass

    def _chk(self, rc):
        if rc != 0:
            raise RtrError(rc, self._L.rtr_last_error(self._h).decode())

    def set_stream(self, stream_handle):
        self._chk(self._L.rtr_set_stream(self._h, C.c_void_p(stream_handle or None)))

    def upload(self, scene):
        if not isinstance(scene, Scene):
            raise TypeError("expected a flattened Scene")
        d = scene.desc()
        self._chk(self._L.rtr_upload_scene(self._h, C.byref(d)))
        self.scene = scene
        self.camera_updated = False

    def set_camera(self, cam):
        c = camera_struct(cam)
# ... 429 lines not shown
```

Baseline: 5739.

## Compile pair-cast traversal into a flat opcode program interpreted on device

Replaces the per-instance FInst load and run-bitfield decode in trace_pair with a host-built linear program of fixed-size records (frame, rect pairs, box, sphere runs, end), fetched in 12-word chunks from constant memory. Each instance's frame transform becomes a program op, and the fast/plain intersection choice is made per frame through a wave-uniform selector, with sphere reciprocal setup optionally deferred. The aim is to cut scalar load and branch overhead in the paired-ray closest-hit loop. In exchange it adds a new device buffer, a larger branch tree held together with asm barriers, and possible over-fetch past the end of the program.

```diff
diff --git a/ray_tracing-rendering_amd/csrc/rt_compile.h b/ray_tracing-rendering_amd/csrc/rt_compile.h
--- a/ray_tracing-rendering_amd/csrc/rt_compile.h
+++ b/ray_tracing-rendering_amd/csrc/rt_compile.h
@@ -20,6 +20,7 @@
     std::vector<int32_t> exits;
     std::vector<FBvh> bvh;
     std::vector<double> scan;
+    std::vector<unsigned long long> pair;
     std::vector<FStep> steps;
     std::vector<FGuard> guards;
     std::map<int, std::pair<int, int>> guard_of_ref;
diff --git a/ray_tracing-rendering_amd/csrc/rt_debug.h b/ray_tracing-rendering_amd/csrc/rt_debug.h
--- a/ray_tracing-rendering_amd/csrc/rt_debug.h
+++ b/ray_tracing-rendering_amd/csrc/rt_debug.h
@@ -37,6 +37,7 @@
 int rtr_debug_scene_plan(const rtr_scene_desc* scene, int integrator, int flags, rtr_debug_plan* out, size_t size_of_out,
                          int32_t* ref_flags, int64_t cap, void* finish, int64_t finish_cap);
 int rtr_debug_frame_shapes(const rtr_scene_desc* scene, int32_t* shapes, int64_t cap, int32_t* n_inst);
+int rtr_debug_pair_program(const rtr_scene_desc* scene, unsigned long long* words, int64_t cap, int64_t* n_words);
 int rtr_debug_view_get(rtr_context* ctx, int flags, rtr_debug_view* view, size_t size_of_view);
 int rtr_debug_last_kernel(rtr_context* ctx, rtr_debug_kernel* out, size_t size_of_out);
 int rtr_debug_li(rtr_context* ctx, const rtr_render_params* params, const int32_t* ijs, rtr_debug_li_out* out, int64_t n);
diff --git a/ray_tracing-rendering_amd/csrc/rt_device.h b/ray_tracing-rendering_amd/csrc/rt_device.h
--- a/ray_tracing-rendering_amd/csrc/rt_device.h
+++ b/ray_tracing-rendering_amd/csrc/rt_device.h
@@ -248,6 +248,7 @@
     int32_t n_fvisit;
     const struct FVisit* fvisit;
     const struct FFin* ffin;
+    const unsigned long long* fpair;
 };
 
 struct FInst {
@@ -1264,57 +1265,28 @@
     RayDiv q;
 };
 template <int TYPE>
-RT_DEV void pair_rects(const RT_CONST_AS double* p, int cnt, int ref, const PairRay& A, Real& tmaxA, int& hitA, const PairRay& B,
-                       Real& tmaxB, int& hitB) {
-    int k = 0;
-    for (; k + 1 < cnt; k += 2, p += 10) {
-        const Real f0 = p[0], f1 = p[1], f2 = p[2], f3 = p[3], f4 = p[4];
-        const Real g0 = p[5], g1 = p[6], g2 = p[7], g3 = p[8], g4 = p[9];
-        pair_rect<TYPE>(f0, f1, f2, f3, f4, ref + k, A.o, A.d, A.q, tmaxA, hitA, B.o, B.d, B.q, tmaxB, hitB);
-        pair_rect<TYPE>(g0, g1, g2, g3, g4, ref + k + 1, A.o, A.d, A.q, tmaxA, hitA, B.o, B.d, B.q, tmaxB, hitB);
-    }
-    if (k < cnt) pair_rect<TYPE>(p[0], p[1], p[2], p[3], p[4], ref + k, A.o, A.d, A.q, tmaxA, hitA, B.o, B.d, B.q, tmaxB, hitB);
-}
-RT_DEV void pair_runs(const DScene& sc, const FInst& I, const PairRay& A, Real time, Real& tmaxA, int& hitA, const PairRay& B,
-                      Real& tmaxB, int& hitB) {
-    const RT_CONST_AS double* p = as_const(sc.fscan) + I.scan_first;
-    int ref = I.ref_first;
-#pragma nounroll
-    for (uint64_t runs = I.runs; runs != 0; runs >>= RT_RUN_BITS) {
-        const int type = RTR_NODE_SPHERE + (int)((runs >> RT_RUN_COUNT_BITS) & 7), cnt = (int)(runs & RT_RUN_COUNT_MAX);
-        RT_REGION(type >= RTR_NODE_XY_RECT ? RG_PAIR_RUNS : RG_PAIR_SPHERES);
-        if (type == RTR_NODE_XY_RECT) {
-            pair_rects<RTR_NODE_XY_RECT>(p, cnt, ref, A, tmaxA, hitA, B, tmaxB, hitB);
-            p += 5 * cnt;
-        } else if (type == RTR_NODE_XZ_RECT) {
-            pair_rects<RTR_NODE_XZ_RECT>(p, cnt, ref, A, tmaxA, hitA, B, tmaxB, hitB);
-            p += 5 * cnt;
-        } else if (type == RTR_NODE_YZ_RECT) {
-            pair_rects<RTR_NODE_YZ_RECT>(p, cnt, ref, A, tmaxA, hitA, B, tmaxB, hitB);
-            p += 5 * cnt;
-        } else if (type == RTR_NODE_SPHERE + RT_RUN_BOX) {
-            for (int b = 0, r = ref; b < cnt; ++b, p += 6, r += 6) {
-                const Real x0 = p[0], x1 = p[1], y0 = p[2], y1 = p[3], z0 = p[4], z1 = p[5];
-                pair_rect<RTR_NODE_XY_RECT>(x0, x1, y0, y1, z1, r, A.o, A.d, A.q, tmaxA, hitA, B.o, B.d, B.q, tmaxB, hitB);
-                pair_rect<RTR_NODE_XY_RECT>(x0, x1, y0, y1, z0, r + 1, A.o, A.d, A.q, tmaxA, hitA, B.o, B.d, B.q, tmaxB, hitB);
-                pair_rect<RTR_NODE_XZ_RECT>(x0, x1, z0, z1, y1, r + 2, A.o, A.d, A.q, tmaxA, hitA, B.o, B.d, B.q, tmaxB, hitB);
-                pair_rect<RTR_NODE_XZ_RECT>(x0, x1, z0, z1, y0, r + 3, A.o, A.d, A.q, tmaxA, hitA, B.o, B.d, B.q, tmaxB, hitB);
-                pair_rect<RTR_NODE_YZ_RECT>(y0, y1, z0, z1, x1, r + 4, A.o, A.d, A.q, tmaxA, hitA, B.o, B.d, B.q, tmaxB, hitB);
-                pair_rect<RTR_NODE_YZ_RECT>(y0, y1, z0, z1, x0, r + 5, A.o, A.d, A.q, tmaxA, hitA, B.o, B.d, B.q, tmaxB, hitB);
-            }
-            ref += 5 * cnt;
-        } else {
-            for (int k = 0; k < cnt; ++k, p += 4) {
-                const V3 c = mk(p[0], p[1], p[2]);
-                const Real r = p[3];
-                Real t;
-                if (sphere_hit_t<true>(c, r, A.o, A.d, A.q, 0.001, tmaxA, t)) tmaxA = t, hitA = ref + k;
-                if (sphere_hit_t<true>(c, r, B.o, B.d, B.q, 0.001, tmaxB, t)) tmaxB = t, hitB = ref + k;
-            }
-        }
-        ref += cnt;
-    }
-}
+RT_DEV void pair_rect_plain(Real a0, Real a1, Real b0, Real b1, Real k, int ref, const PairRay& A, Real& tmaxA, int& hitA,
+                            const PairRay& B, Real& tmaxB, int& hitB) {
+    run_rect_test<TYPE, false, false>(a0, a1, b0, b1, k, ref, A.o, A.d, A.q, 0.001, tmaxA, hitA);
+    run_rect_test<TYPE, false, false>(a0, a1, b0, b1, k, ref, B.o, B.d, B.q, 0.001, tmaxB, hitB);
+}
+template <int TYPE, bool FAST>
+RT_DEV void pair_rect_any(Real a0, Real a1, Real b0, Real b1, Real k, int ref, const PairRay& A, Real& tmaxA, int& hitA,
+                          const PairRay& B, Real& tmaxB, int& hitB) {
+    if (FAST)
+        pair_rect<TYPE>(a0, a1, b0, b1, k, ref, A.o, A.d, A.q, tmaxA, hitA, B.o, B.d, B.q, tmaxB, hitB);
+    else
+        pair_rect_plain<TYPE>(a0, a1, b0, b1, k, ref, A, tmaxA, hitA, B, tmaxB, hitB);
+}
+#define RT_PAIR_END 0
+#define RT_PAIR_FRAME 1
+#define RT_PAIR_RECT_XY 2
+#define RT_PAIR_RECT_XZ 3
+#define RT_PAIR_RECT_YZ 4
+#define RT_PAIR_BOX 5
+#define RT_PAIR_SPHERES 6
+#define RT_PAIR_PLAIN 8
+#define RT_PAIR_FETCH_WORDS 12
 struct PairFrame {
     V3 ao, bo;
     Real adx, adz, bdx, bdz;
@@ -1361,67 +1333,153 @@
     }
     return F;
 }
-__device__ __forceinline__ void trace_pair(const DScene& sc, V3 ao, V3 ad, Real atime, Real& a_tmax, int& a_ref, int& a_inst,
-                                           V3 bo, V3 bd, Real& b_tmax, int& b_ref, const Stack st) {
+template <bool SPH_FRAME>
+__device__ __forceinline__ void trace_pair(const DScene& sc, V3 ao, V3 ad, Real& a_tmax, int& a_ref, int& a_inst, V3 bo, V3 bd,
+                                           Real& b_tmax, int& b_ref) {
     a_ref = -1, a_inst = -1, b_ref = -1;
 #ifndef RTR_NO_SHARED_DIV
-    const bool ok_a = raydiv_origin_ok(ao), ok_b = raydiv_origin_ok(bo);
+    const bool origin_ok = raydiv_origin_ok(ao) & raydiv_origin_ok(bo);
 #else
-    const bool ok_a = false, ok_b = false;
+    const bool origin_ok = false;
 #endif
     const Real way = rcp_refined(ad.y), wby = rcp_refined(bd.y);
     const bool wa_y = rcp_safe(ad.y), wb_y = rcp_safe(bd.y);
-    for (int ii = 0; ii < sc.n_finst; ++ii) {
-        RT_REGION(RG_PAIR_SETUP);
-        const FInst I = ld_const(sc.finst, ii);
-        PairRay A, B;
-        if (I.shape != RT_SHAPE_OTHER) {
-            const PairFrame F = pair_frame(I.shape, I.xf_f[0], I.xf_f[1], ao, ad, bo, bd);
-            A.o = F.ao, B.o = F.bo;
-            A.d = mk(F.adx, ad.y, F.adz), B.d = mk(F.bdx, bd.y, F.bdz);
-        } else {
-            A.o = ao, A.d = ad, B.o = bo, B.d = bd;
-            wrapper_enter(I.xf_type[0], I.xf_f[0], A.o, A.d);
-            wrapper_enter(I.xf_type[0], I.xf_f[0], B.o, B.d);
-            if (I.n_xf > 1) {
-                wrapper_enter(I.xf_type[1], I.xf_f[1], A.o, A.d);
-                wrapper_enter(I.xf_type[1], I.xf_f[1], B.o, B.d);
+    PairRay A, B;
+    A.q.guard = B.q.guard = false;
+    A.q.fast = B.q.fast = false;
+    A.q.ry = way, B.q.ry = wby;
+    A.q.a = A.q.ra = B.q.a = B.q.ra = 0;
+    int plain = RT_PAIR_PLAIN;
+    int inst = -1, ref_first = 0;
+    const RT_CONST_AS unsigned long long* p = as_const(sc.fpair);
+#define RT_PAIR_NEXT(v) asm volatile("" : "+s"(v))
+#define RT_W(k) __longlong_as_double((long long)w[(k) + 2])
+#define RT_PAIR_RECTS(TYPE, FAST)                                                                                           \
+    do {                                                                                                                    \
+        RT_REGION(RG_PAIR_RUNS);                                                                                            \
+        pair_rect_any<TYPE, FAST>(RT_W(0), RT_W(1), RT_W(2), RT_W(3), RT_W(4), ref, A, a_tmax, a_ref, B, b_tmax, b_ref);     \
+        if (cnt > 1)                                                                                                        \
+            pair_rect_any<TYPE, FAST>(RT_W(5), RT_W(6), RT_W(7), RT_W(8), RT_W(9), ref + 1, A, a_tmax, a_ref, B, b_tmax, b_ref); \
+    } while (0)
+#define RT_PAIR_BOX_SIDES(FAST)                                                  \
+    do {                                                                                                                    \
+        RT_REGION(RG_PAIR_RUNS);                                                                  \
+        const Real x0 = RT_W(0), x1 = RT_W(1), y0 = RT_W(2), y1 = RT_W(3), z0 = RT_W(4), z1 = RT_W(5);                       \
+        pair_rect_any<RTR_NODE_XY_RECT, FAST>(x0, x1, y0, y1, z1, ref, A, a_tmax, a_ref, B, b_tmax, b_ref);                  \
+        pair_rect_any<RTR_NODE_XY_RECT, FAST>(x0, x1, y0, y1, z0, ref + 1, A, a_tmax, a_ref, B, b_tmax, b_ref);              \
+        pair_rect_any<RTR_NODE_XZ_RECT, FAST>(x0, x1, z0, z1, y1, ref + 2, A, a_tmax, a_ref, B, b_tmax, b_ref);              \
+        pair_rect_any<RTR_NODE_XZ_RECT, FAST>(x0, x1, z0, z1, y0, ref + 3, A, a_tmax, a_ref, B, b_tmax, b_ref);              \
+        pair_rect_any<RTR_NODE_YZ_RECT, FAST>(y0, y1, z0, z1, x1, ref + 4, A, a_tmax, a_ref, B, b_tmax, b_ref);              \
+        pair_rect_any<RTR_NODE_YZ_RECT, FAST>(y0, y1, z0, z1, x0, ref + 5, A, a_tmax, a_ref, B, b_tmax, b_ref);              \
+    } while (0)
+#define RT_PAIR_SPHERE_RUN(FAST)                             \
+    do {                                                                                                                    \
+        RT_REGION(RG_PAIR_SPHERES);                                                                                         \
+        RayDiv qa = A.q, qb = B.q;                                                                                          \
+        if (FAST && !SPH_FRAME) {                                   \
+            qa.a = len2(A.d), qb.a = len2(B.d);                                                                             \
+            qa.ra = rcp_refined(qa.a), qb.ra = rcp_refined(qb.a);                                                           \
+        }                                                                                                                   \
+        for (int k = 0; k < cnt; ++k) {                                                                                     \
+            const V3 c = mk(body[4 * k], body[4 * k + 1], body[4 * k + 2]);                                                 \
+            const Real r = body[4 * k + 3];                                                                                 \
+            Real t;                                                                                                         \
+            if (sphere_hit_t<FAST>(c, r, A.o, A.d, qa, 0.001, a_tmax, t)) a_tmax = t, a_ref = ref + k;                        \
+            if (sphere_hit_t<FAST>(c, r, B.o, B.d, qb, 0.001, b_tmax, t)) b_tmax = t, b_ref = ref + k;                        \
+        }                                                                                                                   \
+    } while (0)
+    for (;;) {
+        unsigned long long w[RT_PAIR_FETCH_WORDS];
+#pragma unroll
+        for (int k = 0; k < RT_PAIR_FETCH_WORDS; ++k) w[k] = p[k];
+        const int kind = (int)(w[0] & 0xffffffffu), size = (int)(w[0] >> 32);
+        const int ref = (int)(w[1] & 0xffffffffu), cnt = (int)(w[1] >> 32);
+        const RT_CONST_AS double* body = (const RT_CONST_AS double*)(p + 2);
+        p += 4 * size;
+        if (kind == RT_PAIR_END) break;
+        int sel = kind == RT_PAIR_FRAME ? kind : (kind | plain);
+        if (sel <= RT_PAIR_BOX) {
+            RT_PAIR_NEXT(sel);
+            if (sel >= RT_PAIR_RECT_YZ) {
+                RT_PAIR_NEXT(sel);
+                if (sel == RT_PAIR_RECT_YZ) RT_PAIR_RECTS(RTR_NODE_YZ_RECT, true);
+                RT_PAIR_NEXT(sel);
+                if (sel == RT_PAIR_BOX) RT_PAIR_BOX_SIDES(true);
             }
-            for (int k = RT_INST_XF_INLINE; k < I.n_xf; ++k) {
-                const FXf x = ld_const(sc.fxf, I.xf_first + k);
-                wrapper_enter(x.type, x.f, A.o, A.d);
-                wrapper_enter(x.type, x.f, B.o, B.d);
+            RT_PAIR_NEXT(sel);
+            if (sel <= RT_PAIR_RECT_XZ) {
+                RT_PAIR_NEXT(sel);
+                if (sel == RT_PAIR_RECT_XY) RT_PAIR_RECTS(RTR_NODE_XY_RECT, true);
+                RT_PAIR_NEXT(sel);
+                if (sel == RT_PAIR_RECT_XZ) RT_PAIR_RECTS(RTR_NODE_XZ_RECT, true);
+                RT_PAIR_NEXT(sel);
+                if (sel == RT_PAIR_FRAME) {
+                    RT_REGION(RG_PAIR_SETUP);
+                    if (a_ref >= ref_first) a_inst = inst;
+                    inst = cnt, ref_first = ref;
+                    int shape = (int)(w[2] & 0xffffffffu);
+                    const int flags = (int)(w[2] >> 32);
+                    const double f0[3] = {RT_W(2), RT_W(3), RT_W(4)}, f1[3] = {RT_W(5), RT_W(6), RT_W(7)};
+                    A.d.y = ad.y, B.d.y = bd.y;
+#define RT_PAIR_SHAPE(SHAPE)                                                           \
+        if (shape == SHAPE) {                                                                                                   \
+            double g0[3] = {f0[0], f0[1], f0[2]}, g1[3] = {f1[0], f1[1], f1[2]};                                                \
+            asm volatile("" : "+s"(g0[0]), "+s"(g0[1]), "+s"(g0[2]), "+s"(g1[0]), "+s"(g1[1]), "+s"(g1[2]));                    \
+            const PairFrame F = pair_frame(SHAPE, g0, g1, ao, ad, bo, bd);                                                      \
+            A.o = F.ao, B.o = F.bo;                                                                                             \
+            A.d.x = F.adx, A.d.z = F.adz, B.d.x = F.bdx, B.d.z = F.bdz;                                                         \
+        }                                                                                                                       \
+        RT_PAIR_NEXT(shape)
+                    RT_PAIR_SHAPE(RT_SHAPE_NONE);
+                    RT_PAIR_SHAPE(RT_SHAPE_TR);
+                    RT_PAIR_SHAPE(RT_SHAPE_T);
+                    RT_PAIR_SHAPE(RT_SHAPE_R);
+                    RT_PAIR_SHAPE(RT_SHAPE_RT);
+#undef RT_PAIR_SHAPE
+                    if (shape == RT_SHAPE_OTHER) {
+                        const int xf_first = (int)(w[3] & 0xffffffffu), n_xf = (int)(w[3] >> 32);
+                        A.o = ao, A.d = ad, B.o = bo, B.d = bd;
+                        for (int k = 0; k < n_xf; ++k) {
+                            const FXf x = ld_const(sc.fxf, xf_first + k);
+                            wrapper_enter(x.type, x.f, A.o, A.d);
+                            wrapper_enter(x.type, x.f, B.o, B.d);
+                        }
+                    }
+                    A.q.rx = rcp_refined(A.d.x), A.q.rz = rcp_refined(A.d.z);
+                    B.q.rx = rcp_refined(B.d.x), B.q.rz = rcp_refined(B.d.z);
+                    bool sa = rcp_safe(A.d.x) & rcp_safe(A.d.z) & wa_y, sb = rcp_safe(B.d.x) & rcp_safe(B.d.z) & wb_y;
+                    if (flags & RT_INST_SPHERES) {
+                        const Real la = len2(A.d), lb = len2(B.d);
+                        sa = sa & rcp_safe(la), sb = sb & rcp_safe(lb);
+                        if (SPH_FRAME) A.q.a = la, B.q.a = lb, A.q.ra = rcp_refined(la), B.q.ra = rcp_refined(lb);
+                    }
+                    plain = origin_ok && __all(sa & sb) ? 0 : RT_PAIR_PLAIN;
+                }
             }
         }
-        A.q.guard = B.q.guard = false;
-        A.q.rx = rcp_refined(A.d.x), A.q.rz = rcp_refined(A.d.z);
-        B.q.rx = rcp_refined(B.d.x), B.q.rz = rcp_refined(B.d.z);
-        A.q.ry = way, B.q.ry = wby;
-        bool sa = rcp_safe(A.d.x) & rcp_safe(A.d.z) & wa_y, sb = rcp_safe(B.d.x) & rcp_safe(B.d.z) & wb_y;
-        A.q.a = A.q.ra = B.q.a = B.q.ra = 0;
-        if (I.flags & RT_INST_SPHERES) {
-            A.q.a = len2(A.d), B.q.a = len2(B.d);
-            A.q.ra = rcp_refined(A.q.a), B.q.ra = rcp_refined(B.q.a);
-            sa = sa & rcp_safe(A.q.a), sb = sb & rcp_safe(B.q.a);
-        }
-        if (ok_a && ok_b && __all(sa & sb)) {
-            A.q.fast = B.q.fast = true;
-            pair_runs(sc, I, A, atime, a_tmax, a_ref, B, b_tmax, b_ref);
-        } else {
-            A.q.fast = ok_a && __all(sa), B.q.fast = ok_b && __all(sb);
-            int order = -1;
-            if (A.q.fast)
-                scan_instance<false, false, false, true>(sc, I, A.o, A.d, A.q, atime, 0.001, a_tmax, a_ref, order, st, 0);
-            else
-                scan_instance<false, false, false, false>(sc, I, A.o, A.d, A.q, atime, 0.001, a_tmax, a_ref, order, st, 0);
-            if (B.q.fast)
-                scan_instance<true, false, true, true>(sc, I, B.o, B.d, B.q, 0.0, 0.001, b_tmax, b_ref, order, st, 0);
-            else
-                scan_instance<true, false, true, false>(sc, I, B.o, B.d, B.q, 0.0, 0.001, b_tmax, b_ref, order, st, 0);
-        }
-        RT_REGION(RG_PAIR_SETUP);
-        if (a_ref >= I.ref_first) a_inst = ii;
-    }
+        RT_PAIR_NEXT(sel);
+        if (sel > RT_PAIR_BOX) {
+            RT_PAIR_NEXT(sel);
+            if (sel == RT_PAIR_SPHERES) RT_PAIR_SPHERE_RUN(true);
+            RT_PAIR_NEXT(sel);
+            if (sel == (RT_PAIR_RECT_XY | RT_PAIR_PLAIN)) RT_PAIR_RECTS(RTR_NODE_XY_RECT, false);
+            RT_PAIR_NEXT(sel);
+            if (sel == (RT_PAIR_RECT_XZ | RT_PAIR_PLAIN)) RT_PAIR_RECTS(RTR_NODE_XZ_RECT, false);
+            RT_PAIR_NEXT(sel);
+            if (sel == (RT_PAIR_RECT_YZ | RT_PAIR_PLAIN)) RT_PAIR_RECTS(RTR_NODE_YZ_RECT, false);
+            RT_PAIR_NEXT(sel);
+            if (sel == (RT_PAIR_BOX | RT_PAIR_PLAIN)) RT_PAIR_BOX_SIDES(false);
+            RT_PAIR_NEXT(sel);
+            if (sel == (RT_PAIR_SPHERES | RT_PAIR_PLAIN)) RT_PAIR_SPHERE_RUN(false);
+        }
+    }
+#undef RT_PAIR_RECTS
+#undef RT_PAIR_BOX_SIDES
+#undef RT_PAIR_SPHERE_RUN
+#undef RT_PAIR_NEXT
+#undef RT_W
+    RT_REGION(RG_PAIR_SETUP);
+    if (a_ref >= ref_first) a_inst = inst;
 }
 
 template <bool UV>
diff --git a/ray_tracing-rendering_amd/csrc/rt_kernels.h b/ray_tracing-rendering_amd/csrc/rt_kernels.h
--- a/ray_tracing-rendering_amd/csrc/rt_kernels.h
+++ b/ray_tracing-rendering_amd/csrc/rt_kernels.h
@@ -363,7 +363,7 @@
             } else {
                 so = mk(0.0, 0.0, 0.0);
             }
-            trace_pair(sc, ps.ro, ps.rd, ps.tm, a_tmax, a_ref, a_inst, so, swi, b_tmax, b_ref, st);
+            trace_pair<MS != RT_MS_LEAN>(sc, ps.ro, ps.rd, a_tmax, a_ref, a_inst, so, swi, b_tmax, b_ref);
             RTR_CLK(closest);
             RT_REGION(RG_POLL);
             const uint32_t cancel_word = cancel_poll_issue(P, it++);
@@ -675,7 +675,7 @@
         } else {
             so = mk(0.0, 0.0, 0.0);
         }
-        trace_pair(sc, ps.ro, ps.rd, ps.tm, a_tmax, a_ref, a_inst, so, swi, b_tmax, b_ref, st);
+        trace_pair<MS != RT_MS_LEAN>(sc, ps.ro, ps.rd, a_tmax, a_ref, a_inst, so, swi, b_tmax, b_ref);
         RTR_CLK(closest);
         RT_REGION(RG_POLL);
         const uint32_t cancel_word = cancel_poll_issue(P, it++);
diff --git a/ray_tracing-rendering_amd/csrc/rt_lower.h b/ray_tracing-rendering_amd/csrc/rt_lower.h
--- a/ray_tracing-rendering_amd/csrc/rt_lower.h
+++ b/ray_tracing-rendering_amd/csrc/rt_lower.h
@@ -356,6 +356,48 @@
     return true;
 }
 
+inline std::vector<unsigned long long> build_pair_program(const CompiledScene& cs, const DScene& d) {
+    std::vector<unsigned long long> out;
+    if (!d.pair_cast) return out;
+    typedef unsigned long long u64;
+    auto two = [](int lo, int hi) { return (u64)(uint32_t)lo | (u64)(uint32_t)hi << 32; };
+    auto op = [&](int kind, int words, int ref, int cnt) {
+        const size_t at = out.size();
+        const int size = (2 + words + 3) / 4;
+        out.resize(at + 4 * (size_t)size, 0);
+        out[at] = two(kind, size), out[at + 1] = two(ref, cnt);
+        return at + 2;
+    };
+    auto put = [&](size_t at, const double* f, int n) { std::memcpy(&out[at], f, 8 * (size_t)n); };
+    for (int ii = 0; ii < d.n_finst; ++ii) {
+        const FInst& I = cs.inst[(size_t)ii];
+        const size_t at = op(RT_PAIR_FRAME, 8, I.ref_first, ii);
+        out[at] = two(I.shape, I.flags), out[at + 1] = two(I.xf_first, I.n_xf);
+        put(at + 2, I.xf_f[0], 3), put(at + 5, I.xf_f[1], 3);
+        const double* p = cs.scan.data() + I.scan_first;
+        int ref = I.ref_first;
+        for (uint64_t runs = I.runs; runs != 0; runs >>= RT_RUN_BITS) {
+            const int type = RTR_NODE_SPHERE + (int)((runs >> RT_RUN_COUNT_BITS) & 7), cnt = (int)(runs & RT_RUN_COUNT_MAX);
+            if (type == RTR_NODE_SPHERE + RT_RUN_BOX) {
+                for (int b = 0; b < cnt; ++b, p += 6, ref += 6) put(op(RT_PAIR_BOX, 6, ref, 1), p, 6);
+            } else if (type == RTR_NODE_SPHERE) {
+                put(op(RT_PAIR_SPHERES, 4 * cnt, ref, cnt), p, 4 * cnt);
+                p += 4 * cnt, ref += cnt;
+            } else {
+                const int kind = type == RTR_NODE_XY_RECT ? RT_PAIR_RECT_XY : (type == RTR_NODE_XZ_RECT ? RT_PAIR_RECT_XZ : RT_PAIR_RECT_YZ);
+                for (int k = 0; k < cnt; k += 2) {
+                    const int n = std::min(2, cnt - k);
+                    put(op(kind, 5 * n, ref + k, n), p + 5 * k, 5 * n);
+                }
+                p += 5 * cnt, ref += cnt;
+            }
+        }
+    }
+    op(RT_PAIR_END, 0, 0, 0);
+    out.resize(out.size() + RT_PAIR_FETCH_WORDS - 4, 0);
+    return out;
+}
+
 inline std::vector<FFin> build_finish(const CompiledScene& cs, const std::vector<rtr_node>& prims, bool flat) {
     std::vector<FFin> out;
     if (!flat || !cs.ok || cs.subs.empty()) return out;
@@ -467,6 +509,7 @@
     d.needs_uv = info.needs_uv;
     d.shared_div = rtc::shared_div_allowed(s, cs);
     d.pair_cast = rtc::pair_cast_allowed(s, cs, d, f.flat_scene);
+    cs.pair = rtc::build_pair_program(cs, d);
     f.top_tree = d.top_root0 >= 0, f.needs_uv = info.needs_uv != 0, f.pair_cast = d.pair_cast != 0;
     L.finish = rtc::build_finish(cs, L.prims, f.flat_scene || f.flat_guarded);
     rtc::material_facts(s, f);
diff --git a/ray_tracing-rendering_amd/csrc/rt_test_kernels.h b/ray_tracing-rendering_amd/csrc/rt_test_kernels.h
--- a/ray_tracing-rendering_amd/csrc/rt_test_kernels.h
+++ b/ray_tracing-rendering_amd/csrc/rt_test_kernels.h
@@ -72,7 +72,15 @@
     rtr_pair_record r = recs[k];
     Real a_t = r.a_tmax, b_t = r.b_tmax;
     int a_ref, a_inst, b_ref;
-    trace_pair(sc, ld3(r.ao), ld3(r.ad), 0.0, a_t, a_ref, a_inst, ld3(r.bo), ld3(r.bd), b_t, b_ref, st);
+    trace_pair<false>(sc, ld3(r.ao), ld3(r.ad), a_t, a_ref, a_inst, ld3(r.bo), ld3(r.bd), b_t, b_ref);
+    {
+        Real f_a_t = r.a_tmax, f_b_t = r.b_tmax;
+        int f_a_ref, f_a_inst, f_b_ref;
+        trace_pair<true>(sc, ld3(r.ao), ld3(r.ad), f_a_t, f_a_ref, f_a_inst, ld3(r.bo), ld3(r.bd), f_b_t, f_b_ref);
+        if (__double_as_longlong(f_a_t) != __double_as_longlong(a_t) || f_a_ref != a_ref || f_a_inst != a_inst ||
+            (f_b_ref >= 0) != (b_ref >= 0))
+            a_inst = -2;
+    }
     Real s_t = r.a_tmax, sb_t = r.b_tmax;
     int s_ref, s_inst, sb_ref, sb_inst;
     trace_fast<false, false, false, false, false>(sc, sub_scene0(sc), ld3(r.ao), ld3(r.ad), 0.0, 0.001, s_t, s_ref, s_inst, st, 0);
diff --git a/ray_tracing-rendering_amd/csrc/rtr_capi.hip b/ray_tracing-rendering_amd/csrc/rtr_capi.hip
--- a/ray_tracing-rendering_amd/csrc/rtr_capi.hip
+++ b/ray_tracing-rendering_amd/csrc/rtr_capi.hip
@@ -24,11 +24,11 @@
 };
 struct SceneBufs {
     DevBuf nodes, kids, mats, tex, perlin, images, imgbytes, lights;
-    DevBuf finst, fxf, fref, fexit, fbvh, fsub, fscan, fguard, fstep, fvisit, fprim, fleaf, fmat, ffin, dscene;
+    DevBuf finst, fxf, fref, fexit, fbvh, fsub, fscan, fpair, fguard, fstep, fvisit, fprim, fleaf, fmat, ffin, dscene;
     DevBuf* begin() { return &nodes; }
     DevBuf* end() { return begin() + sizeof(SceneBufs) / sizeof(DevBuf); }
 };
-static_assert(sizeof(SceneBufs) == 23 * sizeof(DevBuf), "SceneBufs holds DevBufs only");
+static_assert(sizeof(SceneBufs) == 24 * sizeof(DevBuf), "SceneBufs holds DevBufs only");
 
 }
 
@@ -826,6 +826,7 @@
     if ((rc = put(c, b.fbvh, cs.bvh, d.fbvh))) return rc;
     if ((rc = put(c, b.fsub, cs.subs, d.fsub))) return rc;
     if ((rc = put(c, b.fscan, cs.scan, d.fscan))) return rc;
+    if ((rc = put(c, b.fpair, cs.pair, d.fpair))) return rc;
     if ((rc = put(c, b.fguard, cs.guards, d.fguard))) return rc;
     if ((rc = put(c, b.fstep, L.steps, d.fstep))) return rc;
     if ((rc = put(c, b.fvisit, L.visits, d.fvisit))) return rc;
@@ -1776,6 +1777,17 @@
     for (int k = 0; k < L.ds.n_finst && k < cap; ++k) shapes[k] = L.cs.inst[(size_t)k].shape;
     return RTR_OK;
 }
+int rtr_debug_pair_program(const rtr_scene_desc* s, unsigned long long* words, int64_t cap, int64_t* n_words) {
+    if (!n_words || cap < 0 || (cap > 0 && !words)) return RTR_ERR_INVALID;
+    Validator v;
+    v.s = s;
+    rtr_scene_info info{};
+    if (int rc = v.run(&info)) return rc;
+    const LoweredScene L = lower_scene(s, info);
+    *n_words = (int64_t)L.cs.pair.size();
+    if (cap > 0 && !L.cs.pair.empty()) std::memcpy(words, L.cs.pair.data(), 8 * (size_t)std::min<int64_t>(cap, *n_words));
+    return RTR_OK;
+}
 int rtr_debug_last_kernel(rtr_context* c, rtr_debug_kernel* out, size_t size) {
     if (!c || !out || size != sizeof(rtr_debug_kernel)) return RTR_ERR_INVALID;
     *out = c->last_kernel;
diff --git a/ray_tracing-rendering_amd/native.py b/ray_tracing-rendering_amd/native.py
--- a/ray_tracing-rendering_amd/native.py
+++ b/ray_tracing-rendering_amd/native.py
@@ -29,7 +29,8 @@
 TEST_EXPORTS = ("rtr_test_hits", "rtr_test_materials", "rtr_test_lights", "rtr_test_li", "rtr_test_reference_order",
                 "rtr_test_stream8", "rtr_test_sincos_exhaustive", "rtr_test_shared_division", "rtr_test_issue_rates", "rtr_test_last_kernel",
                 "rtr_test_temporal_planes", "rtr_test_scene_plan", "rtr_test_flat_hits", "rtr_test_pair_frames",
-                "rtr_test_pair_frame_host", "rtr_test_pair_cast", "rtr_test_queue_blocks_host", "rtr_test_queue_pack_host")
+                "rtr_test_pair_frame_host", "rtr_test_pair_cast", "rtr_test_queue_blocks_host", "rtr_test_queue_pack_host",
+                "rtr_test_pair_program")
 _TEST_LIB = None
 
 
@@ -183,6 +184,8 @@
     T.rtr_test_flat_hits.argtypes = [vp, vp, C.c_int64, C.c_int, C.POINTER(C.c_int32)]
     T.rtr_test_pair_frames.argtypes = [C.POINTER(A.SceneDescC), vp, C.c_int64, C.POINTER(C.c_int32)]
     T.rtr_test_pair_frame_host.argtypes = [C.c_int32, vp, vp, C.c_int64]
+    if hasattr(T, "rtr_test_pair_program"):
+        T.rtr_test_pair_program.argtypes = [C.POINTER(A.SceneDescC), vp, C.c_int64, C.POINTER(C.c_int64)]
     T.rtr_test_pair_cast.argtypes = [vp, vp, C.c_int64]
     T.rtr_test_queue_blocks_host.argtypes = [C.c_int32] * 6 + [vp, C.c_int64]
     T.rtr_test_queue_pack_host.argtypes = [C.c_int32] * 3 + [C.POINTER(C.c_uint32), C.POINTER(C.c_uint32), vp]
@@ -232,6 +235,18 @@
     shapes = np.zeros(n.value, dtype=np.int32)
     T.rtr_test_pair_frames(C.byref(d), shapes.ctypes.data, len(shapes), C.byref(n))
     return [FRAME_SHAPES[k] for k in shapes]
+
+
+def pair_program(scene):
+    T = test_lib()
+    d = scene.desc()
+    n = C.c_int64(0)
+    rc = T.rtr_test_pair_program(C.byref(d), None, 0, C.byref(n))
+    if rc != 0:
+        raise RtrError(rc, "scene rejected")
+    words = np.zeros(n.value, dtype=np.uint64)
+    T.rtr_test_pair_program(C.byref(d), words.ctypes.data, len(words), C.byref(n))
+    return words
 
 
 def pair_frame_host(shape, ops, ao, ad, bo, bd):
```

Result: faster. 5858, median of 6 (+2.1%).
